# chaitjo/efficient-gnns

Measured on NVIDIA H100. Metric: edges aggregated/s (fwd+bwd), 3-layer GCN student + logit-KD, ARXIV-shape, higher is better.
Workload: dtype f32

## Files before the change

### efficient-gnns_b200/csrc/dense_rows.cu

```cuda
#include "common.cuh"
#include "philox.cuh"

namespace b200gnn {

constexpr int ROWS_THREADS = 256;

struct RowMap {
  int nvec, rows_per_iter, cv, rg;
  bool active;
};
__device__ __forceinline__ RowMap make_row_map(int K) {
  RowMap m;
  m.nvec = K >> 2;
  m.rows_per_iter = ROWS_THREADS / m.nvec;
  m.rg = threadIdx.x / m.nvec;
  m.cv = threadIdx.x - m.rg * m.nvec;
  m.active = m.rg < m.rows_per_iter;
  return m;
}

__device__ __forceinline__ float4 ld4(const float* p) { return *reinterpret_cast<const float4*>(p); }
__device__ __forceinline__ float4 ld4s(const float* p) { return __ldcs(reinterpret_cast<const float4*>(p)); }
__device__ __forceinline__ void st4(float* p, const float4& v) { *reinterpret_cast<float4*>(p) = v; }

// ... 132 lines not shown
        y.z = m.z ? y.z * inv_keep : 0.f; y.w = m.w ? y.w * inv_keep : 0.f;
      }
      st4(out + 4 * i, y);
    }
  }
}

struct RowScatter {
  float* ptr[16];
  int32_t off[17];
  int32_t n;
  int64_t ld, col;
};
__device__ __forceinline__ float* scatter_row(const RowScatter& sc, int64_t r) {
  int q = 0;
#pragma unroll 1
  while (q + 1 < sc.n && r >= sc.off[q + 1]) ++q;
  return sc.ptr[q] + (size_t)(r - sc.off[q]) * (size_t)sc.ld + sc.col;
}

template <bool P16>
__global__ void __launch_bounds__(256) affine_relu_dropout_mapped_kernel(
    const float* __restrict__ Y, float* __restrict__ out, int64_t n_rows, int nvec_l, const float* __restrict__ scale,
    const float* __restrict__ shift, int relu, float p, uint32_t thr16, uint64_t seed, uint64_t offset,
    const int32_t* __restrict__ step_dev, uint64_t step_mul, const int32_t* __restrict__ rowmap, uint64_t row_offset,
    uint64_t nvec_g, uint64_t cv_off, int paired, const RowScatter sc) {
  const float inv_keep = p > 0.f ? 1.f / (1.f - p) : 1.f;
  if (step_dev) offset += (uint64_t)(*step_dev) * step_mul;
  const int64_t tid = (int64_t)blockIdx.x * blockDim.x + threadIdx.x, stride = (int64_t)gridDim.x * blockDim.x;
  if (P16 && paired) {
    const int half_l = nvec_l >> 1;
    for (int64_t u = tid; u < n_rows * half_l; u += stride) {
      const int64_t r = u / half_l;
      const int cv = (int)(u - r * half_l) * 2;
      const uint64_t gid = rowmap ? (uint64_t)rowmap[r] : (uint64_t)r + row_offset;
      const uint64_t g = gid * nvec_g + cv_off + (uint64_t)cv;
      const uint4 rnd = philox4x32(seed, offset, g >> 1);
#pragma unroll
      for (int half = 0; half < 2; ++half) {
        const int64_t i = r * nvec_l + cv + half;
        float4 y = affine_relu4(ld4s(Y + 4 * i), scale, shift, cv + half, relu);
        const uchar4 m = keep16(half ? rnd.z : rnd.x, half ? rnd.w : rnd.y, thr16);
        y.x = m.x ? y.x * inv_keep : 0.f; y.y = m.y ? y.y * inv_keep : 0.f;
        y.z = m.z ? y.z * inv_keep : 0.f; y.w = m.w ? y.w * inv_keep : 0.f;
        st4(out + 4 * i, y);
        if (sc.n) st4(scatter_row(sc, r) + 4 * (cv + half), y);
      }
    }
    return;
  }
  for (int64_t i = tid; i < n_rows * nvec_l; i += stride) {
    const int64_t r = i / nvec_l;
    const int cv = (int)(i - r * nvec_l);
    float4 y = affine_relu4(ld4s(Y + 4 * i), scale, shift, cv, relu);
    if (p > 0.f) {
      const uint64_t gid = rowmap ? (uint64_t)rowmap[r] : (uint64_t)r + row_offset;
      const uint64_t g = gid * nvec_g + cv_off + (uint64_t)cv;
      uchar4 m;
      if (P16) {
        const uint4 rnd = philox4x32(seed, offset, g >> 1);
        m = keep16((g & 1) ? rnd.z : rnd.x, (g & 1) ? rnd.w : rnd.y, thr16);
      } else {
        m = keep24(philox4x32(seed, offset, g), p);
      }
      y.x = m.x ? y.x * inv_keep : 0.f; y.y = m.y ? y.y * inv_keep : 0.f;
      y.z = m.z ? y.z * inv_keep : 0.f; y.w = m.w ? y.w * inv_keep : 0.f;
    }
    st4(out + 4 * i, y);
    if (sc.n) st4(scatter_row(sc, r) + 4 * cv, y);
  }
}

__global__ void __launch_bounds__(256) dropout_mask_kernel(uint8_t* __restrict__ mask, int64_t n_vec, float p, int p16,
                                                           uint32_t thr16, uint64_t seed, uint64_t offset) {
  for (int64_t i = (int64_t)blockIdx.x * blockDim.x + threadIdx.x; i < n_vec; i += (int64_t)gridDim.x * blockDim.x) {
    uchar4 m;
    if (p16) {
      const uint4 r = philox4x32(seed, offset, (uint64_t)i >> 1);
      m = keep16((i & 1) ? r.z : r.x, (i & 1) ? r.w : r.y, thr16);
    } else {
      m = keep24(philox4x32(seed, offset, (uint64_t)i), p);
    }
    reinterpret_cast<uchar4*>(mask)[i] = m;
  }
}

static inline bool dropout_p16(float p, uint32_t& thr16) {
  const double t = (double)p * 65536.0;
  thr16 = (uint32_t)t;
  return p > 0.f && t == (double)thr16;
}

__global__ void __launch_bounds__(256) relu_dropout_bwd_kernel(const float4* __restrict__ dOut, const float4* __restrict__ Xout,
                                                               float4* dY, int64_t n_vec, float inv_keep) {
  for (int64_t i = (int64_t)blockIdx.x * blockDim.x + threadIdx.x; i < n_vec; i += (int64_t)gridDim.x * blockDim.x) {
    const float4 g = dOut[i], x = Xout[i];
    float4 d;
    d.x = x.x > 0.f ? g.x * inv_keep : 0.f; d.y = x.y > 0.f ? g.y * inv_keep : 0.f;
    d.z = x.z > 0.f ? g.z * inv_keep : 0.f; d.w = x.w > 0.f ? g.w * inv_keep : 0.f;
    dY[i] = d;
  }
}

__global__ void __launch_bounds__(ROWS_THREADS) bn_act_bwd_reduce_kernel(
    const float* __restrict__ dOut, const float* __restrict__ Xout, const float* __restrict__ Y,
    const float* __restrict__ mean, const float* __restrict__ invstd, int64_t n_rows, int K, float inv_keep,
    float* __restrict__ partial, int slots) {
  extern __shared__ float smem[];
  const RowMap m = make_row_map(K);
  const int64_t per = (n_rows + slots - 1) / slots;
  const int64_t r0 = (int64_t)blockIdx.x * per, r1 = min(n_rows, r0 + per);
  float4 s = make_float4(0, 0, 0, 0), q = s;
  if (m.active) {
    const float4 mu = ld4(mean + 4 * m.cv), is = ld4(invstd + 4 * m.cv);
    for (int64_t r = r0 + m.rg; r < r1; r += m.rows_per_iter) {
      const size_t o = (size_t)r * K + 4 * m.cv;
      const float4 g = ld4(dOut + o), x = ld4(Xout + o), y = ld4(Y + o);
      const float dx = x.x > 0.f ? g.x * inv_keep : 0.f, dy = x.y > 0.f ? g.y * inv_keep : 0.f;
      const float dz = x.z > 0.f ? g.z * inv_keep : 0.f, dw = x.w > 0.f ? g.w * inv_keep : 0.f;
      s.x += dx; s.y += dy; s.z += dz; s.w += dw;
      q.x = fmaf(dx, (y.x - mu.x) * is.x, q.x); q.y = fmaf(dy, (y.y - mu.y) * is.y, q.y);
      q.z = fmaf(dz, (y.z - mu.z) * is.z, q.z); q.w = fmaf(dw, (y.w - mu.w) * is.w, q.w);
    }
  }
  reduce_store_2xK(m, K, s, q, smem, partial + (size_t)blockIdx.x * 2 * K);
}

__global__ void __launch_bounds__(256) bn_bwd_finalize_kernel(const float* __restrict__ partial, int slots, int K,
                                                              int64_t n, const float* __restrict__ gamma,
                                                              const float* __restrict__ invstd, float* dgamma,
                                                              float* dbeta, float* coef ) {
  double s, q; int k;
  if (finalize_reduce(partial, slots, K, true, s, q, k)) {
    dbeta[k] = (float)s;
    dgamma[k] = (float)q;
    coef[k] = gamma[k] * invstd[k];
    coef[K + k] = (float)(s / (double)n);
    coef[2 * K + k] = (float)(q / (double)n);
  }
}

template <bool DZ>
__global__ void __launch_bounds__(ROWS_THREADS) bn_act_bwd_apply_kernel(
    const float* __restrict__ dOut, const float* __restrict__ Xout, const float* __restrict__ Y,
    const float* __restrict__ mean, const float* __restrict__ invstd, const float* __restrict__ coef, int64_t n_rows,
    int K, float inv_keep, float* __restrict__ dY, float* __restrict__ colsum_partial, int slots) {
  extern __shared__ float smem[];
  const RowMap m = make_row_map(K);
  const int64_t per = (n_rows + slots - 1) / slots;
  const int64_t r0 = (int64_t)blockIdx.x * per, r1 = min(n_rows, r0 + per);
  float4 s = make_float4(0, 0, 0, 0), q = s;
  if (m.active) {
    const float4 mu = ld4(mean + 4 * m.cv), is = ld4(invstd + 4 * m.cv);
    const float4 c1 = ld4(coef + 4 * m.cv), c2 = ld4(coef + K + 4 * m.cv), c3 = ld4(coef + 2 * K + 4 * m.cv);
    for (int64_t r = r0 + m.rg; r < r1; r += m.rows_per_iter) {
      const size_t o = (size_t)r * K + 4 * m.cv;
      float4 g = ld4s(dOut + o);
      const float4 y = ld4s(Y + o);
      if (!DZ) {
        const float4 x = ld4s(Xout + o);
        g.x = x.x > 0.f ? g.x * inv_keep : 0.f; g.y = x.y > 0.f ? g.y * inv_keep : 0.f;
        g.z = x.z > 0.f ? g.z * inv_keep : 0.f; g.w = x.w > 0.f ? g.w * inv_keep : 0.f;
      }
      float4 d;
      d.x = c1.x * (g.x - c2.x - (y.x - mu.x) * is.x * c3.x);
      d.y = c1.y * (g.y - c2.y - (y.y - mu.y) * is.y * c3.y);
// ... 87 lines not shown
  if (!rows_ok(n_rows, K) || !Y || !out || p < 0.f || p >= 1.f || ((scale == nullptr) != (shift == nullptr)) ||
      !aligned_to(Y, 16) || !aligned_to(out, 16))
    return B200GNN_ERR_BAD_ARG;
  if (n_rows == 0) return B200GNN_OK;
  const int64_t n_vec = n_rows * (K / 4);
  uint32_t thr16 = 0;
  if (dropout_p16(p, thr16))
    affine_relu_dropout_kernel<true><<<grid_for((n_vec + 1) / 2 + 1, 256 * 2), 256, 0, (cudaStream_t)stream>>>(
        Y, out, n_vec, (int)(K / 4), scale, shift, relu, p, thr16, seed, offset, step_dev, step_mul,
        row_offset * (uint64_t)(K / 4));
  else
    affine_relu_dropout_kernel<false><<<grid_for(n_vec, 256 * 4), 256, 0, (cudaStream_t)stream>>>(
        Y, out, n_vec, (int)(K / 4), scale, shift, relu, p, 0u, seed, offset, step_dev, step_mul,
        row_offset * (uint64_t)(K / 4));
  return check_launch();
}

static int mapped_launch(const float* Y, float* out, int64_t n_rows, int64_t K, const float* scale, const float* shift, int relu,
                         float p, uint64_t seed, uint64_t offset, const int32_t* step_dev, uint64_t step_mul, const int32_t* rowmap,
                         uint64_t row_offset, int64_t K_global, int64_t col_offset, const RowScatter& sc, void* stream) {
  if (!rows_ok(n_rows, K) || !Y || !out || p < 0.f || p >= 1.f || ((scale == nullptr) != (shift == nullptr)) ||
      !aligned_to(Y, 16) || !aligned_to(out, 16) || K_global < K || K_global % 4 || col_offset < 0 || col_offset % 4 ||
      col_offset + K > K_global)
    return B200GNN_ERR_BAD_ARG;
  if (n_rows == 0) return B200GNN_OK;
  const int nvec_l = (int)(K / 4);
  const uint64_t nvec_g = (uint64_t)(K_global / 4), cv_off = (uint64_t)(col_offset / 4);
  const int paired = (nvec_l % 2 == 0 && nvec_g % 2 == 0 && cv_off % 2 == 0) ? 1 : 0;
  const int64_t n_vec = n_rows * nvec_l;
  uint32_t thr16 = 0;
  if (dropout_p16(p, thr16))
    affine_relu_dropout_mapped_kernel<true><<<grid_for(paired ? n_vec / 2 : n_vec, 256 * 2), 256, 0, (cudaStream_t)stream>>>(
        Y, out, n_rows, nvec_l, scale, shift, relu, p, thr16, seed, offset, step_dev, step_mul, rowmap, row_offset, nvec_g,
        cv_off, paired, sc);
  else
    affine_relu_dropout_mapped_kernel<false><<<grid_for(n_vec, 256 * 4), 256, 0, (cudaStream_t)stream>>>(
        Y, out, n_rows, nvec_l, scale, shift, relu, p, 0u, seed, offset, step_dev, step_mul, rowmap, row_offset, nvec_g,
        cv_off, 0, sc);
  return check_launch();
}

extern "C" int b200gnn_affine_relu_dropout_mapped_f32(const float* Y, float* out, int64_t n_rows, int64_t K,
                                                      const float* scale, const float* shift, int relu, float p,
                                                      uint64_t seed, uint64_t offset, const int32_t* step_dev,
                                                      uint64_t step_mul, const int32_t* rowmap, uint64_t row_offset,
                                                      int64_t K_global, int64_t col_offset, void* stream) {
  RowScatter sc;
  sc.n = 0; sc.ld = 0; sc.col = 0;
  return mapped_launch(Y, out, n_rows, K, scale, shift, relu, p, seed, offset, step_dev, step_mul, rowmap, row_offset, K_global,
                       col_offset, sc, stream);
}

extern "C" int b200gnn_affine_relu_dropout_scatter_f32(const float* Y, float* out, int64_t n_rows, int64_t K,
                                                       const float* scale, const float* shift, int relu, float p,
                                                       uint64_t seed, uint64_t offset, const int32_t* step_dev,
                                                       uint64_t step_mul, const int32_t* rowmap, uint64_t row_offset,
                                                       int64_t K_global, int64_t col_offset, float* const* dst_ptrs,
                                                       const int32_t* row_off, int32_t world, int64_t ld_dst, void* stream) {
  if (!dst_ptrs || !row_off || world <= 0 || world > 16 || ld_dst < K_global || ld_dst % 4 || row_off[0] != 0 ||
      row_off[world] != n_rows)
    return B200GNN_ERR_BAD_ARG;
  RowScatter sc;
  sc.n = world; sc.ld = ld_dst; sc.col = col_offset;
  for (int q = 0; q < world; ++q) {
    if (!dst_ptrs[q] || !aligned_to(dst_ptrs[q], 16) || row_off[q + 1] < row_off[q]) return B200GNN_ERR_BAD_ARG;
    sc.ptr[q] = dst_ptrs[q]; sc.off[q] = row_off[q];
  }
  sc.off[world] = row_off[world];
  return mapped_launch(Y, out, n_rows, K, scale, shift, relu, p, seed, offset, step_dev, step_mul, rowmap, row_offset, K_global,
                       col_offset, sc, stream);
}

extern "C" int b200gnn_dropout_mask_u8(uint8_t* mask, int64_t n_rows, int64_t K, float p, uint64_t seed,
                                       uint64_t offset, void* stream) {
  if (!rows_ok(n_rows, K) || !mask || p < 0.f || p >= 1.f) return B200GNN_ERR_BAD_ARG;
  if (n_rows == 0) return B200GNN_OK;
  const int64_t n_vec = n_rows * (K / 4);
  uint32_t thr16 = 0;
  const int p16 = dropout_p16(p, thr16) ? 1 : 0;
  dropout_mask_kernel<<<grid_for(n_vec, 256 * 4), 256, 0, (cudaStream_t)stream>>>(mask, n_vec, p, p16, thr16, seed, offset);
  return check_launch();
}

extern "C" int b200gnn_relu_dropout_bwd_f32(const float* dOut, const float* Xout, float* dY, int64_t n_rows, int64_t K,
                                            float p, void* stream) {
  if (!rows_ok(n_rows, K) || p < 0.f || p >= 1.f) return B200GNN_ERR_BAD_ARG;
  if (n_rows == 0) return B200GNN_OK;
  if (!dOut || !Xout || !dY || !aligned_to(dOut, 16) || !aligned_to(Xout, 16) || !aligned_to(dY, 16)) return B200GNN_ERR_BAD_ARG;
  const int64_t n_vec = n_rows * (K / 4);
  const float inv_keep = p > 0.f ? 1.f / (1.f - p) : 1.f;
  relu_dropout_bwd_kernel<<<grid_for(n_vec, 256 * 4), 256, 0, (cudaStream_t)stream>>>(
      reinterpret_cast<const float4*>(dOut), reinterpret_cast<const float4*>(Xout), reinterpret_cast<float4*>(dY), n_vec, inv_keep);
  return check_launch();
}

extern "C" int b200gnn_bn_act_bwd_reduce_f32(const float* dOut, const float* Xout, const float* Y, const float* mean,
                                             const float* invstd, int64_t n_rows, int64_t K, float p, float* partial,
                                             int64_t slots, void* stream) {
  if (!rows_ok(n_rows, K) || n_rows == 0 || !dOut || !Xout || !Y || !mean || !invstd || !partial || slots < 1 ||
      p < 0.f || p >= 1.f)
    return B200GNN_ERR_BAD_ARG;
  if (ROWS_THREADS / (K / 4) < 1) return B200GNN_ERR_UNSUPPORTED;
  const float inv_keep = p > 0.f ? 1.f / (1.f - p) : 1.f;
  bn_act_bwd_reduce_kernel<<<(int)slots, ROWS_THREADS, 2 * K * sizeof(float), (cudaStream_t)stream>>>(
      dOut, Xout, Y, mean, invstd, n_rows, (int)K, inv_keep, partial, (int)slots);
  return check_launch();
}

extern "C" int b200gnn_bn_act_bwd_apply_f32(const float* dOut, const float* Xout, const float* Y, const float* mean,
                                            const float* invstd, const float* gamma, const float* sums,
                                            int64_t sum_slots, int64_t n_norm, int64_t n_rows, int64_t K, float p,
                                            float* dY, float* dgamma, float* dbeta, float* dbias, float* partial,
                                            int64_t slots, float* coef, void* stream) {
  if (!rows_ok(n_rows, K) || n_rows == 0 || !dOut || !Y || !mean || !invstd || !gamma || !sums || !dY ||
      !dgamma || !dbeta || !partial || !coef || slots < 1 || sum_slots < 1 || n_norm < 1 || p < 0.f || p >= 1.f)
    return B200GNN_ERR_BAD_ARG;
  cudaStream_t st = (cudaStream_t)stream;
  const float inv_keep = p > 0.f ? 1.f / (1.f - p) : 1.f;
  const size_t smem = 2 * K * sizeof(float);
  int rc;
  bn_bwd_finalize_kernel<<<(int)((K + FIN_COLS - 1) / FIN_COLS), 256, 0, st>>>(sums, (int)sum_slots, (int)K, n_norm, gamma,
                                                                              invstd, dgamma, dbeta, coef);
  if ((rc = check_launch())) return rc;
  if (Xout)
    bn_act_bwd_apply_kernel<false><<<(int)slots, ROWS_THREADS, smem, st>>>(dOut, Xout, Y, mean, invstd, coef, n_rows, (int)K,
                                                                          inv_keep, dY, dbias ? partial : nullptr, (int)slots);
  else
    bn_act_bwd_apply_kernel<true><<<(int)slots, ROWS_THREADS, smem, st>>>(dOut, nullptr, Y, mean, invstd, coef, n_rows, (int)K,
                                                                         inv_keep, dY, dbias ? partial : nullptr, (int)slots);
  if ((rc = check_launch())) return rc;
  if (dbias) {
    colsum_finalize_kernel<<<(int)((K + FIN_COLS - 1) / FIN_COLS), 256, 0, st>>>(partial, (int)slots, (int)K, dbias);
    if ((rc = check_launch())) return rc;
  }
  return B200GNN_OK;
}

extern "C" int b200gnn_bn_act_bwd_f32(const float* dOut, const float* Xout, const float* Y, const float* mean,
                                      const float* invstd, const float* gamma, int64_t n_rows, int64_t K, float p,
                                      float* dY, float* dgamma, float* dbeta, float* dbias, float* partial,
                                      int64_t slots, float* coef, void* stream) {
  int rc = b200gnn_bn_act_bwd_reduce_f32(dOut, Xout, Y, mean, invstd, n_rows, K, p, partial, slots, stream);
  if (rc) return rc;
  return b200gnn_bn_act_bwd_apply_f32(dOut, Xout, Y, mean, invstd, gamma, partial, slots, n_rows, n_rows, K, p, dY,
                                      dgamma, dbeta, dbias, partial, slots, coef, stream);
}

extern "C" int b200gnn_partial_reduce_f32(const float* partial, int64_t slots, int64_t K2, float* out, void* stream) {
  if (!partial || !out || slots < 1 || K2 < 1) return B200GNN_ERR_BAD_ARG;
  partial_reduce_kernel<<<(int)((K2 + FIN_COLS - 1) / FIN_COLS), 256, 0, (cudaStream_t)stream>>>(partial, (int)slots, (int)K2,
                                                                                               out);
  return check_launch();
}

extern "C" int b200gnn_col_sum_f32(const float* Y, int64_t n_rows, int64_t K, float* out, float* partial,
                                   int64_t slots, void* stream) {
  if (!rows_ok(n_rows, K) || !Y || !out || !partial || slots < 1) return B200GNN_ERR_BAD_ARG;
  cudaStream_t st = (cudaStream_t)stream;
  int rc;
  col_stats4_kernel<<<(int)slots, ROWS_THREADS, 2 * K * sizeof(float), st>>>(Y, n_rows, (int)K, partial, (int)slots);
  if ((rc = check_launch())) return rc;
  colsum_finalize_kernel<<<(int)((K + FIN_COLS - 1) / FIN_COLS), 256, 0, st>>>(partial, (int)slots, (int)K, out);
  return check_launch();
}

extern "C" int b200gnn_adam_step_f32(float* params, const float* grads, float* exp_avg, float* exp_avg_sq, int64_t n,
// ... 12 lines not shown
```

### efficient-gnns_b200/csrc/gemm_tf32x3.cu

```cuda
#include <cuda.h>

#include "common.cuh"
#include "tc_common.cuh"

namespace b200gnn {
namespace gemm {
using namespace tc;

constexpr int BM = 128, BK = 32;
constexpr int THREADS = 384;
constexpr int CONSUMER_WARPS = 8;
constexpr int TILE_BYTES = BM * BK * 4;
constexpr int BAR_BYTES = 256;
constexpr int EPI_BYTES = CONSUMER_WARPS * 16 * 32 * 4;
constexpr int STAT_MAX_N = 256;
constexpr int STAT_BYTES = CONSUMER_WARPS * 2 * STAT_MAX_N * 4;
constexpr int XY_ROWS = 16;
constexpr int XY_SLOT_BYTES = 2 * XY_ROWS * 32 * 4;
constexpr int XY_BYTES = CONSUMER_WARPS * 2 * XY_SLOT_BYTES;
constexpr int XY_BAR_OFF = 128;
constexpr int BNBWD_TMA_MAX_K = 128;

template <int BN_T, int NSTAGE, int EXTRA = 0>
struct Cfg {
  static constexpr int BN = BN_T, STAGES = NSTAGE;
  static constexpr int B_TILE_BYTES = BN_T * BK * 4;
  static constexpr int STAGE_BYTES = TILE_BYTES + 2 * B_TILE_BYTES;
  static constexpr int ACC = BN_T / 2;
  static constexpr int SMEM_BYTES = NSTAGE * STAGE_BYTES + BAR_BYTES + EPI_BYTES + STAT_BYTES + EXTRA + 1024;
  static_assert(B_TILE_BYTES % 1024 == 0 && (BN_T == 128 || BN_T == 48), "tile shape (wgmma wrappers: N = 128, 48)");
  static_assert(2 * NSTAGE * 8 <= XY_BAR_OFF, "barrier block");
  static_assert(SMEM_BYTES <= 232448, "shared memory");
};

__device__ __forceinline__ void mma(float (&d)[64], const uint32_t (&a)[4], uint64_t b, uint32_t s) { wgmma_tf32_n128_rs(d, a, b, s); }
__device__ __forceinline__ void mma(float (&d)[24], const uint32_t (&a)[4], uint64_t b, uint32_t s) { wgmma_tf32_n48_rs(d, a, b, s); }

__device__ __forceinline__ uint32_t a_frag_offset(int r0, int lane) { return r0 * 128 + ((lane >> 2) << 4) + (lane & 3) * 4; }
__device__ __forceinline__ void load_a(uint32_t frag, uint32_t (&v)[BK / 8][4]) {
  asm("" : "+r"(frag));
#pragma unroll
  for (int k = 0; k < BK / 8; ++k)
#pragma unroll
    for (int i = 0; i < 4; ++i) v[k][i] = lds32((frag ^ ((2 * k + (i >> 1)) << 4)) + (i & 1) * 8 * 128);
}

__device__ __forceinline__ int stg(int r, int c4) { return r * 32 + ((c4 ^ (r & 7)) << 2); }

struct Params {
  float* C;
  const float* bias;
  int64_t ldc;
  int32_t M, N, K;
  int32_t accumulate;
  float* Cp[16];
  int32_t n_peer, kc;
  int64_t row_off;
  int32_t bcast;
  int32_t stat_mode;
  float* stat_partial;
  const float* bn_x;
  const float* bn_y;
  const float* bn_mean;
  const float* bn_invstd;
  float inv_keep;
};

__device__ __forceinline__ void load_bn_chunk(const Params& p, int m0, int col, int q, int lane, float4 (&x)[4], float4 (&y)[4]) {
  if (col + 32 > p.N) return;
  const int sub = lane >> 3, cq = (lane & 7) * 4;
#pragma unroll
  for (int it = 0; it < 4; ++it) {
    const int grow = m0 + q * 16 + it * 4 + sub;
    if (grow < p.M) {
      const size_t o = (size_t)grow * p.ldc + col + cq;
      x[it] = __ldg(reinterpret_cast<const float4*>(p.bn_x + o));
      y[it] = __ldg(reinterpret_cast<const float4*>(p.bn_y + o));
    }
  }
}

template <class C, int STAT, bool PEER>
__global__ void __launch_bounds__(THREADS, 1)
gemm_tf32x3_kernel(const __grid_constant__ CUtensorMap tmA, const __grid_constant__ CUtensorMap tmBhi,
                   const __grid_constant__ CUtensorMap tmBlo, const __grid_constant__ CUtensorMap tmX,
                   const __grid_constant__ CUtensorMap tmY, const Params p) {
  constexpr bool BNB = STAT >= 2;
  constexpr bool XYTMA = STAT == 3;
  constexpr int BN = C::BN, STAGES = C::STAGES, STAGE_BYTES = C::STAGE_BYTES, B_TILE_BYTES = C::B_TILE_BYTES, ACC = C::ACC;
  extern __shared__ uint8_t smem_raw[];
  uint8_t* smem = reinterpret_cast<uint8_t*>((reinterpret_cast<uintptr_t>(smem_raw) + 1023) & ~(uintptr_t)1023);
  uint64_t* bars = reinterpret_cast<uint64_t*>(smem + STAGES * STAGE_BYTES);
  uint64_t* full = bars;
  uint64_t* empty = bars + STAGES;
  float* epi_smem = reinterpret_cast<float*>(smem + STAGES * STAGE_BYTES + BAR_BYTES);
  float* stat_smem = reinterpret_cast<float*>(smem + STAGES * STAGE_BYTES + BAR_BYTES + EPI_BYTES);
  uint8_t* xy_smem = smem + STAGES * STAGE_BYTES + BAR_BYTES + EPI_BYTES + STAT_BYTES;
  uint64_t* xy_full = reinterpret_cast<uint64_t*>(smem + STAGES * STAGE_BYTES + XY_BAR_OFF);

  const int warp = threadIdx.x >> 5, lane = threadIdx.x & 31;

  if (threadIdx.x == 0) {
    for (int s = 0; s < STAGES; ++s) { mbar_init(&full[s], 1); mbar_init(&empty[s], 256); }
    if (XYTMA)
      for (int i = 0; i < 2 * CONSUMER_WARPS; ++i) mbar_init(&xy_full[i], 1);
    asm volatile("fence.mbarrier_init.release.cluster;" ::: "memory");
  }
  __syncthreads();

  const int num_m = (p.M + BM - 1) / BM, num_n = (p.N + BN - 1) / BN;
  const int num_tiles = num_m * num_n;
  const int num_kb = (p.K + BK - 1) / BK;

  if (warp < 4) {
    regs_dec<40>();
    if (threadIdx.x == 0) {
      int s = 0; uint32_t ph = 0;
      for (int tile = blockIdx.x; tile < num_tiles; tile += gridDim.x) {
        const int m0 = (tile / num_n) * BM, n0 = (tile % num_n) * BN;
        for (int kb = 0; kb < num_kb; ++kb) {
          mbar_wait(&empty[s], ph ^ 1);
          uint8_t* st = smem + s * STAGE_BYTES;
          mbar_expect_tx(&full[s], TILE_BYTES + 2 * B_TILE_BYTES);
          tma_load_2d(&tmA, &full[s], st, kb * BK, m0);
          tma_load_2d(&tmBhi, &full[s], st + TILE_BYTES, kb * BK, n0);
          tma_load_2d(&tmBlo, &full[s], st + TILE_BYTES + B_TILE_BYTES, kb * BK, n0);
          if (++s == STAGES) { s = 0; ph ^= 1; }
        }
      }
    }
    return;
  }
  regs_inc<232>();

  const int q = warp - 4;
  const bool vec_ok = PEER ? true : ((p.ldc % 4 == 0) && ((reinterpret_cast<uintptr_t>(p.C) & 15) == 0));
  float* stat = stat_smem + q * (2 * STAT_MAX_N);
  if (STAT) {
    for (int i = lane; i < 2 * p.N; i += 32) stat[i] = 0.f;
    __syncwarp();
  }
  constexpr int NCHUNK = (BN + 31) / 32;
  uint8_t* xy = xy_smem + q * (2 * XY_SLOT_BYTES);
  uint64_t* xyb = xy_full + q * 2;
  int n_mine = 0;
  if (XYTMA) {
    for (int tt = blockIdx.x; tt < num_tiles; tt += gridDim.x) n_mine += NCHUNK;
    if (lane == 0)
      for (int g = 0; g < 2 && g < n_mine; ++g) {
        const int tt = blockIdx.x + (g / NCHUNK) * gridDim.x, cc = g % NCHUNK;
        mbar_expect_tx(&xyb[g], XY_SLOT_BYTES);
        tma_load_2d(&tmX, &xyb[g], xy + g * XY_SLOT_BYTES, (tt % num_n) * BN + cc * 32, (tt / num_n) * BM + q * XY_ROWS);
        tma_load_2d(&tmY, &xyb[g], xy + g * XY_SLOT_BYTES + XY_SLOT_BYTES / 2, (tt % num_n) * BN + cc * 32,
                    (tt / num_n) * BM + q * XY_ROWS);
      }
  }
  float acc[ACC], sum[ACC];
  uint32_t ah0[BK / 8][4], al0[BK / 8][4], ah1[BK / 8][4], al1[BK / 8][4];
  const uint32_t frag = a_frag_offset(q * 16 + (lane >> 2), lane);
  int s = 0; uint32_t ph = 0;
  int g_chunk = 0;
  for (int tile = blockIdx.x; tile < num_tiles; tile += gridDim.x) {
    const int m0 = (tile / num_n) * BM, n0 = (tile % num_n) * BN;
#pragma unroll
    for (int i = 0; i < ACC; ++i) sum[i] = acc[i] = 0.f;
    int prev = 0;
    auto stage = [&](int kb, uint32_t (&h)[BK / 8][4], uint32_t (&l)[BK / 8][4]) {
      mbar_wait(&full[s], ph);
      uint8_t* st = smem + s * STAGE_BYTES;
      load_a(smem_u32(st) + frag, h);
#pragma unroll
      for (int k = 0; k < BK / 8; ++k)
#pragma unroll
        for (int i = 0; i < 4; ++i) split1(h[k][i], h[k][i], l[k][i]);
      reg_fence(h); reg_fence(l);
      if (kb > 0) {
        wgmma_wait<0>();
        acc_fence(acc);
#pragma unroll
        for (int i = 0; i < ACC; ++i) sum[i] += acc[i];
        mbar_arrive(&empty[prev]);
      }
      wgmma_fence();
      const uint32_t sb = smem_u32(st + TILE_BYTES);
#pragma unroll
      for (int k = 0; k < BK / 8; ++k) {
        const uint32_t koff = k * 32;
        mma(acc, l[k], make_desc_k128(sb + koff), k != 0);
        mma(acc, h[k], make_desc_k128(sb + B_TILE_BYTES + koff), 1);
      }
#pragma unroll
      for (int k = 0; k < BK / 8; ++k) mma(acc, h[k], make_desc_k128(sb + k * 32), 1);
      wgmma_commit();
      prev = s;
      if (++s == STAGES) { s = 0; ph ^= 1; }
    };
    for (int kb = 0; kb < num_kb; kb += 2) {
      stage(kb, ah0, al0);
      if (kb + 1 < num_kb) stage(kb + 1, ah1, al1);
    }
    wgmma_wait<0>();
    acc_fence(acc);
#pragma unroll
    for (int i = 0; i < ACC; ++i) sum[i] += acc[i];
    mbar_arrive(&empty[prev]);

    float* tile_s = epi_smem + q * (16 * 32);
#pragma unroll
    for (int c = 0; c < NCHUNK; ++c, ++g_chunk) {
      const int col0 = n0 + c * 32;
      float4 xr[4], yr[4];
      if (STAT == 2) load_bn_chunk(p, m0, col0, q, lane, xr, yr);
#pragma unroll
      for (int jj = 0; jj < 4; ++jj) {
        const int j = c * 4 + jj;
        if (j * 8 < BN) {
          const int r0 = lane >> 2, cc = jj * 8 + 2 * (lane & 3);
          *reinterpret_cast<float2*>(tile_s + stg(r0, cc >> 2) + (cc & 3)) = make_float2(sum[4 * j], sum[4 * j + 1]);
          *reinterpret_cast<float2*>(tile_s + stg(r0 + 8, cc >> 2) + (cc & 3)) = make_float2(sum[4 * j + 2], sum[4 * j + 3]);
        }
      }
      __syncwarp();
      if (vec_ok && col0 + 32 <= p.N) {
        const float* xs = reinterpret_cast<const float*>(xy + (g_chunk & 1) * XY_SLOT_BYTES);
        const float* ys = xs + XY_ROWS * 32;
        if (XYTMA) mbar_wait(&xyb[g_chunk & 1], (uint32_t)((g_chunk >> 1) & 1));
        const int sub = lane >> 3, cq = (lane & 7) * 4;
        float4 b4 = make_float4(0.f, 0.f, 0.f, 0.f);
        if (p.bias) b4 = make_float4(__ldg(p.bias + col0 + cq), __ldg(p.bias + col0 + cq + 1), __ldg(p.bias + col0 + cq + 2),
                                     __ldg(p.bias + col0 + cq + 3));
        float4 s4 = make_float4(0.f, 0.f, 0.f, 0.f), q4 = s4, mu4 = s4, is4 = s4;
        if (BNB) {
          mu4 = __ldg(reinterpret_cast<const float4*>(p.bn_mean + col0 + cq));
          is4 = __ldg(reinterpret_cast<const float4*>(p.bn_invstd + col0 + cq));
        }
#pragma unroll
        for (int it = 0; it < 4; ++it) {
          const int rr = it * 4 + sub;
          const int grow = m0 + q * 16 + rr;
          float4 v = *reinterpret_cast<const float4*>(tile_s + stg(rr, lane & 7));
          v.x += b4.x; v.y += b4.y; v.z += b4.z; v.w += b4.w;
          if (PEER && grow < p.M && p.bcast) {
            for (int r = 0; r < p.n_peer; ++r)
              *reinterpret_cast<float4*>(p.Cp[r] + (size_t)(p.row_off + grow) * p.ldc + col0 + cq) = v;
          } else if (grow < p.M) {
            float4* dst;
            if (PEER) {
              const int r = col0 / p.kc;
              dst = reinterpret_cast<float4*>(p.Cp[r] + (size_t)(p.row_off + grow) * p.kc + (col0 - r * p.kc) + cq);
            } else {
              dst = reinterpret_cast<float4*>(p.C + (size_t)grow * p.ldc + col0 + cq);
            }
            if (!PEER && p.accumulate) { const float4 o = *dst; v.x += o.x; v.y += o.y; v.z += o.z; v.w += o.w; }
            if (STAT == 1) {
              vstat(s4, q4, v);
            } else if (BNB) {
              const float4 x = XYTMA ? *reinterpret_cast<const float4*>(xs + rr * 32 + cq) : xr[it];
              const float4 y = XYTMA ? *reinterpret_cast<const float4*>(ys + rr * 32 + cq) : yr[it];
              v.x = x.x > 0.f ? v.x * p.inv_keep : 0.f; v.y = x.y > 0.f ? v.y * p.inv_keep : 0.f;
              v.z = x.z > 0.f ? v.z * p.inv_keep : 0.f; v.w = x.w > 0.f ? v.w * p.inv_keep : 0.f;
              s4.x += v.x; s4.y += v.y; s4.z += v.z; s4.w += v.w;
              q4.x = fmaf(v.x, (y.x - mu4.x) * is4.x, q4.x); q4.y = fmaf(v.y, (y.y - mu4.y) * is4.y, q4.y);
              q4.z = fmaf(v.z, (y.z - mu4.z) * is4.z, q4.z); q4.w = fmaf(v.w, (y.w - mu4.w) * is4.w, q4.w);
            }
            *dst = v;
          }
        }
        if (STAT) {
#pragma unroll
          for (int d = 8; d <= 16; d <<= 1) {
            s4.x += __shfl_xor_sync(0xffffffffu, s4.x, d); s4.y += __shfl_xor_sync(0xffffffffu, s4.y, d);
            s4.z += __shfl_xor_sync(0xffffffffu, s4.z, d); s4.w += __shfl_xor_sync(0xffffffffu, s4.w, d);
            q4.x += __shfl_xor_sync(0xffffffffu, q4.x, d); q4.y += __shfl_xor_sync(0xffffffffu, q4.y, d);
            q4.z += __shfl_xor_sync(0xffffffffu, q4.z, d); q4.w += __shfl_xor_sync(0xffffffffu, q4.w, d);
          }
          if (lane < 8) {
            float4* ps = reinterpret_cast<float4*>(stat + col0 + cq);
            float4* pq = reinterpret_cast<float4*>(stat + p.N + col0 + cq);
            float4 a0 = *ps, a1 = *pq;
            a0.x += s4.x; a0.y += s4.y; a0.z += s4.z; a0.w += s4.w;
            a1.x += q4.x; a1.y += q4.y; a1.z += q4.z; a1.w += q4.w;
            *ps = a0; *pq = a1;
          }
        }
        __syncwarp();
        if (XYTMA && lane == 0 && g_chunk + 2 < n_mine) {
          const int g = g_chunk + 2, tt = blockIdx.x + (g / NCHUNK) * gridDim.x, cc = g % NCHUNK;
          uint8_t* dst = xy + (g & 1) * XY_SLOT_BYTES;
          mbar_expect_tx(&xyb[g & 1], XY_SLOT_BYTES);
          tma_load_2d(&tmX, &xyb[g & 1], dst, (tt % num_n) * BN + cc * 32, (tt / num_n) * BM + q * XY_ROWS);
          tma_load_2d(&tmY, &xyb[g & 1], dst + XY_SLOT_BYTES / 2, (tt % num_n) * BN + cc * 32, (tt / num_n) * BM + q * XY_ROWS);
        }
      } else {
        const int rr = lane & 15, cb = (lane >> 4) * 16, grow = m0 + q * 16 + rr;
        if (grow < p.M && col0 + cb < p.N) {
          for (int jx = 0; jx < 16; ++jx) {
            const int cc = cb + jx, col = col0 + cc;
            if (col >= p.N) break;
            const float v = tile_s[stg(rr, cc >> 2) + (cc & 3)] + (p.bias ? __ldg(p.bias + col) : 0.f);
            if (PEER && p.bcast) {
              for (int r = 0; r < p.n_peer; ++r) p.Cp[r][(size_t)(p.row_off + grow) * p.ldc + col] = v;
            } else if (!PEER) {
              float* dst = p.C + (size_t)grow * p.ldc + col;
              *dst = v + (p.accumulate ? *dst : 0.f);
            }
          }
        }
        __syncwarp();
      }
    }
  }
  if (STAT) {
    __syncwarp();
    float* out = p.stat_partial + (size_t)(blockIdx.x * CONSUMER_WARPS + q) * 2 * p.N;
    for (int i = lane; i < 2 * p.N; i += 32) out[i] = stat[i];
  }
}

__global__ void __launch_bounds__(256) split_tf32_kernel(const float* __restrict__ W, int64_t rows, int64_t cols,
                                                         int transpose, float* __restrict__ hi, float* __restrict__ lo) {
  const int64_t n = rows * cols;
  for (int64_t i = (int64_t)blockIdx.x * blockDim.x + threadIdx.x; i < n; i += (int64_t)gridDim.x * blockDim.x) {
    const int64_t r = i / cols, c = i - r * cols;
    uint32_t h, l;
    split1(__float_as_uint(W[i]), h, l);
    const int64_t o = transpose ? c * rows + r : i;
    hi[o] = __uint_as_float(h);
    lo[o] = __uint_as_float(l);
  }
}

static bool make_map(CUtensorMap* m, const float* base, int64_t rows, int64_t cols, int64_t ld, int box_rows, bool swizzle = true) {
  EncodeTiledFn fn = encode_fn();
  if (!fn) return false;
  cuuint64_t dims[2] = {(cuuint64_t)cols, (cuuint64_t)rows};
  cuuint64_t strides[1] = {(cuuint64_t)ld * 4};
  cuuint32_t box[2] = {(cuuint32_t)BK, (cuuint32_t)box_rows};
  cuuint32_t estr[2] = {1, 1};
  return fn(m, CU_TENSOR_MAP_DATA_TYPE_FLOAT32, 2, const_cast<float*>(base), dims, strides, box, estr,
            CU_TENSOR_MAP_INTERLEAVE_NONE, swizzle ? CU_TENSOR_MAP_SWIZZLE_128B : CU_TENSOR_MAP_SWIZZLE_NONE,
            CU_TENSOR_MAP_L2_PROMOTION_L2_256B, CU_TENSOR_MAP_FLOAT_OOB_FILL_NONE) == CUDA_SUCCESS;
}

template <class C, int STAT = 0, bool PEER = false>
static int launch(const float* A, int64_t lda, const float* B_hi, const float* B_lo, int64_t ldb, const Params& p,
                  cudaStream_t stream) {
  CUtensorMap tA, tBh, tBl, tX, tY;
  if (!make_map(&tA, A, p.M, p.K, lda, BM) || !make_map(&tBh, B_hi, p.N, p.K, ldb, C::BN) ||
      !make_map(&tBl, B_lo, p.N, p.K, ldb, C::BN))
    return B200GNN_ERR_UNSUPPORTED;
  tX = tA; tY = tA;
  if (STAT == 3 && (!make_map(&tX, p.bn_x, p.M, p.N, p.ldc, XY_ROWS, false) || !make_map(&tY, p.bn_y, p.M, p.N, p.ldc, XY_ROWS, false)))
    return B200GNN_ERR_UNSUPPORTED;
  int dev = 0, sms = 132;
  cudaGetDevice(&dev);
  static bool attr_set[64] = {};
  if (dev >= 0 && dev < 64 && !attr_set[dev]) {
    cudaError_t e = cudaFuncSetAttribute(gemm_tf32x3_kernel<C, STAT, PEER>, cudaFuncAttributeMaxDynamicSharedMemorySize, C::SMEM_BYTES);
    if (e != cudaSuccess) { set_cuda_error(e); return B200GNN_ERR_CUDA; }
    attr_set[dev] = true;
  }
  const int tiles = ((p.M + BM - 1) / BM) * ((p.N + C::BN - 1) / C::BN);
  cudaDeviceGetAttribute(&sms, cudaDevAttrMultiProcessorCount, dev);
  const int grid = tiles < sms ? tiles : sms;
  gemm_tf32x3_kernel<C, STAT, PEER><<<grid, THREADS, C::SMEM_BYTES, stream>>>(tA, tBh, tBl, tX, tY, p);
  return check_launch();
}

}
}

using namespace b200gnn;

extern "C" int b200gnn_split_tf32_f32(const float* W, int64_t rows, int64_t cols, int transpose, float* hi, float* lo,
                                      void* stream) {
  if (!W || !hi || !lo || rows <= 0 || cols <= 0) return B200GNN_ERR_BAD_ARG;
  const int64_t n = rows * cols;
  int grid = (int)((n + 255) / 256);
  if (grid > 132 * 8) grid = 132 * 8;
  gemm::split_tf32_kernel<<<grid, 256, 0, (cudaStream_t)stream>>>(W, rows, cols, transpose, hi, lo);
  return check_launch();
}

static int g_bnbwd_variant = 0;
extern "C" void b200gnn_gemm_set_bnbwd_variant(int v) { g_bnbwd_variant = v; }

static int gemm_dispatch(const float* A, int64_t lda, const float* B_hi, const float* B_lo, int64_t ldb, float* C, int64_t ldc,
                         int64_t M, int64_t N, int64_t K, const float* bias, int accumulate, void* stream,
                         const gemm::Params* st = nullptr) {
  if (!A || !B_hi || !B_lo || !C || M <= 0 || N <= 0 || K <= 0 || lda < K || ldb < K || ldc < N ||
      M >= INT32_MAX || N >= INT32_MAX || K >= INT32_MAX)
    return B200GNN_ERR_BAD_ARG;
  if (lda % 4 || ldb % 4 || !aligned_to(A, 16) || !aligned_to(B_hi, 16) || !aligned_to(B_lo, 16))
    return B200GNN_ERR_UNSUPPORTED;
  gemm::Params p{};
  p.C = C; p.bias = bias; p.ldc = ldc; p.M = (int32_t)M; p.N = (int32_t)N; p.K = (int32_t)K; p.accumulate = accumulate ? 1 : 0;
  p.n_peer = 0; p.kc = 0; p.row_off = 0; p.bcast = 0;
  if (st) {
    if (N % 32 || N > gemm::STAT_MAX_N || N <= 48 || ldc % 4 || !aligned_to(C, 16) || !st->stat_partial) return B200GNN_ERR_UNSUPPORTED;
    p.stat_mode = st->stat_mode; p.stat_partial = st->stat_partial; p.bn_x = st->bn_x; p.bn_y = st->bn_y;
    p.bn_mean = st->bn_mean; p.bn_invstd = st->bn_invstd; p.inv_keep = st->inv_keep;
    if (p.stat_mode == 1) return gemm::launch<gemm::Cfg<128, 4>, 1>(A, lda, B_hi, B_lo, ldb, p, (cudaStream_t)stream);
    if (N % 128 == 0 && (g_bnbwd_variant == 1 || (g_bnbwd_variant == 0 && K < gemm::BNBWD_TMA_MAX_K)))
      return gemm::launch<gemm::Cfg<128, 2, gemm::XY_BYTES>, 3>(A, lda, B_hi, B_lo, ldb, p, (cudaStream_t)stream);
    return gemm::launch<gemm::Cfg<128, 4>, 2>(A, lda, B_hi, B_lo, ldb, p, (cudaStream_t)stream);
  }
  if (N <= 48) return gemm::launch<gemm::Cfg<48, 6>>(A, lda, B_hi, B_lo, ldb, p, (cudaStream_t)stream);
  return gemm::launch<gemm::Cfg<128, 4>>(A, lda, B_hi, B_lo, ldb, p, (cudaStream_t)stream);
}

extern "C" int64_t b200gnn_gemm_stat_slots(int64_t M, int64_t N) {
  if (M <= 0 || N <= 0) return B200GNN_ERR_BAD_ARG;
  int dev = 0, sms = 132;
  cudaGetDevice(&dev);
  cudaDeviceGetAttribute(&sms, cudaDevAttrMultiProcessorCount, dev);
  const int64_t tiles = ((M + gemm::BM - 1) / gemm::BM) * ((N + 127) / 128);
  return gemm::CONSUMER_WARPS * (tiles < sms ? tiles : sms);
}

extern "C" int b200gnn_gemm_tf32x3_stats_f32(const float* A, int64_t lda, const float* B_hi, const float* B_lo, int64_t ldb,
                                             float* C, int64_t ldc, int64_t M, int64_t N, int64_t K, const float* bias,
                                             int accumulate, float* partial, int64_t slots, void* stream) {
  if (!partial || slots < b200gnn_gemm_stat_slots(M, N) || (accumulate && bias)) return B200GNN_ERR_BAD_ARG;
  gemm::Params st{};
  st.stat_mode = 1; st.stat_partial = partial;
  return gemm_dispatch(A, lda, B_hi, B_lo, ldb, C, ldc, M, N, K, bias, accumulate, stream, &st);
}

extern "C" int b200gnn_gemm_tf32x3_bnbwd_f32(const float* A, int64_t lda, const float* B_hi, const float* B_lo, int64_t ldb,
                                             float* C, int64_t ldc, int64_t M, int64_t N, int64_t K, int accumulate,
                                             const float* Xout, const float* Y, const float* mean, const float* invstd, float p_drop,
                                             float* partial, int64_t slots, void* stream) {
  if (!partial || !Xout || !Y || !mean || !invstd || p_drop < 0.f || p_drop >= 1.f || slots < b200gnn_gemm_stat_slots(M, N))
    return B200GNN_ERR_BAD_ARG;
  if (!aligned_to(Xout, 16) || !aligned_to(Y, 16) || !aligned_to(mean, 16) || !aligned_to(invstd, 16)) return B200GNN_ERR_UNSUPPORTED;
  gemm::Params st{};
  st.stat_mode = 2; st.stat_partial = partial; st.bn_x = Xout; st.bn_y = Y; st.bn_mean = mean; st.bn_invstd = invstd;
  st.inv_keep = p_drop > 0.f ? 1.f / (1.f - p_drop) : 1.f;
  return gemm_dispatch(A, lda, B_hi, B_lo, ldb, C, ldc, M, N, K, nullptr, accumulate, stream, &st);
}

extern "C" int b200gnn_gemm_tf32x3_f32(const float* A, int64_t lda, const float* B_hi, const float* B_lo, int64_t ldb,
                                       float* C, int64_t ldc, int64_t M, int64_t N, int64_t K, const float* bias,
                                       void* stream) {
  return gemm_dispatch(A, lda, B_hi, B_lo, ldb, C, ldc, M, N, K, bias, 0, stream);
}

extern "C" int b200gnn_gemm_tf32x3_acc_f32(const float* A, int64_t lda, const float* B_hi, const float* B_lo, int64_t ldb,
                                           float* C, int64_t ldc, int64_t M, int64_t N, int64_t K, void* stream) {
  return gemm_dispatch(A, lda, B_hi, B_lo, ldb, C, ldc, M, N, K, nullptr, 1, stream);
}

extern "C" int b200gnn_gemm_tf32x3_scatter_f32(const float* A, int64_t lda, const float* B_hi, const float* B_lo, int64_t ldb,
                                               float* const* C_ptrs, int32_t world, int64_t row_off, int64_t M, int64_t N, int64_t K,
                                               const float* bias, void* stream) {
  if (!A || !B_hi || !B_lo || !C_ptrs || world <= 0 || world > 16 || M <= 0 || N <= 0 || K <= 0 || lda < K || ldb < K || row_off < 0 ||
      M >= INT32_MAX || N >= INT32_MAX || K >= INT32_MAX)
    return B200GNN_ERR_BAD_ARG;
  if (N % world || (N / world) % 32 || N <= 48) return B200GNN_ERR_UNSUPPORTED;
  if (lda % 4 || ldb % 4 || !aligned_to(A, 16) || !aligned_to(B_hi, 16) || !aligned_to(B_lo, 16)) return B200GNN_ERR_UNSUPPORTED;
  gemm::Params p{};
  p.C = nullptr; p.bias = bias; p.ldc = N; p.M = (int32_t)M; p.N = (int32_t)N; p.K = (int32_t)K; p.accumulate = 0;
  p.n_peer = world; p.kc = (int32_t)(N / world); p.row_off = row_off; p.bcast = 0;
  for (int q = 0; q < world; ++q) {
    if (!C_ptrs[q] || !aligned_to(C_ptrs[q], 16)) return B200GNN_ERR_BAD_ARG;
    p.Cp[q] = C_ptrs[q];
  }
  return gemm::launch<gemm::Cfg<128, 4>, 0, true>(A, lda, B_hi, B_lo, ldb, p, (cudaStream_t)stream);
}

extern "C" int b200gnn_gemm_tf32x3_bcast_f32(const float* A, int64_t lda, const float* B_hi, const float* B_lo, int64_t ldb,
                                             float* const* C_ptrs, int32_t world, int64_t row_off, int64_t ldc, int64_t M, int64_t N,
                                             int64_t K, const float* bias, void* stream) {
  if (!A || !B_hi || !B_lo || !C_ptrs || world <= 0 || world > 16 || M <= 0 || N <= 0 || K <= 0 || lda < K || ldb < K || ldc < N ||
      row_off < 0 || M >= INT32_MAX || N >= INT32_MAX || K >= INT32_MAX)
    return B200GNN_ERR_BAD_ARG;
  if (lda % 4 || ldb % 4 || ldc % 4 || !aligned_to(A, 16) || !aligned_to(B_hi, 16) || !aligned_to(B_lo, 16)) return B200GNN_ERR_UNSUPPORTED;
  gemm::Params p{};
  p.C = C_ptrs[0]; p.bias = bias; p.ldc = ldc; p.M = (int32_t)M; p.N = (int32_t)N; p.K = (int32_t)K; p.accumulate = 0;
  p.n_peer = world; p.kc = (int32_t)N; p.row_off = row_off; p.bcast = 1;
  for (int q = 0; q < world; ++q) {
    if (!C_ptrs[q] || !aligned_to(C_ptrs[q], 16)) return B200GNN_ERR_BAD_ARG;
    p.Cp[q] = C_ptrs[q];
  }
  if (N <= 48) return gemm::launch<gemm::Cfg<48, 6>, 0, true>(A, lda, B_hi, B_lo, ldb, p, (cudaStream_t)stream);
  return gemm::launch<gemm::Cfg<128, 4>, 0, true>(A, lda, B_hi, B_lo, ldb, p, (cudaStream_t)stream);
}
```

### efficient-gnns_b200/csrc/gemm_wgrad_tf32x3.cu

```cuda
#include "common.cuh"
#include "tc_common.cuh"

namespace b200gnn {
namespace wgrad {
using namespace tc;

constexpr int BKN = 32;
constexpr int TM = 128, TN = 128;
constexpr int THREADS = 384;
constexpr int STAGES = 5;
constexpr int X_BOX = 8;
constexpr int RAW_BYTES = BKN * (TM + TN) * 4;
constexpr int OP_BYTES = 128 * BKN * 4;
constexpr int T_BYTES = 2 * OP_BYTES;
constexpr int SMEM_BYTES = STAGES * RAW_BYTES + 2 * T_BYTES + 256 + 1024;
constexpr int MAX_RANGES = 132;
constexpr int64_t MAX_PARTIAL_FLOATS = (int64_t)MAX_RANGES * 256 * 256;
constexpr int MAX_KIN = 2048, MAX_NOUT = 512;
static_assert(SMEM_BYTES <= 232448, "shared memory");

struct Params {
  float* partial;
  int32_t Nn, Kin, Kpad, Nout, Npad, num_kb;
  int32_t n_tn, n_ranges;
};

__global__ void __launch_bounds__(THREADS, 1)
wgrad_tf32x3_kernel(const __grid_constant__ CUtensorMap tmX, const __grid_constant__ CUtensorMap tmG, const Params p) {
  extern __shared__ uint8_t smem_raw[];
  uint8_t* smem = reinterpret_cast<uint8_t*>((reinterpret_cast<uintptr_t>(smem_raw) + 1023) & ~(uintptr_t)1023);
  uint8_t* tbuf = smem + STAGES * RAW_BYTES;
  uint64_t* full = reinterpret_cast<uint64_t*>(tbuf + 2 * T_BYTES);
  uint64_t* empty = full + STAGES;

  const int tiles = (p.Kpad / TM) * p.n_tn;
  const int tile = (int)blockIdx.x % tiles, range = (int)blockIdx.x / tiles;
  const int mt = tile / p.n_tn, nt = tile % p.n_tn;
  const int kb0 = (int)((int64_t)p.num_kb * range / p.n_ranges);
  const int kb1 = (int)((int64_t)p.num_kb * (range + 1) / p.n_ranges);

  const int warp = threadIdx.x >> 5, lane = threadIdx.x & 31;
  if (threadIdx.x == 0) {
    for (int s = 0; s < STAGES; ++s) { mbar_init(&full[s], 1); mbar_init(&empty[s], 256); }
    asm volatile("fence.mbarrier_init.release.cluster;" ::: "memory");
  }
  __syncthreads();

  if (warp < 4) {
    regs_dec<40>();
    if (threadIdx.x == 0) {
      int s = 0; uint32_t ph = 0;
      for (int kb = kb0; kb < kb1; ++kb) {
        mbar_wait(&empty[s], ph ^ 1);
        uint8_t* st = smem + s * RAW_BYTES;
        mbar_expect_tx(&full[s], RAW_BYTES);
        for (int j = 0; j < TM / X_BOX; ++j)
          tma_load_2d(&tmX, &full[s], st + j * BKN * X_BOX * 4, mt * TM + j * X_BOX, kb * BKN);
        tma_load_2d(&tmG, &full[s], st + BKN * TM * 4, nt * TN, kb * BKN);
        if (++s == STAGES) { s = 0; ph ^= 1; }
      }
    }
    return;
  }
  regs_inc<232>();

  const int cw = (warp >> 2) - 1;
  const int ct = threadIdx.x - 128;
  const uint32_t xfrag = (8 * cw + 2 * (warp & 3)) * (BKN * X_BOX * 4) + (lane & 3) * (X_BOX * 4) + (lane >> 2) * 4;
  float acc[64], sum[64];
#pragma unroll
  for (int i = 0; i < 64; ++i) sum[i] = acc[i] = 0.f;
  uint32_t xh0[BKN / 8][4], xl0[BKN / 8][4], xh1[BKN / 8][4], xl1[BKN / 8][4];
  int s = 0; uint32_t ph = 0;
  auto block = [&](int i, uint32_t (&h)[BKN / 8][4], uint32_t (&l)[BKN / 8][4]) {
    mbar_wait(&full[s], ph);
    const uint32_t sraw = smem_u32(smem + s * RAW_BYTES);
    const float* rg = reinterpret_cast<const float*>(smem + s * RAW_BYTES + BKN * TM * 4);
    uint8_t* T = tbuf + (i & 1) * T_BYTES;
#pragma unroll
    for (int u = 0; u < 4; ++u) {
      const int idx = u * 256 + ct;
      const int r = idx & 127, c = idx >> 7;
      const float* src = rg + (4 * c) * 128 + r;
      const uint4 v = make_uint4(__float_as_uint(src[0]), __float_as_uint(src[128]), __float_as_uint(src[256]),
                                 __float_as_uint(src[384]));
      uint4 hv, lv;
      split4(v, hv, lv);
      *reinterpret_cast<uint4*>(T + swz128(r, c)) = hv;
      *reinterpret_cast<uint4*>(T + OP_BYTES + swz128(r, c)) = lv;
    }
#pragma unroll
    for (int k = 0; k < BKN / 8; ++k)
#pragma unroll
      for (int j = 0; j < 4; ++j)
        split1(lds32(sraw + xfrag + (j & 1) * (BKN * X_BOX * 4) + (8 * k + 4 * (j >> 1)) * (X_BOX * 4)), h[k][j], l[k][j]);
    asm volatile("fence.proxy.async.shared::cta;" ::: "memory");
    mbar_arrive(&empty[s]);
    if (i > 0) {
      wgmma_wait<0>();
      acc_fence(acc);
#pragma unroll
      for (int j = 0; j < 64; ++j) sum[j] += acc[j];
    }
    named_sync(1, 256);
    reg_fence(h); reg_fence(l);
    wgmma_fence();
    const uint32_t sa = smem_u32(T);
#pragma unroll
    for (int k = 0; k < BKN / 8; ++k) {
      const uint32_t koff = k * 32;
      wgmma_tf32_n128_rs(acc, l[k], make_desc_k128(sa + koff), k != 0);
      wgmma_tf32_n128_rs(acc, h[k], make_desc_k128(sa + OP_BYTES + koff), 1);
    }
#pragma unroll
    for (int k = 0; k < BKN / 8; ++k) wgmma_tf32_n128_rs(acc, h[k], make_desc_k128(sa + k * 32), 1);
    wgmma_commit();
    if (++s == STAGES) { s = 0; ph ^= 1; }
  };
  for (int i = 0; i < kb1 - kb0; i += 2) {
    block(i, xh0, xl0);
    if (i + 1 < kb1 - kb0) block(i + 1, xh1, xl1);
  }
  if (kb1 > kb0) {
    wgmma_wait<0>();
    acc_fence(acc);
#pragma unroll
    for (int j = 0; j < 64; ++j) sum[j] += acc[j];
  }
  float* out = p.partial + (size_t)range * p.Kpad * p.Npad;
  const int row0 = mt * TM + cw * 64 + (warp & 3) * 16 + (lane >> 2);
#pragma unroll
  for (int j = 0; j < 16; ++j) {
    const int col = nt * TN + 8 * j + 2 * (lane & 3);
    if (col < p.Npad) {
      *reinterpret_cast<float2*>(out + (size_t)row0 * p.Npad + col) = make_float2(sum[4 * j], sum[4 * j + 1]);
      *reinterpret_cast<float2*>(out + (size_t)(row0 + 8) * p.Npad + col) = make_float2(sum[4 * j + 2], sum[4 * j + 3]);
    }
  }
}

constexpr int RED_VECS = 32, RED_GROUPS = 8;
__global__ void __launch_bounds__(RED_VECS * RED_GROUPS) wgrad_reduce_kernel(const float4* __restrict__ partial, int n_part,
                                                                             int Kin, int Kpad, int Nout, int Npad,
                                                                             float* __restrict__ out) {
  __shared__ float4 sh[RED_GROUPS][RED_VECS];
  const int64_t n_vec = (int64_t)Kpad * Npad / 4;
  const int v = threadIdx.x % RED_VECS, g = threadIdx.x / RED_VECS;
  const int64_t i = (int64_t)blockIdx.x * RED_VECS + v;
  float4 acc = make_float4(0.f, 0.f, 0.f, 0.f);
  if (i < n_vec)
    for (int c = g; c < n_part; c += RED_GROUPS) {
      const float4 x = __ldcs(partial + (size_t)c * n_vec + i);
      acc.x += x.x; acc.y += x.y; acc.z += x.z; acc.w += x.w;
    }
  sh[g][v] = acc;
  __syncthreads();
  if (g != 0 || i >= n_vec) return;
  const int row = (int)(i / (Npad / 4)), c4 = (int)(i % (Npad / 4)) * 4;
  if (c4 >= Nout || row >= Kin) return;
#pragma unroll
  for (int j = 1; j < RED_GROUPS; ++j) {
    const float4 x = sh[j][v];
    acc.x += x.x; acc.y += x.y; acc.z += x.z; acc.w += x.w;
  }
  *reinterpret_cast<float4*>(out + (size_t)row * Nout + c4) = acc;
}

static bool make_map_rows(CUtensorMap* m, const float* base, int64_t rows, int64_t width, int64_t ld, int box_cols) {
  EncodeTiledFn fn = encode_fn();
  if (!fn) return false;
  cuuint64_t dims[2] = {(cuuint64_t)width, (cuuint64_t)rows};
  cuuint64_t strides[1] = {(cuuint64_t)ld * 4};
  cuuint32_t box[2] = {(cuuint32_t)box_cols, (cuuint32_t)BKN};
  cuuint32_t estr[2] = {1, 1};
  return fn(m, CU_TENSOR_MAP_DATA_TYPE_FLOAT32, 2, const_cast<float*>(base), dims, strides, box, estr,
            CU_TENSOR_MAP_INTERLEAVE_NONE, CU_TENSOR_MAP_SWIZZLE_NONE, CU_TENSOR_MAP_L2_PROMOTION_L2_256B,
            CU_TENSOR_MAP_FLOAT_OOB_FILL_NONE) == CUDA_SUCCESS;
}

static int64_t pad_k(int64_t Kin) { return (Kin + TM - 1) / TM * TM; }
static int64_t pad_n(int64_t Nout) { return (Nout + 31) / 32 * 32; }
static int range_cap(int64_t Kin, int64_t Nout) {
  const int64_t c = MAX_PARTIAL_FLOATS / (pad_k(Kin) * pad_n(Nout));
  return (int)(c > MAX_RANGES ? MAX_RANGES : (c < 1 ? 1 : c));
}

}
}

using namespace b200gnn;

extern "C" int64_t b200gnn_wgrad_workspace_floats(int64_t Kin, int64_t Nout) {
  if (Kin <= 0 || Nout <= 0) return B200GNN_ERR_BAD_ARG;
  if (Kin > wgrad::MAX_KIN || Nout > wgrad::MAX_NOUT) return B200GNN_ERR_UNSUPPORTED;
  return wgrad::range_cap(Kin, Nout) * wgrad::pad_k(Kin) * wgrad::pad_n(Nout);
}

extern "C" int b200gnn_gemm_wgrad_tf32x3_f32(const float* X, int64_t ldx, const float* G, int64_t ldg, float* dW,
                                             int64_t Nn, int64_t Kin, int64_t Nout, float* workspace, void* stream) {
  if (!X || !G || !dW || !workspace || Nn <= 0 || Kin <= 0 || Nout <= 0 || ldx < Kin || ldg < Nout || Nn >= INT32_MAX)
    return B200GNN_ERR_BAD_ARG;
  if (Kin % 4 || Kin > wgrad::MAX_KIN || Nout % 4 || Nout > wgrad::MAX_NOUT || ldx % 4 || ldg % 4 || !aligned_to(X, 16) || !aligned_to(G, 16) ||
      !aligned_to(dW, 16) || !aligned_to(workspace, 16))
    return B200GNN_ERR_UNSUPPORTED;
  CUtensorMap tX, tG;
  if (!wgrad::make_map_rows(&tX, X, Nn, Kin, ldx, wgrad::X_BOX) || !wgrad::make_map_rows(&tG, G, Nn, Nout, ldg, wgrad::TN))
    return B200GNN_ERR_UNSUPPORTED;
  int dev = 0, sms = 132;
  cudaGetDevice(&dev);
  static bool attr_set[64] = {};
  if (dev >= 0 && dev < 64 && !attr_set[dev]) {
    cudaError_t e = cudaFuncSetAttribute(wgrad::wgrad_tf32x3_kernel, cudaFuncAttributeMaxDynamicSharedMemorySize,
                                         wgrad::SMEM_BYTES);
    if (e != cudaSuccess) { set_cuda_error(e); return B200GNN_ERR_CUDA; }
    attr_set[dev] = true;
  }
  cudaDeviceGetAttribute(&sms, cudaDevAttrMultiProcessorCount, dev);
  cudaStream_t st = (cudaStream_t)stream;
  wgrad::Params p;
  p.partial = workspace; p.Nn = (int32_t)Nn; p.Kin = (int32_t)Kin; p.Nout = (int32_t)Nout;
  p.Kpad = (int32_t)wgrad::pad_k(Kin);
  p.Npad = (int32_t)wgrad::pad_n(Nout);
  p.num_kb = (int32_t)((Nn + wgrad::BKN - 1) / wgrad::BKN);
  p.n_tn = (p.Npad + wgrad::TN - 1) / wgrad::TN;
  const int tiles = (int)(p.Kpad / wgrad::TM) * p.n_tn;
  int ranges = sms / tiles;
  const int cap = wgrad::range_cap(Kin, Nout);
  if (ranges > cap) ranges = cap;
  if (ranges > p.num_kb) ranges = p.num_kb;
  if (ranges < 1) ranges = 1;
  p.n_ranges = ranges;
  int rc;
  wgrad::wgrad_tf32x3_kernel<<<tiles * ranges, wgrad::THREADS, wgrad::SMEM_BYTES, st>>>(tX, tG, p);
  if ((rc = check_launch())) return rc;
  const int64_t n_vec = (int64_t)p.Kpad * p.Npad / 4;
  wgrad::wgrad_reduce_kernel<<<(int)((n_vec + wgrad::RED_VECS - 1) / wgrad::RED_VECS), wgrad::RED_VECS * wgrad::RED_GROUPS, 0, st>>>(
      reinterpret_cast<const float4*>(workspace), ranges, (int)Kin, p.Kpad, (int)Nout, p.Npad, dW);
  return check_launch();
}
```

### efficient-gnns_b200/dist.py

```python
from __future__ import annotations

import math
from dataclasses import dataclass
from typing import List, Optional

import torch
import torch.distributed as dist

from . import lib, ops
from .engine import GCNStudentTrainer, gcn_norm, _is_symmetric
from .sparse import SparseTensor, csr_graph_from


import os as _os
_DIAG_SKIP_COMM = _os.environ.get("B200GNN_DIAG_SKIP_ALLGATHER", "0") == "1"


@dataclass
class ShardPlan:
    world: int
    n: int
    block: int
    perm: torch.Tensor
    inv: torch.Tensor

    @property
    def n_pad(self) -> int:
        return self.world * self.block

    def real_rows(self, rank: int) -> int:
        full_rounds, rem = divmod(self.n, self.world)
        if rem == 0:
            return full_rounds
        last_round = full_rounds
        k_of_rank = rank if last_round % 2 == 0 else self.world - 1 - rank
        return full_rounds + (1 if k_of_rank < rem else 0)

    def rows_of(self, rank: int):
        return rank * self.block, rank * self.block + self.real_rows(rank)


def make_plan(rowcount: torch.Tensor, world: int) -> ShardPlan:
    n = rowcount.numel()
    block = -(-n // world)
    order = torch.argsort(rowcount.cpu(), descending=True, stable=True)
    pos = torch.arange(n)
    rnd, k = pos // world, pos % world
    rank_of = torch.where(rnd % 2 == 0, k, world - 1 - k)
    slot = rnd
    new_id = rank_of * block + slot
    inv = torch.empty(n, dtype=torch.long)
    inv[order] = new_id
    perm = torch.full((world * block,), -1, dtype=torch.long)
    perm[new_id] = order
    return ShardPlan(world, n, block, perm, inv)


def relabel_adjacency(adj: SparseTensor, plan: ShardPlan) -> SparseTensor:
    row, col, val = adj.coo()
    inv = plan.inv.to(row.device)
    return SparseTensor(row=inv[row], col=inv[col], value=val, sparse_sizes=(plan.n_pad, plan.n_pad), is_sorted=False)


def shard_rows(adj_relabelled: SparseTensor, plan: ShardPlan, rank: int):
    rowptr, col, val = adj_relabelled.csr()
    r0, r1 = plan.rows_of(rank)
    e0, e1 = int(rowptr[r0]), int(rowptr[r1])
    return (rowptr[r0:r1 + 1] - e0).contiguous(), col[e0:e1].contiguous(), None if val is None else val[e0:e1].contiguous()


def scatter_rows(t: torch.Tensor, plan: ShardPlan, fill=0) -> torch.Tensor:
    out = torch.full((plan.n_pad,) + tuple(t.shape[1:]), fill, dtype=t.dtype, device=t.device)
    out[plan.inv.to(t.device)] = t
    return out


class ShardedGCNTrainer(GCNStudentTrainer):

    def __init__(self, adj: SparseTensor, dims: List[int], group=None, **kw):
        assert dist.is_initialized(), "torch.distributed must be initialised (backend nccl)"
        self.group = group
        self.rank, self.world = dist.get_rank(group), dist.get_world_size(group)
        norm = gcn_norm(adj)
        if not _is_symmetric(norm):
            raise NotImplementedError("node-parallel backward relies on a symmetric normalised adjacency")
        self.plan = make_plan(norm.storage.rowcount(), self.world)
        rel = relabel_adjacency(norm, self.plan)
        rowptr, col, val = shard_rows(rel, self.plan, self.rank)
        self._shard = csr_graph_from(rowptr, col, val, self.plan.real_rows(self.rank), self.plan.n_pad)
        self.n_global = adj.size(0)
        super().__init__(adj, dims, _prebuilt_graph=self._shard, _rows_alloc=self.plan.block, **kw)
        dev = self.device
        self.full = {k: torch.empty(self.plan.n_pad, k, device=dev) for k in set(dims[1:])}
        self.sum_buf = {k: torch.empty(2, k, device=dev) for k in set(dims[1:])}
        self.row0 = self.rank * self.plan.block
        self.n_train_global = 0

    def shard_inputs(self, x, y, train_idx, teacher_logits=None):
        plan, dev = self.plan, self.device
        r0, r1 = plan.rows_of(self.rank)
        x_pad = scatter_rows(x.to(dev), plan)
        y_loc = scatter_rows(y.to(dev), plan)[r0:r1].contiguous()
        t_loc = None if teacher_logits is None else scatter_rows(teacher_logits.to(dev), plan)[r0:r1].contiguous()
        new_train = plan.inv.to(dev)[train_idx.to(dev)]
        mine = new_train[(new_train >= r0) & (new_train < r1)] - r0
        self.n_train_global = int(train_idx.numel())
        return x_pad, y_loc, torch.sort(mine).values.contiguous(), t_loc

    def _block_of(self, view: torch.Tensor) -> torch.Tensor:
        for blk in self._blocks:
            if blk.data_ptr() == view.data_ptr() and blk.shape[1] == view.shape[1]:
                return blk
        raise KeyError("not an engine activation buffer")

    def gather_rows(self, local: torch.Tensor) -> torch.Tensor:
        blk = torch.zeros(self.plan.block, local.shape[1], device=local.device)
        blk[:local.shape[0]] = local
        full = torch.empty(self.plan.n_pad, local.shape[1], device=local.device)
        dist.all_gather_into_tensor(full, blk, group=self.group)
        return full[self.plan.inv.to(local.device)]

    def _all_gather(self, local: torch.Tensor) -> torch.Tensor:
        full = self.full[local.shape[1]]
        if _DIAG_SKIP_COMM:
            return full
        dist.all_gather_into_tensor(full, self._block_of(local), group=self.group)
        return full

    def _global_stats(self, partial: torch.Tensor, k: int) -> torch.Tensor:
        s = ops.partial_reduce(partial, out=self.sum_buf[k])
        dist.all_reduce(s, group=self.group)
        return s.view(1, 2, k)

    def forward(self, x_pad: torch.Tensor, training: bool = True) -> torch.Tensor:
        r0 = self.row0
        inp = None
        for l in range(self.L):
            last = l == self.L - 1
            k = self.dims[l + 1]
            if l == 0 and self.agg_first:
                ops.spmm_csr(self.G, x_pad, "sum", out=self.AX)
                self._linear(0, self.AX, self.Y[0], bias=self.b[0])
                part = ops.col_stats(self.Y[0], partial=self._part(k)) if training else None
            else:
                src = x_pad[r0:r0 + self.N] if l == 0 else inp
                self._linear(l, src, self.H[l])
                full = self._all_gather(self.H[l])
                if last or not training:
                    ops.spmm_csr(self.G, full, "sum", bias=self.b[l], out=self.Y[l]); part = None
                else:
                    part = self.stat_part[l]
                    ops.spmm_csr(self.G, full, "sum", bias=self.b[l], out=self.Y[l], stat_partial=part)
            if last:
                break
            if training:
                sums = self._global_stats(part, k)
                ops.bn_finalize(sums, self.n_global, self.gamma[l], self.beta[l], self.bn_eps, self.bn_momentum,
                                self.running_mean[l], self.running_var[l], out=self.bn[l])
                ops.affine_relu_dropout(self.Y[l], self.bn[l][2], self.bn[l][3], True, self.p, self.seed, l, out=self.A[l],
                                        step_dev=self.step_count, step_mul=self.L, row_offset=r0)
            else:
                scale = self.gamma[l] * torch.rsqrt(self.running_var[l] + self.bn_eps)
                shift = self.beta[l] - self.running_mean[l] * scale
                ops.affine_relu_dropout(self.Y[l], scale, shift, True, 0.0, out=self.A[l])
            inp = self.A[l]
        return self.Y[-1]

    def backward(self, x_pad: torch.Tensor):
        r0 = self.row0
        for l in range(self.L - 1, -1, -1):
            k_out = self.dims[l + 1]
            inp = x_pad[r0:r0 + self.N] if l == 0 else self.A[l - 1]
            if l == self.L - 1:
                ops.col_sum(self.dY[l], out=self.gb[l], partial=self._part(k_out))
# ... 37 lines not shown
```

### efficient-gnns_b200/engine.py

```python
from __future__ import annotations

import math
from typing import Dict, List, Optional

import torch

from . import lib, ops
from .sparse import CsrGraph, SparseTensor


def gcn_norm(adj: SparseTensor) -> SparseTensor:
    if not adj.has_value():
        adj = adj.fill_value(1.0)
    adj = adj.fill_diag(1.0)
    deg = adj.sum(dim=1)
    dis = deg.pow(-0.5)
    dis.masked_fill_(dis == float("inf"), 0.0)
    row, col, val = adj.coo()
    return adj.set_value(dis[row] * val * dis[col])


def _is_symmetric(adj: SparseTensor) -> bool:
    st = adj.storage
    if st.sparse_sizes()[0] != st.sparse_sizes()[1]:
        return False
    perm = st.csr2csc()
    same = torch.equal(st.col()[perm], st.row()) and torch.equal(st.row()[perm], st.col())
    if same and st.value() is not None:
        same = torch.equal(st.value()[perm], st.value())
    return bool(same)


class GCNStudentTrainer:

    def __init__(self, adj: SparseTensor, dims: List[int], dropout: float = 0.5, lr: float = 0.01, seed: int = 0,
                 alpha: float = 0.9, kd_T: float = 4.0, bn_eps: float = 1e-5, bn_momentum: float = 0.1,
                 aggregate_first: Optional[bool] = None, tensor_core_gemm: bool = True, overlap_wgrad: bool = True,
                 fuse_row_passes: bool = True, _prebuilt_graph: Optional[CsrGraph] = None, _rows_alloc: Optional[int] = None):
        assert adj.is_cuda(), "the engine runs on a CUDA device"
        self.device = adj.device
        self.dims, self.L = list(dims), len(dims) - 1
        self.p, self.lr, self.alpha, self.kd_T = float(dropout), float(lr), float(alpha), float(kd_T)
        self.bn_eps, self.bn_momentum = bn_eps, bn_momentum
        self.seed = int(seed)
        self.tc_gemm = bool(tensor_core_gemm) and all(d % 4 == 0 for d in dims)
        for d in dims[1:]:
            assert d % 4 == 0 and d <= 1024, "layer widths must be multiples of 4 (128-bit rows)"
        self.N = adj.size(0)
        self.agg_first = (dims[0] < dims[1] and dims[0] % 4 == 0) if aggregate_first is None else bool(aggregate_first)
        if self.L < 2:
            self.agg_first = False

        if _prebuilt_graph is not None:
            self.G = self.Gt = _prebuilt_graph
            self.N = _prebuilt_graph.n_rows
        else:
            norm = gcn_norm(adj)
            self.G: CsrGraph = norm.storage.engine_csr()
            self.Gt: CsrGraph = self.G if _is_symmetric(norm) else norm.storage.engine_csc("value")
        self.nnz = self.G.nnz

        sizes = []
        for l in range(self.L):
            sizes += [dims[l] * dims[l + 1], dims[l + 1]]
            if l < self.L - 1:
                sizes += [dims[l + 1], dims[l + 1]]
        n_par = sum(sizes)
        dev = self.device
        self.params = torch.zeros(n_par, device=dev)
        self.n_par_pad = (n_par + 3) // 4 * 4
        self._grads_buf = torch.zeros(self.n_par_pad + 4, device=dev)
        self.grads = self._grads_buf[:n_par]
        self.exp_avg = torch.zeros(n_par, device=dev)
        self.exp_avg_sq = torch.zeros(n_par, device=dev)
        self.step_count = torch.zeros(1, dtype=torch.int32, device=dev)
        self.W, self.b, self.gamma, self.beta = [], [], [], []
        self.gW, self.gb, self.ggamma, self.gbeta = [], [], [], []
        off = 0

        def take(n, shape):
            nonlocal off
            v = (self.params[off:off + n].view(shape), self.grads[off:off + n].view(shape))
            off += n
            return v
        for l in range(self.L):
            w, gw = take(dims[l] * dims[l + 1], (dims[l], dims[l + 1]))
            b, gb = take(dims[l + 1], (dims[l + 1],))
            self.W.append(w); self.gW.append(gw); self.b.append(b); self.gb.append(gb)
            if l < self.L - 1:
                g, gg = take(dims[l + 1], (dims[l + 1],))
                be, gbe = take(dims[l + 1], (dims[l + 1],))
                self.gamma.append(g); self.ggamma.append(gg); self.beta.append(be); self.gbeta.append(gbe)
        self.Wt_split = [(torch.empty(dims[l + 1], dims[l], device=dev), torch.empty(dims[l + 1], dims[l], device=dev))
                         for l in range(self.L)]
        self.W_split = [(torch.empty(dims[l], dims[l + 1], device=dev), torch.empty(dims[l], dims[l + 1], device=dev))
                        for l in range(self.L)]
        wg = [ops.wgrad_supported(dims[l], dims[l + 1]) for l in range(self.L)]
        self.wgrad_ws = (torch.empty(max(ops.wgrad_workspace_floats(dims[l], dims[l + 1]) for l in range(self.L) if wg[l]), device=dev)
                         if self.tc_gemm and any(wg) else None)
        self.running_mean = [torch.zeros(d, device=dev) for d in dims[1:-1]]
        self.running_var = [torch.ones(d, device=dev) for d in dims[1:-1]]
        self.reset_parameters(seed)

        N = self.N
        rows_alloc = N if _rows_alloc is None else _rows_alloc
        self._blocks = []

        def buf(k):
            blk = torch.zeros(rows_alloc, k, device=dev)
            self._blocks.append(blk)
            return blk[:N]
        self.H = [buf(dims[l + 1]) for l in range(self.L)]
        self.Y = [buf(dims[l + 1]) for l in range(self.L)]
        self.A = [buf(dims[l + 1]) for l in range(self.L - 1)]
        self.dY = [buf(dims[l + 1]) for l in range(self.L)]
        self.dH = [buf(dims[l + 1]) for l in range(self.L)]
        self.dA = [buf(dims[l + 1]) for l in range(self.L - 1)]
        self.AX = buf(dims[0]) if self.agg_first else None
        slots_spmm = ops.stat_slots(self.G)
        self.stat_part = [torch.empty(slots_spmm, 2, dims[l + 1], device=dev) for l in range(self.L - 1)]
        self.bn = [torch.empty(4, dims[l + 1], device=dev) for l in range(self.L - 1)]
        self.rs = ops.rows_slots(N)
        self.fuse_rows = bool(fuse_row_passes) and self.tc_gemm
        self._gemm_part = {k: torch.empty(ops.gemm_stat_slots(N, k), 2, k, device=dev)
                           for k in set(dims[1:-1]) if self.fuse_rows and ops.gemm_stats_supported(k)}
        self.loss_out = self._grads_buf[self.n_par_pad:self.n_par_pad + 3]
        self.kd_part = torch.empty(2 * int(lib.load().b200gnn_kd_partials(N)), device=dev)
        self._graph = None
        self.overlap_wgrad = overlap_wgrad
        self._side = torch.cuda.Stream(device=dev) if overlap_wgrad else None
        self._ev_fork, self._ev_join = torch.cuda.Event(), torch.cuda.Event()
        self._static: Dict[str, torch.Tensor] = {}
        for k in set(dims[1:]):
            self._part(k); self._coef(k)

    def reset_parameters(self, seed: int = 0):
        g = torch.Generator().manual_seed(seed)
        for l in range(self.L):
            fan_in, fan_out = self.dims[l], self.dims[l + 1]
            a = math.sqrt(6.0 / (fan_in + fan_out))
            self.W[l].copy_((torch.rand(fan_in, fan_out, generator=g) * 2 - 1) * a)
            self.b[l].zero_()
        for l in range(self.L - 1):
            self.gamma[l].fill_(1.0); self.beta[l].zero_()
            self.running_mean[l].zero_(); self.running_var[l].fill_(1.0)
        self.exp_avg.zero_(); self.exp_avg_sq.zero_(); self.step_count.zero_()

    def state_dict(self) -> Dict[str, torch.Tensor]:
        sd = {}
        for l in range(self.L):
            sd[f"convs.{l}.weight"] = self.W[l].detach().clone()
            sd[f"convs.{l}.bias"] = self.b[l].detach().clone()
        for l in range(self.L - 1):
            sd[f"bns.{l}.weight"] = self.gamma[l].detach().clone()
            sd[f"bns.{l}.bias"] = self.beta[l].detach().clone()
            sd[f"bns.{l}.running_mean"] = self.running_mean[l].clone()
            sd[f"bns.{l}.running_var"] = self.running_var[l].clone()
        return sd

    def load_state_dict(self, sd: Dict[str, torch.Tensor]):
        for l in range(self.L):
            self.W[l].copy_(sd[f"convs.{l}.weight"]); self.b[l].copy_(sd[f"convs.{l}.bias"])
        for l in range(self.L - 1):
            self.gamma[l].copy_(sd[f"bns.{l}.weight"]); self.beta[l].copy_(sd[f"bns.{l}.bias"])
            if f"bns.{l}.running_mean" in sd:
                self.running_mean[l].copy_(sd[f"bns.{l}.running_mean"]); self.running_var[l].copy_(sd[f"bns.{l}.running_var"])

    def activation_pattern(self, l: int) -> torch.Tensor:
        return self.A[l] > 0

    def out_feat(self) -> torch.Tensor:
        return self.A[-1]

    def dropout_offset(self, layer: int, step: int) -> int:
        return layer + step * self.L

    def forward(self, x: torch.Tensor, training: bool = True) -> torch.Tensor:
        inp = x
        for l in range(self.L):
            last = l == self.L - 1
            if l == 0 and self.agg_first:
                ops.spmm_csr(self.G, x, "sum", out=self.AX)
                if training:
                    gp = self._gemm_part.get(self.dims[1])
                    if gp is not None:
                        hi, lo = ops.split_tf32(self.W[0], transpose=True, hi=self.Wt_split[0][0], lo=self.Wt_split[0][1])
                        ops.gemm_tf32x3_stats(self.AX, hi, lo, self.b[0], self.Y[0], gp)
                        part = gp
                    else:
                        self._linear(0, self.AX, self.Y[0], bias=self.b[0])
                        part = ops.col_stats(self.Y[0], partial=self._part(self.dims[1]))
                    ops.bn_finalize(part, self.N, self.gamma[0], self.beta[0], self.bn_eps,
                                    self.bn_momentum, self.running_mean[0], self.running_var[0], out=self.bn[0])
                    ops.affine_relu_dropout(self.Y[0], self.bn[0][2], self.bn[0][3], True, self.p, self.seed, 0,
                                            out=self.A[0], step_dev=self.step_count, step_mul=self.L)
                else:
                    self._linear(0, self.AX, self.Y[0], bias=self.b[0])
                    scale = self.gamma[0] * torch.rsqrt(self.running_var[0] + self.bn_eps)
                    shift = self.beta[0] - self.running_mean[0] * scale
                    ops.affine_relu_dropout(self.Y[0], scale, shift, True, 0.0, out=self.A[0])
                inp = self.A[0]
                continue
            self._linear(l, inp, self.H[l])
            if last:
                ops.spmm_csr(self.G, self.H[l], "sum", bias=self.b[l], out=self.Y[l])
            elif training:
                ops.spmm_csr(self.G, self.H[l], "sum", bias=self.b[l], out=self.Y[l], stat_partial=self.stat_part[l])
                ops.bn_finalize(self.stat_part[l], self.N, self.gamma[l], self.beta[l], self.bn_eps, self.bn_momentum,
                                self.running_mean[l], self.running_var[l], out=self.bn[l])
                ops.affine_relu_dropout(self.Y[l], self.bn[l][2], self.bn[l][3], True, self.p, self.seed, l,
                                        out=self.A[l], step_dev=self.step_count, step_mul=self.L)
                inp = self.A[l]
            else:
                ops.spmm_csr(self.G, self.H[l], "sum", bias=self.b[l], out=self.Y[l])
                scale = self.gamma[l] * torch.rsqrt(self.running_var[l] + self.bn_eps)
                shift = self.beta[l] - self.running_mean[l] * scale
                ops.affine_relu_dropout(self.Y[l], scale, shift, True, 0.0, out=self.A[l])
                inp = self.A[l]
        return self.Y[-1]

    def backward(self, x: torch.Tensor, d_out_feat: Optional[torch.Tensor] = None):
        for l in range(self.L - 1, -1, -1):
            inp = x if l == 0 else self.A[l - 1]
            if l == self.L - 1:
                ops.col_sum(self.dY[l], out=self.gb[l], partial=self._part(self.dims[l + 1]))
            if l == 0 and self.agg_first:
                self._wgrad_async(0, self.AX, self.dY[0])
                continue
            ops.spmm_csr(self.Gt, self.dY[l], "sum", out=self.dH[l])
            d_prev = self.dA[l - 1] if l > 0 else None
            gp = self._gemm_part.get(self.dims[l]) if l > 0 else None
            if l > 0:
                acc = d_out_feat is not None and l == self.L - 1
                if acc:
                    d_prev = d_out_feat
                if gp is not None:
                    hi, lo = ops.split_tf32(self.W[l], transpose=False, hi=self.W_split[l][0], lo=self.W_split[l][1])
                    ops.gemm_tf32x3_bnbwd(self.dH[l], hi, lo, d_prev, self.A[l - 1], self.Y[l - 1], self.bn[l - 1][0],
                                          self.bn[l - 1][1], self.p, gp, accumulate=acc)
                else:
                    self._linear_dgrad(l, self.dH[l], d_prev, accumulate=acc)
            self._wgrad_async(l, inp, self.dH[l])
            if l > 0:
                k = self.dims[l]
                part = self._part(k)
                if gp is not None:
                    ops.bn_act_bwd_apply(d_prev, None, self.Y[l - 1], self.bn[l - 1][0], self.bn[l - 1][1], self.gamma[l - 1],
                                         gp, self.N, self.p, self.dY[l - 1], self.ggamma[l - 1], self.gbeta[l - 1],
                                         self.gb[l - 1], part, self._coef(k))
                else:
                    ops.bn_act_bwd(d_prev, self.A[l - 1], self.Y[l - 1], self.bn[l - 1][0], self.bn[l - 1][1],
                                   self.gamma[l - 1], self.p, d_y=self.dY[l - 1], d_gamma=self.ggamma[l - 1],
                                   d_beta=self.gbeta[l - 1], d_bias=self.gb[l - 1], partial=part, coef=self._coef(k))
        self._wgrad_join()

    def _wgrad_async(self, l: int, inp: torch.Tensor, d_out: torch.Tensor):
        if self._side is None:
            return self._linear_wgrad(l, inp, d_out)
        self._ev_fork.record(torch.cuda.current_stream())
        self._side.wait_event(self._ev_fork)
        with torch.cuda.stream(self._side):
            self._linear_wgrad(l, inp, d_out)

    def _wgrad_join(self):
        if self._side is not None:
            self._ev_join.record(self._side)
            torch.cuda.current_stream().wait_event(self._ev_join)

    def _linear(self, l: int, inp: torch.Tensor, out: torch.Tensor, bias: Optional[torch.Tensor] = None):
        if self.tc_gemm:
            hi, lo = ops.split_tf32(self.W[l], transpose=True, hi=self.Wt_split[l][0], lo=self.Wt_split[l][1])
            ops.gemm_tf32x3(inp, hi, lo, bias=bias, out=out)
        elif bias is not None:
            torch.addmm(bias, inp, self.W[l], out=out)
        else:
            torch.mm(inp, self.W[l], out=out)

    def _linear_dgrad(self, l: int, d_out: torch.Tensor, d_inp: torch.Tensor, accumulate: bool = False):
        if self.tc_gemm:
            hi, lo = ops.split_tf32(self.W[l], transpose=False, hi=self.W_split[l][0], lo=self.W_split[l][1])
            ops.gemm_tf32x3(d_out, hi, lo, out=d_inp, accumulate=accumulate)
        elif accumulate:
            d_inp.addmm_(d_out, self.W[l].t())
        else:
            torch.mm(d_out, self.W[l].t(), out=d_inp)

    def _linear_wgrad(self, l: int, inp: torch.Tensor, d_out: torch.Tensor):
        if self.tc_gemm and ops.wgrad_supported(self.dims[l], self.dims[l + 1]):
            ops.gemm_wgrad_tf32x3(inp, d_out, out=self.gW[l], workspace=self.wgrad_ws)
        else:
            torch.mm(inp.t(), d_out, out=self.gW[l])

    def _part(self, k: int) -> torch.Tensor:
        key = f"part{k}"
        if key not in self._static:
            self._static[key] = torch.empty(self.rs, 2, k, device=self.device)
        return self._static[key]

    def _coef(self, k: int) -> torch.Tensor:
        key = f"coef{k}"
        if key not in self._static:
            self._static[key] = torch.empty(3, k, device=self.device)
        return self._static[key]

    def _step_impl(self, x, y, train_idx, teacher_logits):
        logits = self.forward(x, training=True)
        self.dY[-1].zero_()
        ops.kd_loss_fwd_bwd(logits, y, train_idx, teacher_logits, self.alpha, self.kd_T, d_logits=self.dY[-1],
                            loss_out=self.loss_out, partial=self.kd_part)
        self.backward(x)
        ops.adam_step(self.params, self.grads, self.exp_avg, self.exp_avg_sq, self.step_count, self.lr)

    def train_step(self, x, y, train_idx, teacher_logits=None, aux=None, beta: float = 1.0) -> torch.Tensor:
        if aux is None:
            self._step_impl(x, y, train_idx, teacher_logits)
            return self.loss_out
        logits = self.forward(x, training=True)
        self.dY[-1].zero_()
        ops.kd_loss_fwd_bwd(logits, y, train_idx, teacher_logits, self.alpha, self.kd_T, d_logits=self.dY[-1],
                            loss_out=self.loss_out, partial=self.kd_part)
        feat = self.out_feat().detach().requires_grad_(True)
        with torch.enable_grad():
            loss_aux = aux(feat)
            (loss_aux * beta).backward()
        d_feat = feat.grad if feat.grad is not None else torch.zeros_like(feat)
        self.backward(x, d_out_feat=d_feat.contiguous())
        ops.adam_step(self.params, self.grads, self.exp_avg, self.exp_avg_sq, self.step_count, self.lr)
        self.loss_aux = loss_aux.detach()
        self.loss_out[0].add_(self.loss_aux * beta)
        return self.loss_out

    def capture(self, x, y, train_idx, teacher_logits=None, warmup: int = 2, key: int = 0):
        self._static.update(x=x, y=y, train_idx=train_idx, teacher=teacher_logits)
        s = torch.cuda.Stream()
        s.wait_stream(torch.cuda.current_stream())
        with torch.cuda.stream(s):
            for _ in range(warmup):
                self._step_impl(x, y, train_idx, teacher_logits)
        torch.cuda.current_stream().wait_stream(s)
        torch.cuda.synchronize()
        if self._graph is None:
            self._graph = {}
        g = torch.cuda.CUDAGraph()
        with torch.cuda.graph(g):
            self._step_impl(x, y, train_idx, teacher_logits)
        self._graph[key] = g
        return self

    def replay(self, key: int = 0) -> torch.Tensor:
        self._graph[key].replay()
        return self.loss_out

    def launches_per_step(self) -> int:
        before = lib.launch_count()
        st = self._static
        self._step_impl(st["x"], st["y"], st["train_idx"], st["teacher"])
        return lib.launch_count() - before

    def aggregations_per_step(self) -> Dict[int, int]:
        out: Dict[int, int] = {}
        for l in range(self.L):
            if l == 0 and self.agg_first:
                out[self.dims[0]] = out.get(self.dims[0], 0) + 1
            else:
                out[self.dims[l + 1]] = out.get(self.dims[l + 1], 0) + 2
        return out

    def spmm_algorithmic_bytes(self) -> Dict[int, int]:
        return {k: 2 * self.N * k * 4 + self.nnz * 8 + (self.N + 1) * 4 for k in set(self.dims)}
```

### efficient-gnns_b200/hybrid.py

```python
from __future__ import annotations

from dataclasses import dataclass
from typing import Dict, List, Optional

import torch
import torch.distributed as dist

from . import lib, ops
from .engine import GCNStudentTrainer, gcn_norm, _is_symmetric
from .sparse import SparseTensor, csr_graph_from


@dataclass
class DensePlan:
    world: int
    n: int
    counts: List[int]
    offsets: List[int]
    perm: torch.Tensor
    inv: torch.Tensor

    @property
    def block(self) -> int:
        return max(self.counts)
# ... 84 lines not shown
        self.n_p = plan.counts[rank]
        self.arena = PeerArena(arena_bytes, group)
        self._order = [(rank + 1 + i) % self.world for i in range(self.world)]

    def buffer(self, name: str, shape, device) -> torch.Tensor:
        return self.arena.alloc(name, shape)

    def fused_r2c_targets(self, name: str):
        return [self.arena.peer_ptr(name, q, 0) for q in range(self.world)]

    def barrier(self):
        self.arena.barrier()

    def fused_c2r_targets(self, name: str):
        return [self.arena.peer_ptr(name, q, 0) for q in range(self.world)]

    def r2c(self, src: torch.Tensor, dst: torch.Tensor, name: str):
        from .peer import copy2d
        P, n_p, K = self.world, self.n_p, src.shape[1]
        kc = K // P
        off = self.plan.offsets[self.rank]
        copies = [(self.arena.peer_ptr(name, q, off * kc), src.data_ptr() + 4 * q * kc, kc, src.stride(0), n_p) for q in self._order]
        self.arena.exchange(copies, kc)

    def c2r(self, src: torch.Tensor, dst: torch.Tensor, name: str):
        from .peer import copy2d
        P, kc = self.world, src.shape[1]
        K = kc * P
        copies = [(self.arena.peer_ptr(name, q, self.rank * kc), src.data_ptr() + 4 * self.plan.offsets[q] * src.stride(0), K,
                   src.stride(0), self.plan.counts[q]) for q in self._order]
        self.arena.exchange(copies, kc)

    def allgather_rows(self, src: torch.Tensor, dst: torch.Tensor, name: str):
        from .peer import copy2d
        K = src.shape[1]
        off = self.plan.offsets[self.rank]
        copies = [(self.arena.peer_ptr(name, q, off * K), src.data_ptr(), K, src.stride(0), self.n_p) for q in self._order]
        self.arena.exchange(copies, K)

    def allgather_vec(self, src: torch.Tensor, dst: torch.Tensor, name: str):
        from .peer import copy2d
        m = src.numel()
        assert m % 4 == 0
        copies = [(self.arena.peer_ptr(name, q, self.rank * m), src.data_ptr(), m, m, 1) for q in self._order]
        self.arena.exchange(copies, m)

    def check(self):
        if self.arena.error_flag():
            raise lib.B200GnnError("peer barrier timed out: a rank never arrived")


def _numel(shape) -> int:
    n = 1
    for d in shape:
        n *= int(d)
    return n


class HybridGCNTrainer(GCNStudentTrainer):

    def __init__(self, adj: SparseTensor, dims: List[int], group=None, exchange: str = "peer", _fake=None, fuse_r2c: bool = True,
                 fuse_c2r: bool = True, fuse_gather: bool = False, **kw):
        self.group = group
        self.fuse_r2c, self.fuse_c2r = bool(fuse_r2c), bool(fuse_c2r)
        self.fuse_gather = bool(fuse_gather)
        if _fake is not None:
            assert exchange == "null"
            self.rank, self.world = _fake
        else:
            assert dist.is_initialized(), "torch.distributed must be initialised"
            self.rank, self.world = dist.get_rank(group), dist.get_world_size(group)
        P = self.world
        norm = gcn_norm(adj)
        if not _is_symmetric(norm):
            raise NotImplementedError("the multi-GPU backward relies on a symmetric normalised adjacency")
        self.plan = make_dense_plan(norm.storage.rowcount(), P)
        rel = relabel(norm, self.plan)
        rowptr, col, val = row_shard(rel, self.plan, self.rank)
        self.n_p = self.plan.counts[self.rank]
        self.n_global = adj.size(0)
        self._shard = csr_graph_from(rowptr, col, val, self.n_p, self.n_global)
        frp, fcol, fval = rel.csr()
        self.Gfull = csr_graph_from(frp, fcol, fval, self.n_global, self.n_global)
        super().__init__(adj, dims, _prebuilt_graph=self._shard, _rows_alloc=self.plan.block, **kw)
        dev = self.device
        N, L = self.n_global, self.L
        self.row0 = self.plan.offsets[self.rank]
        self.rowmap = self.plan.perm[self.row0:self.row0 + self.n_p].to(torch.int32).to(dev)
        self.rowmap_full = self.plan.perm.to(torch.int32).to(dev)
        self.col_mode = {k: (k % (4 * P) == 0) for k in set(dims)}
        n_par = self.params.numel()
        self.n_par = n_par
        n_red = self._grads_buf.numel()
        B = self.plan.block
        kin = dims[0]
        specs = []
        if self.agg_first and self.col_mode[kin]:
            specs += [("loc", "AXc", (N, kin // P)), ("ex", "AX_R", (B, kin))]
        for l in range(L):
            k = dims[l + 1]
            if l == 0 and self.agg_first:
                continue
            if self.col_mode[k]:
                specs += [("ex", f"Hc{l}", (N, k // P)), ("loc", f"Yc{l}", (N, k // P))]
                if l < L - 1:
                    specs += [("loc", f"Ac{l}", (N, k // P)), ("ex", f"A_R{l}", (B, k)), ("ex", f"dAc{l}", (N, k // P)),
                              ("loc", f"dYc{l}", (N, k // P))]
                else:
                    specs += [("ex", f"Y_R{l}", (B, k)), ("ex", f"dYc{l}", (N, k // P))]
                specs += [("loc", f"dHc{l}", (N, k // P)), ("ex", f"dH_R{l}", (B, k))]
            else:
                specs += [("ex", f"Hfull{l}", (N, k)), ("ex", f"dYfull{l}", (N, k))]
        for k in sorted(set(dims[1:-1])):
            specs.append(("ex", f"stat_all{k}", (P, 2, k)))
        specs += [("ex", "grads_all", (P, n_red))]
        need = sum((4 * _numel(shape) + 255) // 256 * 256 for kind, _, shape in specs if kind == "ex") + 4096
        if exchange == "peer":
            self.ex = PeerExchange(self.plan, self.rank, need, group)
        elif exchange == "null":
            self.ex = NullExchange(self.plan, self.rank, group)
        else:
            self.ex = TorchExchange(self.plan, self.rank, group)
        self.c: Dict[str, torch.Tensor] = {}
        for kind, name, shape in specs:
            t = self.ex.buffer(name, shape, dev) if kind == "ex" else torch.zeros(*shape, device=dev)
            if name.endswith("_R") or "_R" in name:
                t = t[:self.n_p]
            self.c[name] = t
        kmax = max(dims[1:])
        self.stat_loc = torch.zeros(2 * kmax, device=dev)
        self.stat_all = {k: self.c[f"stat_all{k}"] for k in set(dims[1:-1])}
        self.grads_all = self.c["grads_all"]
        self.bn_c = {l: torch.empty(4, dims[l + 1] // P, device=dev) for l in range(L - 1) if self.col_mode[dims[l + 1]]}
        slots_full = ops.stat_slots(self.Gfull)
        self.stat_part_c = {l: torch.empty(slots_full, 2, dims[l + 1] // P, device=dev)
                            for l in range(L - 1) if self.col_mode[dims[l + 1]]}
        self.rs_full = ops.rows_slots(N)
        self._layer_in: List[Optional[torch.Tensor]] = [None] * L
        self.n_train_global = 0

    def shard_inputs(self, x, y, train_idx, teacher_logits=None):
        plan, dev = self.plan, self.device
        perm = plan.perm.to(dev)
        r0, r1 = plan.rows_of(self.rank)
        mine = perm[r0:r1]
        x = x.to(dev)
        kin, P = self.dims[0], self.world
        if self.agg_first and self.col_mode[kin]:
            kc = kin // P
            x_in = x[:, self.rank * kc:(self.rank + 1) * kc][perm].contiguous()
        elif self.agg_first:
            x_in = x[perm].contiguous()
        else:
            x_in = x[mine].contiguous()
        y_loc = y.to(dev)[mine].contiguous()
        t_loc = None if teacher_logits is None else teacher_logits.to(dev)[mine].contiguous()
        new_train = plan.inv.to(dev)[train_idx.to(dev)]
        loc = new_train[(new_train >= r0) & (new_train < r1)] - r0
        self.n_train_global = int(train_idx.numel())
        return x_in, y_loc, torch.sort(loc).values.contiguous(), t_loc

    def input_bytes(self, x_in, y_loc, tr_loc, t_loc) -> int:
        return sum(t.numel() * t.element_size() for t in (x_in, y_loc, tr_loc, t_loc) if t is not None)

    def gather_rows(self, local: torch.Tensor) -> torch.Tensor:
        full = torch.empty(self.n_global, local.shape[1], device=local.device)
        dist.all_to_all_single(full, local.contiguous().repeat(self.world, 1), output_split_sizes=self.plan.counts,
# ... 258 lines not shown
```

### efficient-gnns_b200/lib.py

```python
from __future__ import annotations

import ctypes as C
import os
from pathlib import Path

import torch

PKG_DIR = Path(__file__).resolve().parent
LIB_PATH = PKG_DIR / "libb200gnn.so"

OK = 0
REDUCE_SUM = 0
REDUCE_MEAN = 1

_i32p = C.c_void_p
_f32p = C.c_void_p
_ptr = C.c_void_p
_i64 = C.c_int64
_i32 = C.c_int32
_int = C.c_int
_f32 = C.c_float
_u64 = C.c_uint64

SIGNATURES = {
    "b200gnn_abi_version": (_int, []),
    "b200gnn_error_string": (C.c_char_p, [_int]),
    "b200gnn_last_cuda_error": (C.c_char_p, []),
    "b200gnn_launch_count": (_i64, []),
    "b200gnn_reset_launch_count": (None, []),
    "b200gnn_csr_chunk_count": (_i64, [_i64, _i64, _i32, _i32]),
    "b200gnn_csr_chunk_plan": (_int, [_i32p, _i64, _i64, _i32, _i32, _i32p, _ptr]),
    "b200gnn_csr_hub_count": (_int, [_i32p, _i64, _i32, _i32, _i32p, _ptr]),
    "b200gnn_csr_hub_fill": (_int, [_i32p, _i64, _i32, _i32, _i32p, _i32p, _i64, _ptr]),
    "b200gnn_spmm_stat_slots": (_i64, [_i64, _i64]),
    "b200gnn_spmm_set_variant": (None, [_int]),
    "b200gnn_spmm_csr_f32": (_int, [_i32p, _i32p, _f32p, _f32p, _i64, _f32p, _i64, _i64, _i64, _i64, _int,
                                    _f32p, _f32p, _i32p, _i64, _i32, _i32, _i32p, _i32p, _i64, _i64, _f32p, _ptr]),
    "b200gnn_spmm_csr_scatter_f32": (_int, [_i32p, _i32p, _f32p, _f32p, _i64, _ptr, _ptr, _i32, _i64, _i64, _i64, _i64, _i64, _int,
                                            _f32p, _i32p, _i64, _i32, _i32, _i32p, _i32p, _i64, _i64, _f32p, _ptr]),
    "b200gnn_rows_slots": (_i64, [_i64]),
    "b200gnn_col_stats_f32": (_int, [_f32p, _i64, _i64, _f32p, _i64, _ptr]),
    "b200gnn_col_sum_f32": (_int, [_f32p, _i64, _i64, _f32p, _f32p, _i64, _ptr]),
    "b200gnn_bn_finalize_f32": (_int, [_f32p, _i64, _i64, _i64, _f32p, _f32p, _f32, _f32, _f32p, _f32p,
                                       _f32p, _f32p, _f32p, _f32p, _ptr]),
    "b200gnn_affine_relu_dropout_f32": (_int, [_f32p, _f32p, _i64, _i64, _f32p, _f32p, _int, _f32, _u64, _u64,
                                               _i32p, _u64, _u64, _ptr]),
    "b200gnn_affine_relu_dropout_mapped_f32": (_int, [_f32p, _f32p, _i64, _i64, _f32p, _f32p, _int, _f32, _u64, _u64,
                                                      _i32p, _u64, _i32p, _u64, _i64, _i64, _ptr]),
    "b200gnn_affine_relu_dropout_scatter_f32": (_int, [_f32p, _f32p, _i64, _i64, _f32p, _f32p, _int, _f32, _u64, _u64,
                                                       _i32p, _u64, _i32p, _u64, _i64, _i64, _ptr, _ptr, _i32, _i64, _ptr]),
    "b200gnn_dropout_mask_u8": (_int, [_ptr, _i64, _i64, _f32, _u64, _u64, _ptr]),
    "b200gnn_relu_dropout_bwd_f32": (_int, [_f32p, _f32p, _f32p, _i64, _i64, _f32, _ptr]),
    "b200gnn_bn_act_bwd_f32": (_int, [_f32p, _f32p, _f32p, _f32p, _f32p, _f32p, _i64, _i64, _f32, _f32p, _f32p,
                                      _f32p, _f32p, _f32p, _i64, _f32p, _ptr]),
    "b200gnn_bn_act_bwd_reduce_f32": (_int, [_f32p, _f32p, _f32p, _f32p, _f32p, _i64, _i64, _f32, _f32p, _i64, _ptr]),
    "b200gnn_bn_act_bwd_apply_f32": (_int, [_f32p, _f32p, _f32p, _f32p, _f32p, _f32p, _f32p, _i64, _i64, _i64, _i64, _f32,
                                            _f32p, _f32p, _f32p, _f32p, _f32p, _i64, _f32p, _ptr]),
    "b200gnn_partial_reduce_f32": (_int, [_f32p, _i64, _i64, _f32p, _ptr]),
    "b200gnn_adam_step_f32": (_int, [_f32p, _f32p, _f32p, _f32p, _i64, _f32, _f32, _f32, _f32, _i32p, _ptr]),
    "b200gnn_kd_partials": (_i64, [_i64]),
    "b200gnn_kd_loss_fwd_bwd_f32": (_int, [_f32p, _i64, _ptr, _i64, _ptr, _f32p, _i64, _i64, _f32, _f32, _i64, _f32p,
                                           _i64, _f32p, _f32p, _ptr]),
    "b200gnn_split_tf32_f32": (_int, [_f32p, _i64, _i64, _int, _f32p, _f32p, _ptr]),
    "b200gnn_gemm_tf32x3_f32": (_int, [_f32p, _i64, _f32p, _f32p, _i64, _f32p, _i64, _i64, _i64, _i64, _f32p, _ptr]),
    "b200gnn_random_walk_i64": (_int, [_i32p, _i32p, _i64, _ptr, _i64, _i32, _u64, _u64, _ptr, _ptr]),
    "b200gnn_saint_subgraph_count_i64": (_int, [_i32p, _i32p, _ptr, _i64, _i32p, _ptr, _ptr]),
    "b200gnn_saint_subgraph_fill_i64": (_int, [_i32p, _i32p, _ptr, _ptr, _i64, _i32p, _ptr, _ptr, _ptr, _ptr, _ptr]),
    "b200gnn_gemm_stat_slots": (_i64, [_i64, _i64]),
    "b200gnn_gemm_set_bnbwd_variant": (None, [_int]),
    "b200gnn_gemm_tf32x3_stats_f32": (_int, [_f32p, _i64, _f32p, _f32p, _i64, _f32p, _i64, _i64, _i64, _i64, _f32p, _int, _f32p, _i64,
                                             _ptr]),
    "b200gnn_gemm_tf32x3_bnbwd_f32": (_int, [_f32p, _i64, _f32p, _f32p, _i64, _f32p, _i64, _i64, _i64, _i64, _int,
                                             _f32p, _f32p, _f32p, _f32p, _f32, _f32p, _i64, _ptr]),
    "b200gnn_gemm_tf32x3_acc_f32": (_int, [_f32p, _i64, _f32p, _f32p, _i64, _f32p, _i64, _i64, _i64, _i64, _ptr]),
    "b200gnn_gemm_tf32x3_scatter_f32": (_int, [_f32p, _i64, _f32p, _f32p, _i64, _ptr, _i32, _i64, _i64, _i64, _i64, _f32p, _ptr]),
    "b200gnn_gemm_tf32x3_bcast_f32": (_int, [_f32p, _i64, _f32p, _f32p, _i64, _ptr, _i32, _i64, _i64, _i64, _i64, _i64, _f32p, _ptr]),
    "b200gnn_wgrad_workspace_floats": (_i64, [_i64, _i64]),
    "b200gnn_gemm_wgrad_tf32x3_f32": (_int, [_f32p, _i64, _f32p, _i64, _f32p, _i64, _i64, _i64, _f32p, _ptr]),
    "b200gnn_row_normalize_fwd_f32": (_int, [_f32p, _i64, _i64, _f32, _f32, _f32p, _f32p, _ptr]),
    "b200gnn_row_normalize_bwd_f32": (_int, [_f32p, _f32p, _f32p, _i64, _i64, _f32, _f32, _f32p, _int, _ptr]),
    "b200gnn_reduce_slots": (_i64, [_i64]),
    "b200gnn_mse_fwd_bwd_f32": (_int, [_f32p, _f32p, _i64, _f32, _f32p, _f32p, _f32p, _ptr]),
    "b200gnn_bce_logits_fwd_bwd_f32": (_int, [_f32p, _f32p, _int, _i64, _f32, _f32p, _f32p, _f32p, _ptr]),
    "b200gnn_row_sqnorm_f32": (_int, [_f32p, _i64, _i64, _f32p, _ptr]),
    "b200gnn_row_sqnorm_bwd_f32": (_int, [_f32p, _f32p, _i64, _i64, _f32p, _ptr]),
    "b200gnn_nce_rows_f32": (_int, [_f32p, _i64, _f32p, _f32p, _ptr]),
    "b200gnn_nce_rows_chunk_f32": (_int, [_f32p, _i64, _i64, _i64, _i64, _f32p, _ptr]),
    "b200gnn_nce_finish_f32": (_int, [_f32p, _i64, _f32p, _ptr]),
    "b200gnn_transpose_f32": (_int, [_f32p, _i64, _i64, _f32p, _ptr]),
    "b200gnn_gsp_pair_f32": (_int, [_f32p, _f32p, _f32p, _f32p, _i64, _int, _f32p, _f32p, _f32p, _ptr]),
    "b200gnn_row_axpy_f32": (_int, [_f32p, _f32p, _i64, _i64, _f32, _f32p, _ptr]),
    "b200gnn_edge_sim_f32": (_int, [_f32p, _i64, _i32p, _i32p, _i64, _int, _f32p, _ptr]),
    "b200gnn_lsp_partials": (_i64, [_i64]),
    "b200gnn_lsp_segment_f32": (_int, [_f32p, _f32p, _i32p, _i64, _i64, _int, _f32p, _f32p, _f32p, _ptr]),
    "b200gnn_edge_sim_bwd_f32": (_int, [_f32p, _i64, _i32p, _i32p, _i64, _int, _f32p, _f32p, _f32p, _ptr]),
    "b200gnn_lsp_bwd_values_f32": (_int, [_f32p, _i64, _i32p, _i32p, _i64, _int, _f32p, _f32p, _i32p, _i32p, _i32p, _i32p, _i64,
                                          _f32p, _f32p, _ptr]),
    "b200gnn_gat_edge_softmax_f32": (_int, [_i32p, _i32p, _f32p, _f32p, _i64, _i64, _f32, _f32, _f32p, _ptr, _ptr]),
    "b200gnn_gat_aggregate_f32": (_int, [_i32p, _i32p, _i32p, _f32p, _f32p, _i64, _f32p, _i64, _i64, _i64, _i64, _i32p, _i64,
                                         _i32, _i32, _i32p, _i32p, _i64, _i64, _f32p, _ptr]),
    "b200gnn_gat_bwd_rows_f32": (_int, [_i32p, _i32p, _f32p, _f32p, _i64, _f32p, _i64, _f32p, _f32p, _i64, _i64, _i64, _f32,
                                        _f32p, _f32p, _i32p, _i64, _i32, _i32, _i32p, _i32p, _i64, _i64, _f32p, _f32p, _ptr]),
    "b200gnn_segment_sum_heads_f32": (_int, [_i32p, _i32p, _f32p, _i64, _i64, _f32p, _ptr]),
    "b200gnn_graph_sort_workspace_bytes": (_i64, [_i64]),
    "b200gnn_graph_argsort_i64": (_int, [_ptr, _ptr, _i64, _i64, _i64, _i32p, _ptr, _ptr]),
    "b200gnn_graph_coalesce_i64": (_int, [_ptr, _ptr, _i64, _i64, _i64, _ptr, _ptr, _i32p, _ptr, _ptr, _ptr, _ptr]),
    "b200gnn_typed_gather_f32": (_int, [_ptr, _ptr, _i32, _ptr, _ptr, _i64, _i64, _f32p, _i64, _i32p, _ptr]),
    "b200gnn_typed_scatter_f32": (_int, [_f32p, _i64, _ptr, _ptr, _ptr, _i64, _i64, _ptr, _ptr, _i32, _ptr]),
    "b200gnn_embedding_adam_f32": (_int, [_f32p, _i64, _ptr, _ptr, _ptr, _i64, _i64, _f32p, _f32p, _f32p, _i64, _i64, _i32p,
                                          _f32, _f32, _f32, _f32, _i32p, _ptr]),
    "b200gnn_arena_alloc": (_int, [_i64, C.POINTER(C.c_void_p)]),
    "b200gnn_arena_free": (_int, [_ptr]),
    "b200gnn_ipc_get_handle": (_int, [_ptr, _ptr]),
    "b200gnn_ipc_open_handle": (_int, [_ptr, C.POINTER(C.c_void_p)]),
    "b200gnn_ipc_close_handle": (_int, [_ptr]),
    "b200gnn_peer_copy2d_f32": (_int, [_ptr, _i32, _i64, _ptr]),
    "b200gnn_peer_barrier": (_int, [_ptr, _i32, _i32, _ptr, _ptr, _ptr]),
    "b200gnn_peer_exchange_f32": (_int, [_ptr, _i32, _i64, _ptr, _i32, _i32, _ptr, _ptr, _ptr, _ptr]),
}


class Copy2D(C.Structure):
    _fields_ = [("dst", C.c_void_p), ("src", C.c_void_p), ("ld_dst", C.c_int64), ("ld_src", C.c_int64), ("rows", C.c_int64)]

_lib = None


class B200GnnError(RuntimeError):
    pass


def load() -> C.CDLL:
    global _lib
    if _lib is not None:
        return _lib
    if not LIB_PATH.exists():
        raise B200GnnError(
            f"{LIB_PATH} is missing: build it with `python -c 'import __graft_entry__ as g; g.build()'` "
            "(nvcc, sm_90a). There is no CPU or PyTorch fallback for the b200gnn operators.")
    lib = C.CDLL(str(LIB_PATH))
    for name, (res, args) in SIGNATURES.items():
        fn = getattr(lib, name)
        fn.restype = res
        fn.argtypes = args
    if lib.b200gnn_abi_version() != 2:
        raise B200GnnError("libb200gnn.so ABI version mismatch; rebuild")
    _lib = lib
    report = os.environ.get("B200GNN_LAUNCH_REPORT")
    if report:
        import atexit
        atexit.register(lambda: Path(report).write_text(str(int(lib.b200gnn_launch_count()))))
    return lib


def check(rc: int, what: str) -> None:
    if rc != OK:
        lib = load()
        msg = lib.b200gnn_error_string(rc).decode()
        if rc == -3:
            msg += ": " + lib.b200gnn_last_cuda_error().decode()
        raise B200GnnError(f"{what} failed: {msg}")
# ... 27 lines not shown
```

### efficient-gnns_b200/ops.py

```python
from __future__ import annotations

from typing import Optional, Tuple

import torch

from . import lib
from .sparse import CsrGraph, SparseTensor

_REDUCE = {"sum": lib.REDUCE_SUM, "add": lib.REDUCE_SUM, "mean": lib.REDUCE_MEAN}


def set_spmm_variant(variant: int) -> None:
    lib.load().b200gnn_spmm_set_variant(int(variant))


def stat_slots(g: CsrGraph) -> int:
    return int(lib.load().b200gnn_spmm_stat_slots(g.n_chunks, g.n_hub))


def spmm_csr(g: CsrGraph, x: torch.Tensor, reduce: str = "sum", bias: Optional[torch.Tensor] = None,
             out: Optional[torch.Tensor] = None, stat_partial: Optional[torch.Tensor] = None) -> torch.Tensor:
    if reduce not in _REDUCE:
        raise ValueError(f"reduce={reduce!r}: the engine implements sum/add/mean (what the reference path uses)")
    if x.dim() != 2:
# ... 80 lines not shown


def rows_slots(n_rows: int) -> int:
    return int(lib.load().b200gnn_rows_slots(n_rows))


def col_stats(y: torch.Tensor, partial: Optional[torch.Tensor] = None) -> torch.Tensor:
    n, K = y.shape
    slots = rows_slots(n)
    if partial is None:
        partial = torch.empty(slots, 2, K, dtype=torch.float32, device=y.device)
    lib.check(lib.load().b200gnn_col_stats_f32(_f32(y, "y"), n, K, _f32(partial, "partial"), slots, lib.stream_ptr()),
              "col_stats_f32")
    return partial


def col_sum(y: torch.Tensor, out: Optional[torch.Tensor] = None, partial: Optional[torch.Tensor] = None) -> torch.Tensor:
    n, K = y.shape
    slots = rows_slots(n)
    if out is None:
        out = torch.empty(K, dtype=torch.float32, device=y.device)
    if partial is None:
        partial = torch.empty(slots, 2, K, dtype=torch.float32, device=y.device)
    lib.check(lib.load().b200gnn_col_sum_f32(_f32(y, "y"), n, K, _f32(out, "out"), _f32(partial, "partial"), slots,
                                             lib.stream_ptr()), "col_sum_f32")
    return out


def bn_finalize(partial: torch.Tensor, n_rows: int, gamma, beta, eps: float = 1e-5, momentum: float = 0.1,
                running_mean=None, running_var=None, out: Optional[torch.Tensor] = None) -> torch.Tensor:
    slots, _, K = partial.shape
    if out is None:
        out = torch.empty(4, K, dtype=torch.float32, device=partial.device)
    lib.check(lib.load().b200gnn_bn_finalize_f32(
        _f32(partial, "partial"), slots, K, n_rows, _f32(gamma, "gamma"), _f32(beta, "beta"), eps, momentum,
        _f32(running_mean, "running_mean"), _f32(running_var, "running_var"),
        out[0].data_ptr(), out[1].data_ptr(), out[2].data_ptr(), out[3].data_ptr(), lib.stream_ptr()), "bn_finalize_f32")
    return out


def affine_relu_dropout(y: torch.Tensor, scale=None, shift=None, relu: bool = True, p: float = 0.0, seed: int = 0,
                        offset: int = 0, out: Optional[torch.Tensor] = None, step_dev: Optional[torch.Tensor] = None,
                        step_mul: int = 0, row_offset: int = 0) -> torch.Tensor:
    n, K = y.shape
    if out is None:
        out = torch.empty_like(y)
    lib.check(lib.load().b200gnn_affine_relu_dropout_f32(
        _f32(y, "y"), _f32(out, "out"), n, K, _f32(scale, "scale"), _f32(shift, "shift"), int(relu), p, seed, offset,
        lib.dptr(step_dev, torch.int32, "step_dev"), step_mul, row_offset, lib.stream_ptr()), "affine_relu_dropout_f32")
    return out


def affine_relu_dropout_mapped(y: torch.Tensor, scale=None, shift=None, relu: bool = True, p: float = 0.0, seed: int = 0,
                               offset: int = 0, out: Optional[torch.Tensor] = None, step_dev: Optional[torch.Tensor] = None,
                               step_mul: int = 0, rowmap: Optional[torch.Tensor] = None, row_offset: int = 0,
                               k_global: Optional[int] = None, col_offset: int = 0) -> torch.Tensor:
    n, K = y.shape
    if out is None:
        out = torch.empty_like(y)
    lib.check(lib.load().b200gnn_affine_relu_dropout_mapped_f32(
        _f32(y, "y"), _f32(out, "out"), n, K, _f32(scale, "scale"), _f32(shift, "shift"), int(relu), p, seed, offset,
        lib.dptr(step_dev, torch.int32, "step_dev"), step_mul, lib.dptr(rowmap, torch.int32, "rowmap"), row_offset,
        K if k_global is None else k_global, col_offset, lib.stream_ptr()), "affine_relu_dropout_mapped_f32")
    return out


def affine_relu_dropout_scatter(y: torch.Tensor, scale, shift, relu: bool, p: float, seed: int, offset: int, out: torch.Tensor,
                                step_dev, step_mul: int, rowmap, k_global: int, col_offset: int, dst_ptrs, row_off,
                                ld_dst: int) -> torch.Tensor:
    n, K = y.shape
    lib.check(lib.load().b200gnn_affine_relu_dropout_scatter_f32(
        _f32(y, "y"), _f32(out, "out"), n, K, _f32(scale, "scale"), _f32(shift, "shift"), int(relu), p, seed, offset,
        lib.dptr(step_dev, torch.int32, "step_dev"), step_mul, lib.dptr(rowmap, torch.int32, "rowmap"), 0, k_global, col_offset,
        _host_ptr_array(dst_ptrs), _host_i32_array(row_off), len(dst_ptrs), int(ld_dst), lib.stream_ptr()),
        "affine_relu_dropout_scatter_f32")
    return out


def dropout_mask(n_rows: int, K: int, p: float, seed: int, offset: int, device="cuda") -> torch.Tensor:
    mask = torch.empty(n_rows, K, dtype=torch.uint8, device=device)
    lib.check(lib.load().b200gnn_dropout_mask_u8(mask.data_ptr(), n_rows, K, p, seed, offset, lib.stream_ptr()),
              "dropout_mask_u8")
    return mask


def bn_act_bwd(d_out, x_out, y, mean, invstd, gamma, p: float, d_y=None, d_gamma=None, d_beta=None, d_bias=None,
               partial=None, coef=None, want_dbias: bool = True):
    n, K = y.shape
    dev = y.device
    slots = rows_slots(n)
    d_y = torch.empty_like(y) if d_y is None else d_y
    d_gamma = torch.empty(K, device=dev) if d_gamma is None else d_gamma
    d_beta = torch.empty(K, device=dev) if d_beta is None else d_beta
    if want_dbias and d_bias is None:
        d_bias = torch.empty(K, device=dev)
    partial = torch.empty(slots, 2, K, device=dev) if partial is None else partial
    coef = torch.empty(3, K, device=dev) if coef is None else coef
    lib.check(lib.load().b200gnn_bn_act_bwd_f32(
        _f32(d_out, "d_out"), _f32(x_out, "x_out"), _f32(y, "y"), _f32(mean, "mean"), _f32(invstd, "invstd"),
        _f32(gamma, "gamma"), n, K, p, _f32(d_y, "d_y"), _f32(d_gamma, "d_gamma"), _f32(d_beta, "d_beta"),
        _f32(d_bias, "d_bias") if want_dbias else None, _f32(partial, "partial"), slots, _f32(coef, "coef"),
        lib.stream_ptr()), "bn_act_bwd_f32")
    return d_y, d_gamma, d_beta, d_bias


def adam_step(params, grads, exp_avg, exp_avg_sq, step: torch.Tensor, lr: float, betas=(0.9, 0.999), eps: float = 1e-8):
    lib.check(lib.load().b200gnn_adam_step_f32(
        _f32(params, "params"), _f32(grads, "grads"), _f32(exp_avg, "exp_avg"), _f32(exp_avg_sq, "exp_avg_sq"),
        params.numel(), lr, betas[0], betas[1], eps, lib.dptr(step, torch.int32, "step"), lib.stream_ptr()),
        "adam_step_f32")


def kd_loss_fwd_bwd(logits, labels, train_idx, teacher_logits=None, alpha: float = 0.9, T: float = 4.0,
                    d_logits=None, loss_out=None, partial=None, n_norm: int = 0):
    N, C = logits.shape
    n_train = train_idx.numel() if train_idx is not None else N
    L = lib.load()
    if d_logits is None:
        d_logits = torch.zeros_like(logits)
    if loss_out is None:
        loss_out = torch.empty(3, dtype=torch.float32, device=logits.device)
    if partial is None:
        partial = torch.empty(2 * int(L.b200gnn_kd_partials(max(n_train, 1))), dtype=torch.float32, device=logits.device)
    lib.check(L.b200gnn_kd_loss_fwd_bwd_f32(
        _f32(logits, "logits"), logits.stride(0), lib.dptr(train_idx, torch.int64, "train_idx"), n_train,
        lib.dptr(labels, torch.int64, "labels"), _f32(teacher_logits, "teacher_logits"),
        teacher_logits.stride(0) if teacher_logits is not None else 0, C, alpha, T, n_norm, _f32(d_logits, "d_logits"),
        d_logits.stride(0), _f32(loss_out, "loss_out"), _f32(partial, "partial"), lib.stream_ptr()), "kd_loss_fwd_bwd_f32")
    return loss_out, d_logits


def split_tf32(w: torch.Tensor, transpose: bool = False, hi: Optional[torch.Tensor] = None,
               lo: Optional[torch.Tensor] = None) -> Tuple[torch.Tensor, torch.Tensor]:
    rows, cols = w.shape
    shape = (cols, rows) if transpose else (rows, cols)
    hi = torch.empty(shape, dtype=torch.float32, device=w.device) if hi is None else hi
    lo = torch.empty(shape, dtype=torch.float32, device=w.device) if lo is None else lo
    lib.check(lib.load().b200gnn_split_tf32_f32(_f32(w, "w"), rows, cols, int(transpose), _f32(hi, "hi"), _f32(lo, "lo"),
                                                lib.stream_ptr()), "split_tf32_f32")
    return hi, lo


def gemm_tf32x3(a: torch.Tensor, b_hi: torch.Tensor, b_lo: torch.Tensor, bias: Optional[torch.Tensor] = None,
                out: Optional[torch.Tensor] = None, accumulate: bool = False) -> torch.Tensor:
    M, K = a.shape
    N = b_hi.shape[0]
    assert b_hi.shape == b_lo.shape and b_hi.shape[1] == K
    if out is None:
        assert not accumulate
        out = torch.empty(M, N, dtype=torch.float32, device=a.device)
    L = lib.load()
    if accumulate:
        assert bias is None
        lib.check(L.b200gnn_gemm_tf32x3_acc_f32(_f32(a, "a"), a.stride(0), _f32(b_hi, "b_hi"), _f32(b_lo, "b_lo"),
                                                b_hi.stride(0), _f32(out, "out"), out.stride(0), M, N, K, lib.stream_ptr()),
                  "gemm_tf32x3_acc_f32")
        return out
    lib.check(L.b200gnn_gemm_tf32x3_f32(_f32(a, "a"), a.stride(0), _f32(b_hi, "b_hi"), _f32(b_lo, "b_lo"),
                                        b_hi.stride(0), _f32(out, "out"), out.stride(0), M, N, K,
                                        _f32(bias, "bias"), lib.stream_ptr()), "gemm_tf32x3_f32")
    return out


def gemm_stat_slots(m: int, n: int) -> int:
    return int(lib.load().b200gnn_gemm_stat_slots(m, n))


def gemm_stats_supported(n: int) -> bool:
    return n % 32 == 0 and 48 < n <= 256


def gemm_tf32x3_stats(a: torch.Tensor, b_hi: torch.Tensor, b_lo: torch.Tensor, bias: Optional[torch.Tensor], out: torch.Tensor,
                      partial: torch.Tensor, accumulate: bool = False) -> torch.Tensor:
    M, K = a.shape
    N = b_hi.shape[0]
    lib.check(lib.load().b200gnn_gemm_tf32x3_stats_f32(_f32(a, "a"), a.stride(0), _f32(b_hi, "b_hi"), _f32(b_lo, "b_lo"),
                                                       b_hi.stride(0), _f32(out, "out"), out.stride(0), M, N, K, _f32(bias, "bias"),
                                                       int(accumulate), _f32(partial, "partial"), partial.shape[0], lib.stream_ptr()),
              "gemm_tf32x3_stats_f32")
    return out


def gemm_tf32x3_bnbwd(a: torch.Tensor, b_hi: torch.Tensor, b_lo: torch.Tensor, out: torch.Tensor, x_out: torch.Tensor,
                      y: torch.Tensor, mean: torch.Tensor, invstd: torch.Tensor, p: float, partial: torch.Tensor,
                      accumulate: bool = False) -> torch.Tensor:
    M, K = a.shape
    N = b_hi.shape[0]
    assert out.shape == x_out.shape == y.shape and out.stride(0) == x_out.stride(0) == y.stride(0)
    lib.check(lib.load().b200gnn_gemm_tf32x3_bnbwd_f32(_f32(a, "a"), a.stride(0), _f32(b_hi, "b_hi"), _f32(b_lo, "b_lo"),
                                                       b_hi.stride(0), _f32(out, "out"), out.stride(0), M, N, K, int(accumulate),
                                                       _f32(x_out, "x_out"), _f32(y, "y"), _f32(mean, "mean"),
                                                       _f32(invstd, "invstd"), float(p), _f32(partial, "partial"),
                                                       partial.shape[0], lib.stream_ptr()), "gemm_tf32x3_bnbwd_f32")
    return out


def gemm_tf32x3_scatter(a: torch.Tensor, b_hi: torch.Tensor, b_lo: torch.Tensor, dst_ptrs, row_off: int,
                        bias: Optional[torch.Tensor] = None) -> None:
    import ctypes as C
    M, K = a.shape
    N = b_hi.shape[0]
    world = len(dst_ptrs)
    arr = (C.c_void_p * world)(*[C.c_void_p(int(p)) for p in dst_ptrs])
    lib.check(lib.load().b200gnn_gemm_tf32x3_scatter_f32(_f32(a, "a"), a.stride(0), _f32(b_hi, "b_hi"), _f32(b_lo, "b_lo"),
                                                         b_hi.stride(0), arr, world, int(row_off), M, N, K, _f32(bias, "bias"),
                                                         lib.stream_ptr()), "gemm_tf32x3_scatter_f32")


def gemm_tf32x3_bcast(a: torch.Tensor, b_hi: torch.Tensor, b_lo: torch.Tensor, dst_ptrs, row_off: int, ldc: int,
                      bias: Optional[torch.Tensor] = None) -> None:
    M, K = a.shape
    N = b_hi.shape[0]
    lib.check(lib.load().b200gnn_gemm_tf32x3_bcast_f32(_f32(a, "a"), a.stride(0), _f32(b_hi, "b_hi"), _f32(b_lo, "b_lo"),
                                                       b_hi.stride(0), _host_ptr_array(dst_ptrs), len(dst_ptrs), int(row_off), int(ldc),
                                                       M, N, K, _f32(bias, "bias"), lib.stream_ptr()), "gemm_tf32x3_bcast_f32")


def wgrad_supported(k_in: int, n_out: int) -> bool:
    return k_in in (128, 256) and n_out % 4 == 0 and 0 < n_out <= 256


def wgrad_workspace_floats(k_in: int, n_out: int) -> int:
    return int(lib.load().b200gnn_wgrad_workspace_floats(k_in, n_out))


def gemm_wgrad_tf32x3(x: torch.Tensor, g: torch.Tensor, out: Optional[torch.Tensor] = None,
                      workspace: Optional[torch.Tensor] = None, wide: bool = False) -> torch.Tensor:
    nn_, k_in = x.shape
    n_out = g.shape[1]
    assert g.shape[0] == nn_
    if not wide and not wgrad_supported(k_in, n_out):
        raise lib.B200GnnError(f"gemm_wgrad_tf32x3: Kin={k_in}, Nout={n_out} is outside the 128/256-row tilings "
                               "(pass wide=True for the padded ones)")
    L = lib.load()
    if out is None:
        out = torch.empty(k_in, n_out, dtype=torch.float32, device=x.device)
    if workspace is None:
        n_ws = int(L.b200gnn_wgrad_workspace_floats(k_in, n_out))
        if n_ws < 0:
            lib.check(n_ws, "wgrad_workspace_floats")
        workspace = torch.empty(n_ws, dtype=torch.float32, device=x.device)
    lib.check(L.b200gnn_gemm_wgrad_tf32x3_f32(_f32(x, "x"), x.stride(0), _f32(g, "g"), g.stride(0), _f32(out, "out"), nn_,
                                              k_in, n_out, _f32(workspace, "workspace"), lib.stream_ptr()),
              "gemm_wgrad_tf32x3_f32")
    return out


def partial_reduce(partial: torch.Tensor, out: Optional[torch.Tensor] = None) -> torch.Tensor:
    slots = partial.shape[0]
    k2 = partial.numel() // slots
    if out is None:
        out = torch.empty(partial.shape[1:], dtype=torch.float32, device=partial.device)
    lib.check(lib.load().b200gnn_partial_reduce_f32(_f32(partial, "partial"), slots, k2, _f32(out, "out"), lib.stream_ptr()),
              "partial_reduce_f32")
    return out


def bn_act_bwd_reduce(d_out, x_out, y, mean, invstd, p: float, partial: torch.Tensor) -> torch.Tensor:
    n, K = y.shape
    lib.check(lib.load().b200gnn_bn_act_bwd_reduce_f32(_f32(d_out, "d_out"), _f32(x_out, "x_out"), _f32(y, "y"),
                                                       _f32(mean, "mean"), _f32(invstd, "invstd"), n, K, p,
                                                       _f32(partial, "partial"), partial.shape[0], lib.stream_ptr()),
              "bn_act_bwd_reduce_f32")
    return partial


def bn_act_bwd_apply(d_out, x_out, y, mean, invstd, gamma, sums, n_norm: int, p: float, d_y, d_gamma, d_beta, d_bias,
                     partial, coef):
    n, K = y.shape
    sum_slots = sums.numel() // (2 * K)
    lib.check(lib.load().b200gnn_bn_act_bwd_apply_f32(
        _f32(d_out, "d_out"), _f32(x_out, "x_out"), _f32(y, "y"), _f32(mean, "mean"), _f32(invstd, "invstd"),
        _f32(gamma, "gamma"), _f32(sums, "sums"), sum_slots, n_norm, n, K, p, _f32(d_y, "d_y"), _f32(d_gamma, "d_gamma"),
        _f32(d_beta, "d_beta"), _f32(d_bias, "d_bias"), _f32(partial, "partial"), partial.shape[0], _f32(coef, "coef"),
        lib.stream_ptr()), "bn_act_bwd_apply_f32")


def relu_dropout_bwd(d_out: torch.Tensor, x_out: torch.Tensor, p: float, out: Optional[torch.Tensor] = None) -> torch.Tensor:
    n, K = x_out.shape
    assert d_out.shape == x_out.shape and d_out.is_contiguous() and x_out.is_contiguous()
    out = torch.empty_like(x_out) if out is None else out
    lib.check(lib.load().b200gnn_relu_dropout_bwd_f32(_f32(d_out, "d_out"), _f32(x_out, "x_out"), _f32(out, "out"), n, K, float(p),
                                                      lib.stream_ptr()), "relu_dropout_bwd_f32")
    return out


def _table_arrays(tables: dict, n_tables: int):
    import ctypes as C
    ptrs = (C.c_void_p * n_tables)()
    rows = (C.c_int64 * n_tables)()
    for k, t in tables.items():
        ptrs[k], rows[k] = t.data_ptr(), t.shape[0]
    return ptrs, rows


def typed_gather(tables: dict, n_tables: int, node_type: torch.Tensor, local_idx: torch.Tensor, out: torch.Tensor) -> torch.Tensor:
    ptrs, rows = _table_arrays(tables, n_tables)
    err = torch.zeros(1, dtype=torch.int32, device=out.device)
    lib.check(lib.load().b200gnn_typed_gather_f32(ptrs, rows, n_tables, lib.dptr(node_type, torch.int64, "node_type"),
                                                  lib.dptr(local_idx, torch.int64, "local_idx"), out.shape[0], out.shape[1],
                                                  _f32(out, "out"), out.stride(0), err.data_ptr(), lib.stream_ptr()),
              "typed_gather_f32")
    return out


def typed_scatter(d_out: torch.Tensor, node_type: torch.Tensor, local_idx: torch.Tensor, order: torch.Tensor, grads: dict,
                  n_tables: int) -> None:
    ptrs, rows = _table_arrays(grads, n_tables)
    lib.check(lib.load().b200gnn_typed_scatter_f32(_f32(d_out, "d_out"), d_out.stride(0), lib.dptr(node_type, torch.int64, "node_type"),
                                                   lib.dptr(local_idx, torch.int64, "local_idx"), lib.dptr(order, torch.int64, "order"),
                                                   d_out.shape[0], d_out.shape[1], ptrs, rows, n_tables, lib.stream_ptr()),
              "typed_scatter_f32")


def embedding_adam(d_out: torch.Tensor, node_type: torch.Tensor, local_idx: torch.Tensor, order: torch.Tensor, table_type: int,
                   table: torch.Tensor, exp_avg: torch.Tensor, exp_avg_sq: torch.Tensor, head: torch.Tensor, step: torch.Tensor,
                   lr: float, betas=(0.9, 0.999), eps: float = 1e-8) -> None:
    rows, F_ = table.shape
    assert exp_avg.shape == table.shape == exp_avg_sq.shape and head.numel() >= rows and d_out.shape[1] == F_
    lib.check(lib.load().b200gnn_embedding_adam_f32(
        _f32(d_out, "d_out"), d_out.stride(0), lib.dptr(node_type, torch.int64, "node_type"),
        lib.dptr(local_idx, torch.int64, "local_idx"), lib.dptr(order, torch.int64, "order"), d_out.shape[0], int(table_type),
        _f32(table, "table"), _f32(exp_avg, "exp_avg"), _f32(exp_avg_sq, "exp_avg_sq"), rows, F_,
        lib.dptr(head, torch.int32, "head"), lr, betas[0], betas[1], eps, lib.dptr(step, torch.int32, "step"), lib.stream_ptr()),
        "embedding_adam_f32")
```

### include/b200gnn.h

```cpp
#ifndef B200GNN_H_
#define B200GNN_H_

#include <stdint.h>

#ifdef __cplusplus
extern "C" {
#endif

#define B200GNN_OK 0
#define B200GNN_ERR_BAD_ARG (-1)
#define B200GNN_ERR_UNSUPPORTED (-2)
#define B200GNN_ERR_CUDA (-3)

#define B200GNN_REDUCE_SUM 0
#define B200GNN_REDUCE_MEAN 1

#define B200GNN_ABI_VERSION 2

int b200gnn_abi_version(void);
const char* b200gnn_error_string(int code);
const char* b200gnn_last_cuda_error(void);
int64_t b200gnn_launch_count(void);
void b200gnn_reset_launch_count(void);

int64_t b200gnn_csr_chunk_count(int64_t n_rows, int64_t nnz, int32_t chunk_nnz,
                                int32_t row_cost);
int b200gnn_csr_chunk_plan(const int32_t* rowptr, int64_t n_rows, int64_t nnz,
                           int32_t chunk_nnz, int32_t row_cost,
                           int32_t* chunk_rowptr, void* stream);

int b200gnn_csr_hub_count(const int32_t* rowptr, int64_t n_rows,
                          int32_t hub_threshold, int32_t seg_len,
                          int32_t* counts_out, void* stream);
int b200gnn_csr_hub_fill(const int32_t* rowptr, int64_t n_rows,
                         int32_t hub_threshold, int32_t seg_len,
                         int32_t* hub_rows, int32_t* hub_segptr,
                         int64_t n_hub, void* stream);

int64_t b200gnn_spmm_stat_slots(int64_t n_chunks, int64_t n_hub);
void b200gnn_spmm_set_variant(int variant);
int b200gnn_spmm_csr_f32(const int32_t* rowptr, const int32_t* col,
                         const float* val, const float* X, int64_t ldx,
                         float* Y, int64_t ldy, int64_t n_rows, int64_t n_src,
                         int64_t K, int reduce, const float* bias,
                         float* stat_partial, const int32_t* chunk_rowptr,
                         int64_t n_chunks, int32_t hub_threshold,
                         int32_t seg_len, const int32_t* hub_rows,
                         const int32_t* hub_segptr, int64_t n_hub,
                         int64_t n_seg, float* hub_workspace, void* stream);
int b200gnn_spmm_csr_scatter_f32(const int32_t* rowptr, const int32_t* col, const float* val, const float* X,
                                 int64_t ldx, float* const* Y_ptrs, const int32_t* row_off, int32_t world,
                                 int64_t ldy_dst, int64_t col_dst, int64_t n_rows, int64_t n_src, int64_t K,
                                 int reduce, const float* bias, const int32_t* chunk_rowptr, int64_t n_chunks,
                                 int32_t hub_threshold, int32_t seg_len, const int32_t* hub_rows,
                                 const int32_t* hub_segptr, int64_t n_hub, int64_t n_seg,
                                 float* hub_workspace, void* stream);

int64_t b200gnn_rows_slots(int64_t n_rows);
int b200gnn_col_stats_f32(const float* Y, int64_t n_rows, int64_t K,
                          float* partial, int64_t slots, void* stream);
int b200gnn_col_sum_f32(const float* Y, int64_t n_rows, int64_t K, float* out,
                        float* partial, int64_t slots, void* stream);
int b200gnn_bn_finalize_f32(const float* partial, int64_t slots, int64_t K,
                            int64_t n_rows, const float* gamma,
                            const float* beta, float eps, float momentum,
                            float* running_mean, float* running_var,
                            float* mean_out, float* invstd_out,
                            float* scale_out, float* shift_out, void* stream);
int b200gnn_affine_relu_dropout_f32(const float* Y, float* out, int64_t n_rows,
                                    int64_t K, const float* scale,
                                    const float* shift, int relu, float p,
                                    uint64_t seed, uint64_t offset,
                                    const int32_t* step_dev, uint64_t step_mul,
                                    uint64_t row_offset, void* stream);
int b200gnn_affine_relu_dropout_mapped_f32(const float* Y, float* out, int64_t n_rows, int64_t K,
                                           const float* scale, const float* shift, int relu, float p,
                                           uint64_t seed, uint64_t offset, const int32_t* step_dev,
                                           uint64_t step_mul, const int32_t* rowmap, uint64_t row_offset,
                                           int64_t K_global, int64_t col_offset, void* stream);
int b200gnn_affine_relu_dropout_scatter_f32(const float* Y, float* out, int64_t n_rows, int64_t K,
                                            const float* scale, const float* shift, int relu, float p,
                                            uint64_t seed, uint64_t offset, const int32_t* step_dev,
                                            uint64_t step_mul, const int32_t* rowmap, uint64_t row_offset,
                                            int64_t K_global, int64_t col_offset, float* const* dst_ptrs,
                                            const int32_t* row_off, int32_t world, int64_t ld_dst, void* stream);
int b200gnn_dropout_mask_u8(uint8_t* mask, int64_t n_rows, int64_t K, float p,
                            uint64_t seed, uint64_t offset, void* stream);
int b200gnn_relu_dropout_bwd_f32(const float* dOut, const float* Xout, float* dY,
                                 int64_t n_rows, int64_t K, float p, void* stream);
int b200gnn_bn_act_bwd_f32(const float* dOut, const float* Xout, const float* Y,
                           const float* mean, const float* invstd,
                           const float* gamma, int64_t n_rows, int64_t K,
                           float p, float* dY, float* dgamma, float* dbeta,
                           float* dbias, float* partial, int64_t slots,
                           float* coef, void* stream);
int b200gnn_bn_act_bwd_reduce_f32(const float* dOut, const float* Xout,
                                  const float* Y, const float* mean,
                                  const float* invstd, int64_t n_rows,
                                  int64_t K, float p, float* partial,
                                  int64_t slots, void* stream);
int b200gnn_bn_act_bwd_apply_f32(const float* dOut, const float* Xout,
                                 const float* Y, const float* mean,
                                 const float* invstd, const float* gamma,
                                 const float* sums, int64_t sum_slots,
                                 int64_t n_norm, int64_t n_rows, int64_t K,
                                 float p, float* dY, float* dgamma,
                                 float* dbeta, float* dbias, float* partial,
                                 int64_t slots, float* coef, void* stream);
int b200gnn_partial_reduce_f32(const float* partial, int64_t slots, int64_t K2,
                               float* out, void* stream);
int b200gnn_adam_step_f32(float* params, const float* grads, float* exp_avg,
                          float* exp_avg_sq, int64_t n, float lr, float beta1,
                          float beta2, float eps, int32_t* step, void* stream);

int64_t b200gnn_kd_partials(int64_t n_train);
int b200gnn_kd_loss_fwd_bwd_f32(const float* logits, int64_t ld,
                                const int64_t* train_idx, int64_t n_train,
                                const int64_t* labels,
                                const float* teacher_logits, int64_t ldt,
                                int64_t C, float alpha, float T,
                                int64_t n_norm, float* dlogits, int64_t ldd,
                                float* loss_out, float* partial, void* stream);

int b200gnn_split_tf32_f32(const float* W, int64_t rows, int64_t cols,
                           int transpose, float* hi, float* lo, void* stream);
int b200gnn_gemm_tf32x3_f32(const float* A, int64_t lda, const float* B_hi,
                            const float* B_lo, int64_t ldb, float* C,
                            int64_t ldc, int64_t M, int64_t N, int64_t K,
                            const float* bias, void* stream);
int b200gnn_gemm_tf32x3_acc_f32(const float* A, int64_t lda, const float* B_hi, const float* B_lo,
                                int64_t ldb, float* C, int64_t ldc, int64_t M, int64_t N, int64_t K,
                                void* stream);
int64_t b200gnn_gemm_stat_slots(int64_t M, int64_t N);
void b200gnn_gemm_set_bnbwd_variant(int v);
int b200gnn_gemm_tf32x3_stats_f32(const float* A, int64_t lda, const float* B_hi, const float* B_lo, int64_t ldb,
                                  float* C, int64_t ldc, int64_t M, int64_t N, int64_t K, const float* bias,
                                  int accumulate, float* partial, int64_t slots, void* stream);
int b200gnn_gemm_tf32x3_bnbwd_f32(const float* A, int64_t lda, const float* B_hi, const float* B_lo, int64_t ldb,
                                  float* C, int64_t ldc, int64_t M, int64_t N, int64_t K, int accumulate,
                                  const float* Xout, const float* Y, const float* mean, const float* invstd, float p_drop,
                                  float* partial, int64_t slots, void* stream);
int b200gnn_gemm_tf32x3_scatter_f32(const float* A, int64_t lda, const float* B_hi, const float* B_lo,
                                    int64_t ldb, float* const* C_ptrs, int32_t world, int64_t row_off,
                                    int64_t M, int64_t N, int64_t K, const float* bias, void* stream);
int b200gnn_gemm_tf32x3_bcast_f32(const float* A, int64_t lda, const float* B_hi, const float* B_lo,
                                  int64_t ldb, float* const* C_ptrs, int32_t world, int64_t row_off, int64_t ldc,
                                  int64_t M, int64_t N, int64_t K, const float* bias, void* stream);

int64_t b200gnn_wgrad_workspace_floats(int64_t Kin, int64_t Nout);
int b200gnn_gemm_wgrad_tf32x3_f32(const float* X, int64_t ldx, const float* G,
                                  int64_t ldg, float* dW, int64_t Nn,
                                  int64_t Kin, int64_t Nout, float* workspace,
                                  void* stream);

int b200gnn_row_normalize_fwd_f32(const float* x, int64_t n, int64_t F, float eps,
                                  float scale, float* out, float* norm_out,
                                  void* stream);
int b200gnn_row_normalize_bwd_f32(const float* out, const float* norm,
                                  const float* d_out, int64_t n, int64_t F,
                                  float eps, float scale, float* d_x,
                                  int accumulate, void* stream);
int64_t b200gnn_reduce_slots(int64_t n);
int b200gnn_mse_fwd_bwd_f32(const float* a, const float* b, int64_t n,
                            float grad_weight, float* d_a, float* loss_out,
                            float* partial, void* stream);
int b200gnn_bce_logits_fwd_bwd_f32(const float* z, const float* target,
                                   int target_is_logits, int64_t n,
                                   float grad_weight, float* d_z, float* loss_out,
                                   float* partial, void* stream);
int b200gnn_row_sqnorm_f32(const float* x, int64_t n, int64_t F, float* out, void* stream);
int b200gnn_row_sqnorm_bwd_f32(const float* x, const float* d_out, int64_t n,
                               int64_t F, float* d_x, void* stream);
int b200gnn_nce_rows_f32(float* Z, int64_t S, float* loss_out, float* partial, void* stream);
int b200gnn_nce_rows_chunk_f32(float* Z, int64_t ldz, int64_t n_rows, int64_t S, int64_t row_offset,
                               float* partial, void* stream);
int b200gnn_nce_finish_f32(const float* partial, int64_t S, float* loss_out, void* stream);
int b200gnn_transpose_f32(const float* in, int64_t rows, int64_t cols, float* out, void* stream);
int b200gnn_gsp_pair_f32(float* Gs, const float* Gt, const float* ns, const float* nt,
                         int64_t S, int kernel, float* rowcoef, float* loss_out,
                         float* partial, void* stream);
int b200gnn_row_axpy_f32(const float* x, const float* coef, int64_t n, int64_t F,
                         float alpha, float* y, void* stream);

int b200gnn_edge_sim_f32(const float* feat, int64_t F, const int32_t* src,
                         const int32_t* dst, int64_t E, int kernel, float* sim,
                         void* stream);
int64_t b200gnn_lsp_partials(int64_t n_seg);
int b200gnn_lsp_segment_f32(const float* sim_s, const float* sim_t,
                            const int32_t* rowptr, int64_t n_seg, int64_t E,
                            int criterion, float* g, float* loss_out,
                            float* partial, void* stream);
int b200gnn_edge_sim_bwd_f32(const float* feat, int64_t F, const int32_t* src,
                             const int32_t* dst, int64_t E, int kernel,
                             const float* sim, const float* g, float* dfeat,
                             void* stream);
int b200gnn_lsp_bwd_values_f32(const float* feat, int64_t F, const int32_t* src, const int32_t* dst,
                               int64_t E, int kernel, const float* sim, const float* g,
                               const int32_t* pos_dst, const int32_t* pos_src,
                               const int32_t* comb_rowptr, const int32_t* diag_pos, int64_t n_nodes,
                               float* val, float* selfc, void* stream);

int b200gnn_gat_edge_softmax_f32(const int32_t* rowptr, const int32_t* col,
                                 const float* el, const float* er, int64_t n_rows,
                                 int64_t H, float negative_slope, float softmax_eps,
                                 float* a, const uint8_t* edge_keep, void* stream);
int b200gnn_gat_aggregate_f32(const int32_t* rowptr, const int32_t* col,
                              const int32_t* eidx, const float* a, const float* ft,
                              int64_t ldf, float* out, int64_t ldo, int64_t n_rows,
                              int64_t H, int64_t D, const int32_t* chunk_rowptr,
                              int64_t n_chunks, int32_t hub_threshold, int32_t seg_len,
                              const int32_t* hub_rows, const int32_t* hub_segptr,
                              int64_t n_hub, int64_t n_seg, float* hub_workspace,
                              void* stream);
int b200gnn_gat_bwd_rows_f32(const int32_t* rowptr, const int32_t* col, const float* a,
                             const float* ft, int64_t ldf, const float* dout,
                             int64_t ldd, const float* el, const float* er,
                             int64_t n_rows, int64_t H, int64_t D,
                             float negative_slope, float* dpre, float* der,
                             const int32_t* chunk_rowptr, int64_t n_chunks,
                             int32_t hub_threshold, int32_t seg_len,
                             const int32_t* hub_rows, const int32_t* hub_segptr,
                             int64_t n_hub, int64_t n_seg, float* hub_workspace,
                             const float* attn_scale, void* stream);
int b200gnn_segment_sum_heads_f32(const int32_t* rowptr, const int32_t* eidx,
                                  const float* vals, int64_t n_rows, int64_t H,
                                  float* out, void* stream);

typedef struct b200gnn_copy2d {
  float* dst;
  const float* src;
  int64_t ld_dst;
  int64_t ld_src;
  int64_t rows;
} b200gnn_copy2d;
int b200gnn_arena_alloc(int64_t bytes, void** out);
int b200gnn_arena_free(void* ptr);
// ... 44 lines not shown
```

Baseline: 3.204 billion.

## Fuse BN-affine, ReLU and bit-packed dropout into GEMM operand loads

Adds a bit-packed dropout mask (one bit per element, generated for all layers in one launch) and GEMM variants that apply the BN affine, ReLU and dropout to the A operand as it is loaded. The backward BN GEMM and the weight-grad GEMM recompute the activation from Y and the bits, so the post-activation tensor no longer has to be materialized or reread. The aim is to cut HBM traffic from writing and reading the activated hidden tensor and the byte-per-element mask. The cost is extra per-fragment ALU work and scattered bit-word loads inside the GEMM mainloop, plus more template variants to maintain.

New measurement: 3.368 billion (median of 6 runs). +5.1%, better.

```diff
diff --git a/efficient-gnns_b200/csrc/dense_rows.cu b/efficient-gnns_b200/csrc/dense_rows.cu
--- a/efficient-gnns_b200/csrc/dense_rows.cu
+++ b/efficient-gnns_b200/csrc/dense_rows.cu
@@ -238,6 +238,54 @@
       m = keep24(philox4x32(seed, offset, (uint64_t)i), p);
     }
     reinterpret_cast<uchar4*>(mask)[i] = m;
+  }
+}
+
+__global__ void __launch_bounds__(256) dropout_bits_kernel(uint32_t* __restrict__ bits, int n_layers, int64_t n_rows, int nvec_row,
+                                                           int words, float p, int p16, uint32_t thr16, uint64_t seed,
+                                                           uint64_t offset, const int32_t* __restrict__ step_dev,
+                                                           uint64_t step_mul) {
+  if (step_dev) offset += (uint64_t)(*step_dev) * step_mul;
+  const int64_t per_layer = n_rows * words;
+  for (int64_t t = (int64_t)blockIdx.x * blockDim.x + threadIdx.x; t < per_layer * n_layers; t += (int64_t)gridDim.x * blockDim.x) {
+    const int layer = (int)(t / per_layer);
+    const int64_t e = t - layer * per_layer, row = e / words;
+    const int w = (int)(e - row * words);
+    const uint64_t off = offset + (uint64_t)layer;
+    uint32_t out = 0u;
+    uint64_t blk = ~0ull;
+    uint4 r = make_uint4(0u, 0u, 0u, 0u);
+#pragma unroll
+    for (int j = 0; j < 8; ++j) {
+      const int cv = 8 * w + j;
+      if (cv >= nvec_row) break;
+      const uint64_t g = (uint64_t)row * nvec_row + cv;
+      uchar4 m;
+      if (p16) {
+        if ((g >> 1) != blk) { blk = g >> 1; r = philox4x32(seed, off, blk); }
+        m = keep16((g & 1) ? r.z : r.x, (g & 1) ? r.w : r.y, thr16);
+      } else {
+        m = keep24(philox4x32(seed, off, g), p);
+      }
+      out |= ((uint32_t)m.x | ((uint32_t)m.y << 1) | ((uint32_t)m.z << 2) | ((uint32_t)m.w << 3)) << (4 * j);
+    }
+    bits[t] = out;
+  }
+}
+
+__global__ void __launch_bounds__(256) affine_relu_bits_kernel(const float* __restrict__ Y, const uint32_t* __restrict__ bits,
+                                                               const float* __restrict__ scale, const float* __restrict__ shift,
+                                                               float* __restrict__ out, int64_t n_vec, int nvec_row, int words,
+                                                               float p) {
+  const float inv_keep = p > 0.f ? 1.f / (1.f - p) : 1.f;
+  for (int64_t i = (int64_t)blockIdx.x * blockDim.x + threadIdx.x; i < n_vec; i += (int64_t)gridDim.x * blockDim.x) {
+    const int64_t row = i / nvec_row;
+    const int cv = (int)(i - row * nvec_row);
+    float4 y = affine_relu4(ld4(Y + 4 * i), scale, shift, cv, 1);
+    const uint32_t b = bits[row * words + (cv >> 3)] >> (4 * (cv & 7));
+    y.x = (b & 1u) ? y.x * inv_keep : 0.f; y.y = (b & 2u) ? y.y * inv_keep : 0.f;
+    y.z = (b & 4u) ? y.z * inv_keep : 0.f; y.w = (b & 8u) ? y.w * inv_keep : 0.f;
+    st4(out + 4 * i, y);
   }
 }
 
@@ -491,6 +539,30 @@
   return check_launch();
 }
 
+extern "C" int b200gnn_dropout_bits_u32(uint32_t* bits, int64_t n_layers, int64_t n_rows, int64_t K, float p, uint64_t seed,
+                                        uint64_t offset, const int32_t* step_dev, uint64_t step_mul, void* stream) {
+  if (!rows_ok(n_rows, K) || !bits || n_layers < 1 || p < 0.f || p >= 1.f) return B200GNN_ERR_BAD_ARG;
+  if (n_rows == 0) return B200GNN_OK;
+  const int words = (int)((K + 31) / 32);
+  uint32_t thr16 = 0;
+  const int p16 = dropout_p16(p, thr16) ? 1 : 0;
+  dropout_bits_kernel<<<grid_for(n_layers * n_rows * words, 256 * 2), 256, 0, (cudaStream_t)stream>>>(
+      bits, (int)n_layers, n_rows, (int)(K / 4), words, p, p16, thr16, seed, offset, step_dev, step_mul);
+  return check_launch();
+}
+
+extern "C" int b200gnn_affine_relu_bits_f32(const float* Y, const uint32_t* bits, const float* scale, const float* shift,
+                                            float p, float* out, int64_t n_rows, int64_t K, void* stream) {
+  if (!rows_ok(n_rows, K) || !Y || !bits || !scale || !shift || !out || p < 0.f || p >= 1.f || !aligned_to(Y, 16) ||
+      !aligned_to(out, 16) || !aligned_to(scale, 16) || !aligned_to(shift, 16))
+    return B200GNN_ERR_BAD_ARG;
+  if (n_rows == 0) return B200GNN_OK;
+  const int64_t n_vec = n_rows * (K / 4);
+  affine_relu_bits_kernel<<<grid_for(n_vec, 256 * 4), 256, 0, (cudaStream_t)stream>>>(Y, bits, scale, shift, out, n_vec,
+                                                                                     (int)(K / 4), (int)((K + 31) / 32), p);
+  return check_launch();
+}
+
 extern "C" int b200gnn_relu_dropout_bwd_f32(const float* dOut, const float* Xout, float* dY, int64_t n_rows, int64_t K,
                                             float p, void* stream) {
   if (!rows_ok(n_rows, K) || p < 0.f || p >= 1.f) return B200GNN_ERR_BAD_ARG;
diff --git a/efficient-gnns_b200/csrc/gemm_tf32x3.cu b/efficient-gnns_b200/csrc/gemm_tf32x3.cu
--- a/efficient-gnns_b200/csrc/gemm_tf32x3.cu
+++ b/efficient-gnns_b200/csrc/gemm_tf32x3.cu
@@ -64,8 +64,13 @@
   const float* bn_mean;
   const float* bn_invstd;
   float inv_keep;
+  const float* act_scale;
+  const float* act_shift;
+  const uint32_t* act_bits;
+  int32_t act_words;
 };
 
+template <bool ACT>
 __device__ __forceinline__ void load_bn_chunk(const Params& p, int m0, int col, int q, int lane, float4 (&x)[4], float4 (&y)[4]) {
   if (col + 32 > p.N) return;
   const int sub = lane >> 3, cq = (lane & 7) * 4;
@@ -74,13 +79,26 @@
     const int grow = m0 + q * 16 + it * 4 + sub;
     if (grow < p.M) {
       const size_t o = (size_t)grow * p.ldc + col + cq;
-      x[it] = __ldg(reinterpret_cast<const float4*>(p.bn_x + o));
+      if (!ACT) x[it] = __ldg(reinterpret_cast<const float4*>(p.bn_x + o));
       y[it] = __ldg(reinterpret_cast<const float4*>(p.bn_y + o));
     }
   }
 }
 
-template <class C, int STAT, bool PEER>
+__device__ __forceinline__ void load_bits_chunk(const Params& p, int m0, int col, int q, int lane, uint32_t (&w)[4]) {
+  const int sub = lane >> 3;
+#pragma unroll
+  for (int it = 0; it < 4; ++it) {
+    const int grow = m0 + q * 16 + it * 4 + sub;
+    w[it] = grow < p.M ? __ldg(p.act_bits + (size_t)grow * p.act_words + (col >> 5)) : 0u;
+  }
+}
+
+__device__ __forceinline__ uint32_t act1(uint32_t y, float sc, float sh, uint32_t keep, float inv_keep) {
+  return keep ? __float_as_uint(fmaxf(fmaf(__uint_as_float(y), sc, sh), 0.f) * inv_keep) : 0u;
+}
+
+template <class C, int STAT, bool PEER, bool ACT = false>
 __global__ void __launch_bounds__(THREADS, 1)
 gemm_tf32x3_kernel(const __grid_constant__ CUtensorMap tmA, const __grid_constant__ CUtensorMap tmBhi,
                    const __grid_constant__ CUtensorMap tmBlo, const __grid_constant__ CUtensorMap tmX,
@@ -149,12 +167,30 @@
     if (lane == 0)
       for (int g = 0; g < 2 && g < n_mine; ++g) {
         const int tt = blockIdx.x + (g / NCHUNK) * gridDim.x, cc = g % NCHUNK;
-        mbar_expect_tx(&xyb[g], XY_SLOT_BYTES);
-        tma_load_2d(&tmX, &xyb[g], xy + g * XY_SLOT_BYTES, (tt % num_n) * BN + cc * 32, (tt / num_n) * BM + q * XY_ROWS);
+        mbar_expect_tx(&xyb[g], ACT ? XY_SLOT_BYTES / 2 : XY_SLOT_BYTES);
+        if (!ACT)
+          tma_load_2d(&tmX, &xyb[g], xy + g * XY_SLOT_BYTES, (tt % num_n) * BN + cc * 32, (tt / num_n) * BM + q * XY_ROWS);
         tma_load_2d(&tmY, &xyb[g], xy + g * XY_SLOT_BYTES + XY_SLOT_BYTES / 2, (tt % num_n) * BN + cc * 32,
                     (tt / num_n) * BM + q * XY_ROWS);
       }
   }
+  const float* act_ss = stat_smem;
+  if (ACT && !STAT) {
+    for (int c = threadIdx.x - 128; c < num_kb * BK; c += 256) {
+      const int w = c & 31;
+      const float2 v = c < p.K ? make_float2(__ldg(p.act_scale + c), __ldg(p.act_shift + c)) : make_float2(0.f, 0.f);
+      *reinterpret_cast<float2*>(stat_smem + (c >> 5) * 64 + (w & 3) * 16 + (w >> 3) * 4 + ((w >> 2) & 1) * 2) = v;
+    }
+    named_sync(1, 256);
+  }
+  const int arow = q * 16 + (lane >> 2);
+  auto act_words = [&](int tile, int kb, uint32_t (&w)[2]) {
+    const int r = (tile / num_n) * BM + arow;
+    w[0] = r < p.M ? __ldg(p.act_bits + (size_t)r * p.act_words + kb) : 0u;
+    w[1] = r + 8 < p.M ? __ldg(p.act_bits + (size_t)(r + 8) * p.act_words + kb) : 0u;
+  };
+  uint32_t wnext[2] = {0u, 0u};
+  if (ACT && !STAT && blockIdx.x < num_tiles) act_words(blockIdx.x, 0, wnext);
   float acc[ACC], sum[ACC];
   uint32_t ah0[BK / 8][4], al0[BK / 8][4], ah1[BK / 8][4], al1[BK / 8][4];
   const uint32_t frag = a_frag_offset(q * 16 + (lane >> 2), lane);
@@ -166,9 +202,26 @@
     for (int i = 0; i < ACC; ++i) sum[i] = acc[i] = 0.f;
     int prev = 0;
     auto stage = [&](int kb, uint32_t (&h)[BK / 8][4], uint32_t (&l)[BK / 8][4]) {
+      uint32_t wcur[2];
+      if (ACT && !STAT) {
+        wcur[0] = wnext[0] >> (lane & 3); wcur[1] = wnext[1] >> (lane & 3);
+        if (kb + 1 < num_kb) act_words(tile, kb + 1, wnext);
+        else if (tile + (int)gridDim.x < num_tiles) act_words(tile + gridDim.x, 0, wnext);
+      }
       mbar_wait(&full[s], ph);
       uint8_t* st = smem + s * STAGE_BYTES;
       load_a(smem_u32(st) + frag, h);
+      if (ACT && !STAT) {
+        const float4* ss = reinterpret_cast<const float4*>(act_ss + kb * 64 + (lane & 3) * 16);
+#pragma unroll
+        for (int k = 0; k < BK / 8; ++k) {
+          const float4 t = ss[k];
+#pragma unroll
+          for (int i = 0; i < 4; ++i)
+            h[k][i] = act1(h[k][i], (i >> 1) ? t.z : t.x, (i >> 1) ? t.w : t.y, (wcur[i & 1] >> (8 * k + 4 * (i >> 1))) & 1u,
+                           p.inv_keep);
+        }
+      }
 #pragma unroll
       for (int k = 0; k < BK / 8; ++k)
 #pragma unroll
@@ -210,7 +263,7 @@
     for (int c = 0; c < NCHUNK; ++c, ++g_chunk) {
       const int col0 = n0 + c * 32;
       float4 xr[4], yr[4];
-      if (STAT == 2) load_bn_chunk(p, m0, col0, q, lane, xr, yr);
+      if (STAT == 2) load_bn_chunk<ACT>(p, m0, col0, q, lane, xr, yr);
 #pragma unroll
       for (int jj = 0; jj < 4; ++jj) {
         const int j = c * 4 + jj;
@@ -229,10 +282,16 @@
         float4 b4 = make_float4(0.f, 0.f, 0.f, 0.f);
         if (p.bias) b4 = make_float4(__ldg(p.bias + col0 + cq), __ldg(p.bias + col0 + cq + 1), __ldg(p.bias + col0 + cq + 2),
                                      __ldg(p.bias + col0 + cq + 3));
-        float4 s4 = make_float4(0.f, 0.f, 0.f, 0.f), q4 = s4, mu4 = s4, is4 = s4;
+        float4 s4 = make_float4(0.f, 0.f, 0.f, 0.f), q4 = s4, mu4 = s4, is4 = s4, sc4 = s4, sh4 = s4;
         if (BNB) {
           mu4 = __ldg(reinterpret_cast<const float4*>(p.bn_mean + col0 + cq));
           is4 = __ldg(reinterpret_cast<const float4*>(p.bn_invstd + col0 + cq));
+        }
+        uint32_t wb[4];
+        if (BNB && ACT) {
+          sc4 = __ldg(reinterpret_cast<const float4*>(p.act_scale + col0 + cq));
+          sh4 = __ldg(reinterpret_cast<const float4*>(p.act_shift + col0 + cq));
+          load_bits_chunk(p, m0, col0, q, lane, wb);
         }
 #pragma unroll
         for (int it = 0; it < 4; ++it) {
@@ -255,10 +314,19 @@
             if (STAT == 1) {
               vstat(s4, q4, v);
             } else if (BNB) {
-              const float4 x = XYTMA ? *reinterpret_cast<const float4*>(xs + rr * 32 + cq) : xr[it];
+              float4 x = make_float4(0.f, 0.f, 0.f, 0.f);
+              if (!ACT) x = XYTMA ? *reinterpret_cast<const float4*>(xs + rr * 32 + cq) : xr[it];
               const float4 y = XYTMA ? *reinterpret_cast<const float4*>(ys + rr * 32 + cq) : yr[it];
-              v.x = x.x > 0.f ? v.x * p.inv_keep : 0.f; v.y = x.y > 0.f ? v.y * p.inv_keep : 0.f;
-              v.z = x.z > 0.f ? v.z * p.inv_keep : 0.f; v.w = x.w > 0.f ? v.w * p.inv_keep : 0.f;
+              if (ACT) {
+                const uint32_t b = wb[it] >> cq;
+                v.x = (b & 1u) && fmaf(y.x, sc4.x, sh4.x) > 0.f ? v.x * p.inv_keep : 0.f;
+                v.y = (b & 2u) && fmaf(y.y, sc4.y, sh4.y) > 0.f ? v.y * p.inv_keep : 0.f;
+                v.z = (b & 4u) && fmaf(y.z, sc4.z, sh4.z) > 0.f ? v.z * p.inv_keep : 0.f;
+                v.w = (b & 8u) && fmaf(y.w, sc4.w, sh4.w) > 0.f ? v.w * p.inv_keep : 0.f;
+              } else {
+                v.x = x.x > 0.f ? v.x * p.inv_keep : 0.f; v.y = x.y > 0.f ? v.y * p.inv_keep : 0.f;
+                v.z = x.z > 0.f ? v.z * p.inv_keep : 0.f; v.w = x.w > 0.f ? v.w * p.inv_keep : 0.f;
+              }
               s4.x += v.x; s4.y += v.y; s4.z += v.z; s4.w += v.w;
               q4.x = fmaf(v.x, (y.x - mu4.x) * is4.x, q4.x); q4.y = fmaf(v.y, (y.y - mu4.y) * is4.y, q4.y);
               q4.z = fmaf(v.z, (y.z - mu4.z) * is4.z, q4.z); q4.w = fmaf(v.w, (y.w - mu4.w) * is4.w, q4.w);
@@ -287,8 +355,8 @@
         if (XYTMA && lane == 0 && g_chunk + 2 < n_mine) {
           const int g = g_chunk + 2, tt = blockIdx.x + (g / NCHUNK) * gridDim.x, cc = g % NCHUNK;
           uint8_t* dst = xy + (g & 1) * XY_SLOT_BYTES;
-          mbar_expect_tx(&xyb[g & 1], XY_SLOT_BYTES);
-          tma_load_2d(&tmX, &xyb[g & 1], dst, (tt % num_n) * BN + cc * 32, (tt / num_n) * BM + q * XY_ROWS);
+          mbar_expect_tx(&xyb[g & 1], ACT ? XY_SLOT_BYTES / 2 : XY_SLOT_BYTES);
+          if (!ACT) tma_load_2d(&tmX, &xyb[g & 1], dst, (tt % num_n) * BN + cc * 32, (tt / num_n) * BM + q * XY_ROWS);
           tma_load_2d(&tmY, &xyb[g & 1], dst + XY_SLOT_BYTES / 2, (tt % num_n) * BN + cc * 32, (tt / num_n) * BM + q * XY_ROWS);
         }
       } else {
@@ -342,7 +410,7 @@
             CU_TENSOR_MAP_L2_PROMOTION_L2_256B, CU_TENSOR_MAP_FLOAT_OOB_FILL_NONE) == CUDA_SUCCESS;
 }
 
-template <class C, int STAT = 0, bool PEER = false>
+template <class C, int STAT = 0, bool PEER = false, bool ACT = false>
 static int launch(const float* A, int64_t lda, const float* B_hi, const float* B_lo, int64_t ldb, const Params& p,
                   cudaStream_t stream) {
   CUtensorMap tA, tBh, tBl, tX, tY;
@@ -350,20 +418,21 @@
       !make_map(&tBl, B_lo, p.N, p.K, ldb, C::BN))
     return B200GNN_ERR_UNSUPPORTED;
   tX = tA; tY = tA;
-  if (STAT == 3 && (!make_map(&tX, p.bn_x, p.M, p.N, p.ldc, XY_ROWS, false) || !make_map(&tY, p.bn_y, p.M, p.N, p.ldc, XY_ROWS, false)))
+  if (STAT == 3 && ((!ACT && !make_map(&tX, p.bn_x, p.M, p.N, p.ldc, XY_ROWS, false)) ||
+                    !make_map(&tY, p.bn_y, p.M, p.N, p.ldc, XY_ROWS, false)))
     return B200GNN_ERR_UNSUPPORTED;
   int dev = 0, sms = 132;
   cudaGetDevice(&dev);
   static bool attr_set[64] = {};
   if (dev >= 0 && dev < 64 && !attr_set[dev]) {
-    cudaError_t e = cudaFuncSetAttribute(gemm_tf32x3_kernel<C, STAT, PEER>, cudaFuncAttributeMaxDynamicSharedMemorySize, C::SMEM_BYTES);
+    cudaError_t e = cudaFuncSetAttribute(gemm_tf32x3_kernel<C, STAT, PEER, ACT>, cudaFuncAttributeMaxDynamicSharedMemorySize, C::SMEM_BYTES);
     if (e != cudaSuccess) { set_cuda_error(e); return B200GNN_ERR_CUDA; }
     attr_set[dev] = true;
   }
   const int tiles = ((p.M + BM - 1) / BM) * ((p.N + C::BN - 1) / C::BN);
   cudaDeviceGetAttribute(&sms, cudaDevAttrMultiProcessorCount, dev);
   const int grid = tiles < sms ? tiles : sms;
-  gemm_tf32x3_kernel<C, STAT, PEER><<<grid, THREADS, C::SMEM_BYTES, stream>>>(tA, tBh, tBl, tX, tY, p);
+  gemm_tf32x3_kernel<C, STAT, PEER, ACT><<<grid, THREADS, C::SMEM_BYTES, stream>>>(tA, tBh, tBl, tX, tY, p);
   return check_launch();
 }
 
@@ -387,7 +456,7 @@
 
 static int gemm_dispatch(const float* A, int64_t lda, const float* B_hi, const float* B_lo, int64_t ldb, float* C, int64_t ldc,
                          int64_t M, int64_t N, int64_t K, const float* bias, int accumulate, void* stream,
-                         const gemm::Params* st = nullptr) {
+                         const gemm::Params* st = nullptr, const gemm::Params* act = nullptr) {
   if (!A || !B_hi || !B_lo || !C || M <= 0 || N <= 0 || K <= 0 || lda < K || ldb < K || ldc < N ||
       M >= INT32_MAX || N >= INT32_MAX || K >= INT32_MAX)
     return B200GNN_ERR_BAD_ARG;
@@ -396,13 +465,27 @@
   gemm::Params p{};
   p.C = C; p.bias = bias; p.ldc = ldc; p.M = (int32_t)M; p.N = (int32_t)N; p.K = (int32_t)K; p.accumulate = accumulate ? 1 : 0;
   p.n_peer = 0; p.kc = 0; p.row_off = 0; p.bcast = 0;
+  if (act) {
+    if (!act->act_scale || !act->act_shift || !act->act_bits || !aligned_to(act->act_scale, 16) || !aligned_to(act->act_shift, 16))
+      return B200GNN_ERR_BAD_ARG;
+    p.act_scale = act->act_scale; p.act_shift = act->act_shift; p.act_bits = act->act_bits; p.act_words = act->act_words;
+    p.inv_keep = act->inv_keep;
+  }
+  if (act && !st) {
+    if (K > (int64_t)gemm::STAT_BYTES / 8) return B200GNN_ERR_UNSUPPORTED;
+    if (N <= 48) return gemm::launch<gemm::Cfg<48, 6>, 0, false, true>(A, lda, B_hi, B_lo, ldb, p, (cudaStream_t)stream);
+    return gemm::launch<gemm::Cfg<128, 4>, 0, false, true>(A, lda, B_hi, B_lo, ldb, p, (cudaStream_t)stream);
+  }
   if (st) {
     if (N % 32 || N > gemm::STAT_MAX_N || N <= 48 || ldc % 4 || !aligned_to(C, 16) || !st->stat_partial) return B200GNN_ERR_UNSUPPORTED;
     p.stat_mode = st->stat_mode; p.stat_partial = st->stat_partial; p.bn_x = st->bn_x; p.bn_y = st->bn_y;
     p.bn_mean = st->bn_mean; p.bn_invstd = st->bn_invstd; p.inv_keep = st->inv_keep;
     if (p.stat_mode == 1) return gemm::launch<gemm::Cfg<128, 4>, 1>(A, lda, B_hi, B_lo, ldb, p, (cudaStream_t)stream);
-    if (N % 128 == 0 && (g_bnbwd_variant == 1 || (g_bnbwd_variant == 0 && K < gemm::BNBWD_TMA_MAX_K)))
-      return gemm::launch<gemm::Cfg<128, 2, gemm::XY_BYTES>, 3>(A, lda, B_hi, B_lo, ldb, p, (cudaStream_t)stream);
+    const bool tma = N % 128 == 0 && (g_bnbwd_variant == 1 || (g_bnbwd_variant == 0 && K < gemm::BNBWD_TMA_MAX_K));
+    if (act)
+      return tma ? gemm::launch<gemm::Cfg<128, 2, gemm::XY_BYTES>, 3, false, true>(A, lda, B_hi, B_lo, ldb, p, (cudaStream_t)stream)
+                 : gemm::launch<gemm::Cfg<128, 4>, 2, false, true>(A, lda, B_hi, B_lo, ldb, p, (cudaStream_t)stream);
+    if (tma) return gemm::launch<gemm::Cfg<128, 2, gemm::XY_BYTES>, 3>(A, lda, B_hi, B_lo, ldb, p, (cudaStream_t)stream);
     return gemm::launch<gemm::Cfg<128, 4>, 2>(A, lda, B_hi, B_lo, ldb, p, (cudaStream_t)stream);
   }
   if (N <= 48) return gemm::launch<gemm::Cfg<48, 6>>(A, lda, B_hi, B_lo, ldb, p, (cudaStream_t)stream);
@@ -438,6 +521,33 @@
   st.stat_mode = 2; st.stat_partial = partial; st.bn_x = Xout; st.bn_y = Y; st.bn_mean = mean; st.bn_invstd = invstd;
   st.inv_keep = p_drop > 0.f ? 1.f / (1.f - p_drop) : 1.f;
   return gemm_dispatch(A, lda, B_hi, B_lo, ldb, C, ldc, M, N, K, nullptr, accumulate, stream, &st);
+}
+
+extern "C" int b200gnn_gemm_tf32x3_bnbwd_bits_f32(const float* A, int64_t lda, const float* B_hi, const float* B_lo, int64_t ldb,
+                                                  float* C, int64_t ldc, int64_t M, int64_t N, int64_t K, int accumulate,
+                                                  const uint32_t* bits, const float* Y, const float* mean, const float* invstd,
+                                                  const float* scale, const float* shift, float p_drop, float* partial,
+                                                  int64_t slots, void* stream) {
+  if (!partial || !bits || !Y || !mean || !invstd || p_drop < 0.f || p_drop >= 1.f || slots < b200gnn_gemm_stat_slots(M, N))
+    return B200GNN_ERR_BAD_ARG;
+  if (!aligned_to(Y, 16) || !aligned_to(mean, 16) || !aligned_to(invstd, 16)) return B200GNN_ERR_UNSUPPORTED;
+  gemm::Params st{}, act{};
+  st.stat_mode = 2; st.stat_partial = partial; st.bn_y = Y; st.bn_mean = mean; st.bn_invstd = invstd;
+  st.inv_keep = p_drop > 0.f ? 1.f / (1.f - p_drop) : 1.f;
+  act.act_scale = scale; act.act_shift = shift; act.act_bits = bits; act.act_words = (int32_t)((N + 31) / 32);
+  act.inv_keep = st.inv_keep;
+  return gemm_dispatch(A, lda, B_hi, B_lo, ldb, C, ldc, M, N, K, nullptr, accumulate, stream, &st, &act);
+}
+
+extern "C" int b200gnn_gemm_tf32x3_act_f32(const float* Y, int64_t lda, const float* B_hi, const float* B_lo, int64_t ldb,
+                                           float* C, int64_t ldc, int64_t M, int64_t N, int64_t K, const float* bias,
+                                           const float* scale, const float* shift, const uint32_t* bits, float p_drop,
+                                           void* stream) {
+  if (p_drop < 0.f || p_drop >= 1.f) return B200GNN_ERR_BAD_ARG;
+  gemm::Params act{};
+  act.act_scale = scale; act.act_shift = shift; act.act_bits = bits; act.act_words = (int32_t)((K + 31) / 32);
+  act.inv_keep = p_drop > 0.f ? 1.f / (1.f - p_drop) : 1.f;
+  return gemm_dispatch(Y, lda, B_hi, B_lo, ldb, C, ldc, M, N, K, bias, 0, stream, nullptr, &act);
 }
 
 extern "C" int b200gnn_gemm_tf32x3_f32(const float* A, int64_t lda, const float* B_hi, const float* B_lo, int64_t ldb,
diff --git a/efficient-gnns_b200/csrc/gemm_wgrad_tf32x3.cu b/efficient-gnns_b200/csrc/gemm_wgrad_tf32x3.cu
--- a/efficient-gnns_b200/csrc/gemm_wgrad_tf32x3.cu
+++ b/efficient-gnns_b200/csrc/gemm_wgrad_tf32x3.cu
@@ -13,7 +13,8 @@
 constexpr int RAW_BYTES = BKN * (TM + TN) * 4;
 constexpr int OP_BYTES = 128 * BKN * 4;
 constexpr int T_BYTES = 2 * OP_BYTES;
-constexpr int SMEM_BYTES = STAGES * RAW_BYTES + 2 * T_BYTES + 256 + 1024;
+constexpr int SS_BYTES = TM / 2 * 16;
+constexpr int SMEM_BYTES = STAGES * RAW_BYTES + 2 * T_BYTES + 256 + SS_BYTES + 1024;
 constexpr int MAX_RANGES = 132;
 constexpr int64_t MAX_PARTIAL_FLOATS = (int64_t)MAX_RANGES * 256 * 256;
 constexpr int MAX_KIN = 2048, MAX_NOUT = 512;
@@ -23,8 +24,14 @@
   float* partial;
   int32_t Nn, Kin, Kpad, Nout, Npad, num_kb;
   int32_t n_tn, n_ranges;
+  const float* act_scale;
+  const float* act_shift;
+  const uint32_t* act_bits;
+  int32_t act_words;
+  float inv_keep;
 };
 
+template <bool ACT>
 __global__ void __launch_bounds__(THREADS, 1)
 wgrad_tf32x3_kernel(const __grid_constant__ CUtensorMap tmX, const __grid_constant__ CUtensorMap tmG, const Params p) {
   extern __shared__ uint8_t smem_raw[];
@@ -32,6 +39,7 @@
   uint8_t* tbuf = smem + STAGES * RAW_BYTES;
   uint64_t* full = reinterpret_cast<uint64_t*>(tbuf + 2 * T_BYTES);
   uint64_t* empty = full + STAGES;
+  float4* act_ss = reinterpret_cast<float4*>(tbuf + 2 * T_BYTES + 256);
 
   const int tiles = (p.Kpad / TM) * p.n_tn;
   const int tile = (int)blockIdx.x % tiles, range = (int)blockIdx.x / tiles;
@@ -67,13 +75,42 @@
   const int cw = (warp >> 2) - 1;
   const int ct = threadIdx.x - 128;
   const uint32_t xfrag = (8 * cw + 2 * (warp & 3)) * (BKN * X_BOX * 4) + (lane & 3) * (X_BOX * 4) + (lane >> 2) * 4;
+  const int pair = cw * 32 + (warp & 3) * 8 + (lane >> 2);
+  const int c0 = mt * TM + cw * 64 + (warp & 3) * 16 + (lane >> 2);
+  uint32_t wnext = 0u;
+  auto act_word = [&](int kb) {
+    const int node = kb * BKN + lane;
+    return node < p.Nn && (c0 >> 5) < p.act_words ? __ldg(p.act_bits + (size_t)node * p.act_words + (c0 >> 5)) : 0u;
+  };
+  if (ACT) {
+    if (ct < TM / 2) {
+      const int c = mt * TM + (ct >> 3) * 16 + (ct & 7);
+      float4 v = make_float4(0.f, 0.f, 0.f, 0.f);
+      if (c < p.Kin) { v.x = __ldg(p.act_scale + c); v.y = __ldg(p.act_shift + c); }
+      if (c + 8 < p.Kin) { v.z = __ldg(p.act_scale + c + 8); v.w = __ldg(p.act_shift + c + 8); }
+      act_ss[ct] = v;
+    }
+    if (kb0 < kb1) wnext = act_word(kb0);
+    named_sync(1, 256);
+  }
   float acc[64], sum[64];
 #pragma unroll
   for (int i = 0; i < 64; ++i) sum[i] = acc[i] = 0.f;
   uint32_t xh0[BKN / 8][4], xl0[BKN / 8][4], xh1[BKN / 8][4], xl1[BKN / 8][4];
   int s = 0; uint32_t ph = 0;
   auto block = [&](int i, uint32_t (&h)[BKN / 8][4], uint32_t (&l)[BKN / 8][4]) {
+    uint32_t wcur = 0u;
+    if (ACT) {
+      wcur = wnext;
+      if (kb0 + i + 1 < kb1) wnext = act_word(kb0 + i + 1);
+    }
     mbar_wait(&full[s], ph);
+    float4 ss = make_float4(0.f, 0.f, 0.f, 0.f);
+    int l4 = lane & 3;
+    if (ACT) {
+      ss = act_ss[pair];
+      asm volatile("" : "+r"(l4));
+    }
     const uint32_t sraw = smem_u32(smem + s * RAW_BYTES);
     const float* rg = reinterpret_cast<const float*>(smem + s * RAW_BYTES + BKN * TM * 4);
     uint8_t* T = tbuf + (i & 1) * T_BYTES;
@@ -92,8 +129,15 @@
 #pragma unroll
     for (int k = 0; k < BKN / 8; ++k)
 #pragma unroll
-      for (int j = 0; j < 4; ++j)
-        split1(lds32(sraw + xfrag + (j & 1) * (BKN * X_BOX * 4) + (8 * k + 4 * (j >> 1)) * (X_BOX * 4)), h[k][j], l[k][j]);
+      for (int j = 0; j < 4; ++j) {
+        uint32_t v = lds32(sraw + xfrag + (j & 1) * (BKN * X_BOX * 4) + (8 * k + 4 * (j >> 1)) * (X_BOX * 4));
+        if (ACT) {
+          const uint32_t w = __shfl_sync(0xffffffffu, wcur, 8 * k + l4 + 4 * (j >> 1));
+          const float y = fmaxf(fmaf(__uint_as_float(v), (j & 1) ? ss.z : ss.x, (j & 1) ? ss.w : ss.y), 0.f) * p.inv_keep;
+          v = (w >> ((c0 & 31) + 8 * (j & 1))) & 1u ? __float_as_uint(y) : 0u;
+        }
+        split1(v, h[k][j], l[k][j]);
+      }
     asm volatile("fence.proxy.async.shared::cta;" ::: "memory");
     mbar_arrive(&empty[s]);
     if (i > 0) {
@@ -196,8 +240,9 @@
   return wgrad::range_cap(Kin, Nout) * wgrad::pad_k(Kin) * wgrad::pad_n(Nout);
 }
 
-extern "C" int b200gnn_gemm_wgrad_tf32x3_f32(const float* X, int64_t ldx, const float* G, int64_t ldg, float* dW,
-                                             int64_t Nn, int64_t Kin, int64_t Nout, float* workspace, void* stream) {
+template <bool ACT>
+static int wgrad_launch(const float* X, int64_t ldx, const float* G, int64_t ldg, float* dW, int64_t Nn, int64_t Kin, int64_t Nout,
+                        float* workspace, const wgrad::Params& act, void* stream) {
   if (!X || !G || !dW || !workspace || Nn <= 0 || Kin <= 0 || Nout <= 0 || ldx < Kin || ldg < Nout || Nn >= INT32_MAX)
     return B200GNN_ERR_BAD_ARG;
   if (Kin % 4 || Kin > wgrad::MAX_KIN || Nout % 4 || Nout > wgrad::MAX_NOUT || ldx % 4 || ldg % 4 || !aligned_to(X, 16) || !aligned_to(G, 16) ||
@@ -210,14 +255,14 @@
   cudaGetDevice(&dev);
   static bool attr_set[64] = {};
   if (dev >= 0 && dev < 64 && !attr_set[dev]) {
-    cudaError_t e = cudaFuncSetAttribute(wgrad::wgrad_tf32x3_kernel, cudaFuncAttributeMaxDynamicSharedMemorySize,
+    cudaError_t e = cudaFuncSetAttribute(wgrad::wgrad_tf32x3_kernel<ACT>, cudaFuncAttributeMaxDynamicSharedMemorySize,
                                          wgrad::SMEM_BYTES);
     if (e != cudaSuccess) { set_cuda_error(e); return B200GNN_ERR_CUDA; }
     attr_set[dev] = true;
   }
   cudaDeviceGetAttribute(&sms, cudaDevAttrMultiProcessorCount, dev);
   cudaStream_t st = (cudaStream_t)stream;
-  wgrad::Params p;
+  wgrad::Params p = act;
   p.partial = workspace; p.Nn = (int32_t)Nn; p.Kin = (int32_t)Kin; p.Nout = (int32_t)Nout;
   p.Kpad = (int32_t)wgrad::pad_k(Kin);
   p.Npad = (int32_t)wgrad::pad_n(Nout);
@@ -231,10 +276,25 @@
   if (ranges < 1) ranges = 1;
   p.n_ranges = ranges;
   int rc;
-  wgrad::wgrad_tf32x3_kernel<<<tiles * ranges, wgrad::THREADS, wgrad::SMEM_BYTES, st>>>(tX, tG, p);
+  wgrad::wgrad_tf32x3_kernel<ACT><<<tiles * ranges, wgrad::THREADS, wgrad::SMEM_BYTES, st>>>(tX, tG, p);
   if ((rc = check_launch())) return rc;
   const int64_t n_vec = (int64_t)p.Kpad * p.Npad / 4;
   wgrad::wgrad_reduce_kernel<<<(int)((n_vec + wgrad::RED_VECS - 1) / wgrad::RED_VECS), wgrad::RED_VECS * wgrad::RED_GROUPS, 0, st>>>(
       reinterpret_cast<const float4*>(workspace), ranges, (int)Kin, p.Kpad, (int)Nout, p.Npad, dW);
   return check_launch();
 }
+
+extern "C" int b200gnn_gemm_wgrad_tf32x3_f32(const float* X, int64_t ldx, const float* G, int64_t ldg, float* dW,
+                                             int64_t Nn, int64_t Kin, int64_t Nout, float* workspace, void* stream) {
+  return wgrad_launch<false>(X, ldx, G, ldg, dW, Nn, Kin, Nout, workspace, wgrad::Params{}, stream);
+}
+
+extern "C" int b200gnn_gemm_wgrad_tf32x3_act_f32(const float* Y, int64_t ldx, const float* G, int64_t ldg, float* dW,
+                                                 int64_t Nn, int64_t Kin, int64_t Nout, const float* scale, const float* shift,
+                                                 const uint32_t* bits, float p_drop, float* workspace, void* stream) {
+  if (!scale || !shift || !bits || p_drop < 0.f || p_drop >= 1.f) return B200GNN_ERR_BAD_ARG;
+  wgrad::Params act{};
+  act.act_scale = scale; act.act_shift = shift; act.act_bits = bits; act.act_words = (int32_t)((Kin + 31) / 32);
+  act.inv_keep = p_drop > 0.f ? 1.f / (1.f - p_drop) : 1.f;
+  return wgrad_launch<true>(Y, ldx, G, ldg, dW, Nn, Kin, Nout, workspace, act, stream);
+}
diff --git a/efficient-gnns_b200/dist.py b/efficient-gnns_b200/dist.py
--- a/efficient-gnns_b200/dist.py
+++ b/efficient-gnns_b200/dist.py
@@ -89,7 +89,7 @@
         rowptr, col, val = shard_rows(rel, self.plan, self.rank)
         self._shard = csr_graph_from(rowptr, col, val, self.plan.real_rows(self.rank), self.plan.n_pad)
         self.n_global = adj.size(0)
-        super().__init__(adj, dims, _prebuilt_graph=self._shard, _rows_alloc=self.plan.block, **kw)
+        super().__init__(adj, dims, _prebuilt_graph=self._shard, _rows_alloc=self.plan.block, **{**kw, "fuse_activations": False})
         dev = self.device
         self.full = {k: torch.empty(self.plan.n_pad, k, device=dev) for k in set(dims[1:])}
         self.sum_buf = {k: torch.empty(2, k, device=dev) for k in set(dims[1:])}
diff --git a/efficient-gnns_b200/engine.py b/efficient-gnns_b200/engine.py
--- a/efficient-gnns_b200/engine.py
+++ b/efficient-gnns_b200/engine.py
@@ -36,7 +36,7 @@
     def __init__(self, adj: SparseTensor, dims: List[int], dropout: float = 0.5, lr: float = 0.01, seed: int = 0,
                  alpha: float = 0.9, kd_T: float = 4.0, bn_eps: float = 1e-5, bn_momentum: float = 0.1,
                  aggregate_first: Optional[bool] = None, tensor_core_gemm: bool = True, overlap_wgrad: bool = True,
-                 fuse_row_passes: bool = True, _prebuilt_graph: Optional[CsrGraph] = None, _rows_alloc: Optional[int] = None):
+                 fuse_row_passes: bool = True, fuse_activations: bool = True, _prebuilt_graph: Optional[CsrGraph] = None, _rows_alloc: Optional[int] = None):
         assert adj.is_cuda(), "the engine runs on a CUDA device"
         self.device = adj.device
         self.dims, self.L = list(dims), len(dims) - 1
@@ -112,7 +112,7 @@
             return blk[:N]
         self.H = [buf(dims[l + 1]) for l in range(self.L)]
         self.Y = [buf(dims[l + 1]) for l in range(self.L)]
-        self.A = [buf(dims[l + 1]) for l in range(self.L - 1)]
+        self._A = [buf(dims[l + 1]) for l in range(self.L - 1)]
         self.dY = [buf(dims[l + 1]) for l in range(self.L)]
         self.dH = [buf(dims[l + 1]) for l in range(self.L)]
         self.dA = [buf(dims[l + 1]) for l in range(self.L - 1)]
@@ -124,6 +124,15 @@
         self.fuse_rows = bool(fuse_row_passes) and self.tc_gemm
         self._gemm_part = {k: torch.empty(ops.gemm_stat_slots(N, k), 2, k, device=dev)
                            for k in set(dims[1:-1]) if self.fuse_rows and ops.gemm_stats_supported(k)}
+        hid = dims[1:-1]
+        self.fuse_act = (bool(fuse_activations) and self.fuse_rows and self.L >= 2 and len(set(hid)) == 1
+                         and ops.gemm_stats_supported(hid[0]) and hid[0] <= 2048
+                         and all(ops.wgrad_supported(dims[l], dims[l + 1]) for l in range(1, self.L)))
+        self.keep_bits = (torch.zeros(self.L - 1, N, (hid[0] + 31) // 32, dtype=torch.int32, device=dev)
+                          if self.fuse_act else None)
+        self._act_stale = False
+        self._fwd_fused = False
+        self._ev_bits = torch.cuda.Event()
         self.loss_out = self._grads_buf[self.n_par_pad:self.n_par_pad + 3]
         self.kd_part = torch.empty(2 * int(lib.load().b200gnn_kd_partials(N)), device=dev)
         self._graph = None
@@ -166,6 +175,17 @@
             if f"bns.{l}.running_mean" in sd:
                 self.running_mean[l].copy_(sd[f"bns.{l}.running_mean"]); self.running_var[l].copy_(sd[f"bns.{l}.running_var"])
 
+    @property
+    def A(self) -> List[torch.Tensor]:
+        if self._act_stale:
+            self._act_stale = False
+            for l in range(self.L - 1):
+                ops.affine_relu_bits(self.Y[l], self.keep_bits[l], self.bn[l][2], self.bn[l][3], self.p, out=self._A[l])
+        return self._A
+
+    def _act(self, l: int):
+        return self.Y[l], self.bn[l][2], self.bn[l][3], self.keep_bits[l]
+
     def activation_pattern(self, l: int) -> torch.Tensor:
         return self.A[l] > 0
 
@@ -176,6 +196,18 @@
         return layer + step * self.L
 
     def forward(self, x: torch.Tensor, training: bool = True) -> torch.Tensor:
+        fused = training and self.fuse_act
+        self._act_stale = False
+        if fused:
+            if self._side is not None:
+                self._ev_fork.record(torch.cuda.current_stream())
+                self._side.wait_event(self._ev_fork)
+                with torch.cuda.stream(self._side):
+                    ops.dropout_bits(self.keep_bits, self.p, self.seed, 0, step_dev=self.step_count, step_mul=self.L)
+                self._ev_bits.record(self._side)
+            else:
+                ops.dropout_bits(self.keep_bits, self.p, self.seed, 0, step_dev=self.step_count, step_mul=self.L)
+        A = self._A
         inp = x
         for l in range(self.L):
             last = l == self.L - 1
@@ -192,36 +224,46 @@
                         part = ops.col_stats(self.Y[0], partial=self._part(self.dims[1]))
                     ops.bn_finalize(part, self.N, self.gamma[0], self.beta[0], self.bn_eps,
                                     self.bn_momentum, self.running_mean[0], self.running_var[0], out=self.bn[0])
-                    ops.affine_relu_dropout(self.Y[0], self.bn[0][2], self.bn[0][3], True, self.p, self.seed, 0,
-                                            out=self.A[0], step_dev=self.step_count, step_mul=self.L)
+                    if not fused:
+                        ops.affine_relu_dropout(self.Y[0], self.bn[0][2], self.bn[0][3], True, self.p, self.seed, 0,
+                                                out=A[0], step_dev=self.step_count, step_mul=self.L)
                 else:
                     self._linear(0, self.AX, self.Y[0], bias=self.b[0])
                     scale = self.gamma[0] * torch.rsqrt(self.running_var[0] + self.bn_eps)
                     shift = self.beta[0] - self.running_mean[0] * scale
-                    ops.affine_relu_dropout(self.Y[0], scale, shift, True, 0.0, out=self.A[0])
-                inp = self.A[0]
+                    ops.affine_relu_dropout(self.Y[0], scale, shift, True, 0.0, out=A[0])
+                inp = A[0]
                 continue
-            self._linear(l, inp, self.H[l])
+            if fused and l > 0:
+                if l == 1 and self._side is not None:
+                    torch.cuda.current_stream().wait_event(self._ev_bits)
+                self._linear(l, None, self.H[l], act=self._act(l - 1))
+            else:
+                self._linear(l, inp, self.H[l])
             if last:
                 ops.spmm_csr(self.G, self.H[l], "sum", bias=self.b[l], out=self.Y[l])
             elif training:
                 ops.spmm_csr(self.G, self.H[l], "sum", bias=self.b[l], out=self.Y[l], stat_partial=self.stat_part[l])
                 ops.bn_finalize(self.stat_part[l], self.N, self.gamma[l], self.beta[l], self.bn_eps, self.bn_momentum,
                                 self.running_mean[l], self.running_var[l], out=self.bn[l])
-                ops.affine_relu_dropout(self.Y[l], self.bn[l][2], self.bn[l][3], True, self.p, self.seed, l,
-                                        out=self.A[l], step_dev=self.step_count, step_mul=self.L)
-                inp = self.A[l]
+                if not fused:
+                    ops.affine_relu_dropout(self.Y[l], self.bn[l][2], self.bn[l][3], True, self.p, self.seed, l,
+                                            out=A[l], step_dev=self.step_count, step_mul=self.L)
+                inp = A[l]
             else:
                 ops.spmm_csr(self.G, self.H[l], "sum", bias=self.b[l], out=self.Y[l])
                 scale = self.gamma[l] * torch.rsqrt(self.running_var[l] + self.bn_eps)
                 shift = self.beta[l] - self.running_mean[l] * scale
-                ops.affine_relu_dropout(self.Y[l], scale, shift, True, 0.0, out=self.A[l])
-                inp = self.A[l]
+                ops.affine_relu_dropout(self.Y[l], scale, shift, True, 0.0, out=A[l])
+                inp = A[l]
+        self._act_stale = self._fwd_fused = fused
         return self.Y[-1]
 
     def backward(self, x: torch.Tensor, d_out_feat: Optional[torch.Tensor] = None):
+        fused = self._fwd_fused
         for l in range(self.L - 1, -1, -1):
-            inp = x if l == 0 else self.A[l - 1]
+            act = self._act(l - 1) if fused and l > 0 else None
+            inp = x if l == 0 else (None if act else self._A[l - 1])
             if l == self.L - 1:
                 ops.col_sum(self.dY[l], out=self.gb[l], partial=self._part(self.dims[l + 1]))
             if l == 0 and self.agg_first:
@@ -236,11 +278,15 @@
                     d_prev = d_out_feat
                 if gp is not None:
                     hi, lo = ops.split_tf32(self.W[l], transpose=False, hi=self.W_split[l][0], lo=self.W_split[l][1])
-                    ops.gemm_tf32x3_bnbwd(self.dH[l], hi, lo, d_prev, self.A[l - 1], self.Y[l - 1], self.bn[l - 1][0],
-                                          self.bn[l - 1][1], self.p, gp, accumulate=acc)
+                    if act:
+                        ops.gemm_tf32x3_bnbwd_bits(self.dH[l], hi, lo, d_prev, act[3], self.Y[l - 1], self.bn[l - 1][0],
+                                                   self.bn[l - 1][1], act[1], act[2], self.p, gp, accumulate=acc)
+                    else:
+                        ops.gemm_tf32x3_bnbwd(self.dH[l], hi, lo, d_prev, self._A[l - 1], self.Y[l - 1], self.bn[l - 1][0],
+                                              self.bn[l - 1][1], self.p, gp, accumulate=acc)
                 else:
                     self._linear_dgrad(l, self.dH[l], d_prev, accumulate=acc)
-            self._wgrad_async(l, inp, self.dH[l])
+            self._wgrad_async(l, inp, self.dH[l], act=act)
             if l > 0:
                 k = self.dims[l]
                 part = self._part(k)
@@ -249,26 +295,29 @@
                                          gp, self.N, self.p, self.dY[l - 1], self.ggamma[l - 1], self.gbeta[l - 1],
                                          self.gb[l - 1], part, self._coef(k))
                 else:
-                    ops.bn_act_bwd(d_prev, self.A[l - 1], self.Y[l - 1], self.bn[l - 1][0], self.bn[l - 1][1],
+                    ops.bn_act_bwd(d_prev, self._A[l - 1], self.Y[l - 1], self.bn[l - 1][0], self.bn[l - 1][1],
                                    self.gamma[l - 1], self.p, d_y=self.dY[l - 1], d_gamma=self.ggamma[l - 1],
                                    d_beta=self.gbeta[l - 1], d_bias=self.gb[l - 1], partial=part, coef=self._coef(k))
         self._wgrad_join()
 
-    def _wgrad_async(self, l: int, inp: torch.Tensor, d_out: torch.Tensor):
+    def _wgrad_async(self, l: int, inp: Optional[torch.Tensor], d_out: torch.Tensor, act=None):
         if self._side is None:
-            return self._linear_wgrad(l, inp, d_out)
+            return self._linear_wgrad(l, inp, d_out, act)
         self._ev_fork.record(torch.cuda.current_stream())
         self._side.wait_event(self._ev_fork)
         with torch.cuda.stream(self._side):
-            self._linear_wgrad(l, inp, d_out)
+            self._linear_wgrad(l, inp, d_out, act)
 
     def _wgrad_join(self):
         if self._side is not None:
             self._ev_join.record(self._side)
             torch.cuda.current_stream().wait_event(self._ev_join)
 
-    def _linear(self, l: int, inp: torch.Tensor, out: torch.Tensor, bias: Optional[torch.Tensor] = None):
-        if self.tc_gemm:
+    def _linear(self, l: int, inp: Optional[torch.Tensor], out: torch.Tensor, bias: Optional[torch.Tensor] = None, act=None):
+        if act is not None:
+            hi, lo = ops.split_tf32(self.W[l], transpose=True, hi=self.Wt_split[l][0], lo=self.Wt_split[l][1])
+            ops.gemm_tf32x3_act(*act, self.p, hi, lo, bias=bias, out=out)
+        elif self.tc_gemm:
             hi, lo = ops.split_tf32(self.W[l], transpose=True, hi=self.Wt_split[l][0], lo=self.Wt_split[l][1])
             ops.gemm_tf32x3(inp, hi, lo, bias=bias, out=out)
         elif bias is not None:
@@ -285,8 +334,10 @@
         else:
             torch.mm(d_out, self.W[l].t(), out=d_inp)
 
-    def _linear_wgrad(self, l: int, inp: torch.Tensor, d_out: torch.Tensor):
-        if self.tc_gemm and ops.wgrad_supported(self.dims[l], self.dims[l + 1]):
+    def _linear_wgrad(self, l: int, inp: Optional[torch.Tensor], d_out: torch.Tensor, act=None):
+        if act is not None:
+            ops.gemm_wgrad_tf32x3_act(*act, self.p, d_out, out=self.gW[l], workspace=self.wgrad_ws)
+        elif self.tc_gemm and ops.wgrad_supported(self.dims[l], self.dims[l + 1]):
             ops.gemm_wgrad_tf32x3(inp, d_out, out=self.gW[l], workspace=self.wgrad_ws)
         else:
             torch.mm(inp.t(), d_out, out=self.gW[l])
@@ -349,6 +400,7 @@
 
     def replay(self, key: int = 0) -> torch.Tensor:
         self._graph[key].replay()
+        self._act_stale = self.fuse_act
         return self.loss_out
 
     def launches_per_step(self) -> int:
diff --git a/efficient-gnns_b200/hybrid.py b/efficient-gnns_b200/hybrid.py
--- a/efficient-gnns_b200/hybrid.py
+++ b/efficient-gnns_b200/hybrid.py
@@ -190,7 +190,7 @@
         self._shard = csr_graph_from(rowptr, col, val, self.n_p, self.n_global)
         frp, fcol, fval = rel.csr()
         self.Gfull = csr_graph_from(frp, fcol, fval, self.n_global, self.n_global)
-        super().__init__(adj, dims, _prebuilt_graph=self._shard, _rows_alloc=self.plan.block, **kw)
+        super().__init__(adj, dims, _prebuilt_graph=self._shard, _rows_alloc=self.plan.block, **{**kw, "fuse_activations": False})
         dev = self.device
         N, L = self.n_global, self.L
         self.row0 = self.plan.offsets[self.rank]
diff --git a/efficient-gnns_b200/lib.py b/efficient-gnns_b200/lib.py
--- a/efficient-gnns_b200/lib.py
+++ b/efficient-gnns_b200/lib.py
@@ -50,6 +50,8 @@
     "b200gnn_affine_relu_dropout_scatter_f32": (_int, [_f32p, _f32p, _i64, _i64, _f32p, _f32p, _int, _f32, _u64, _u64,
                                                        _i32p, _u64, _i32p, _u64, _i64, _i64, _ptr, _ptr, _i32, _i64, _ptr]),
     "b200gnn_dropout_mask_u8": (_int, [_ptr, _i64, _i64, _f32, _u64, _u64, _ptr]),
+    "b200gnn_dropout_bits_u32": (_int, [_ptr, _i64, _i64, _i64, _f32, _u64, _u64, _i32p, _u64, _ptr]),
+    "b200gnn_affine_relu_bits_f32": (_int, [_f32p, _ptr, _f32p, _f32p, _f32, _f32p, _i64, _i64, _ptr]),
     "b200gnn_relu_dropout_bwd_f32": (_int, [_f32p, _f32p, _f32p, _i64, _i64, _f32, _ptr]),
     "b200gnn_bn_act_bwd_f32": (_int, [_f32p, _f32p, _f32p, _f32p, _f32p, _f32p, _i64, _i64, _f32, _f32p, _f32p,
                                       _f32p, _f32p, _f32p, _i64, _f32p, _ptr]),
@@ -72,11 +74,17 @@
                                              _ptr]),
     "b200gnn_gemm_tf32x3_bnbwd_f32": (_int, [_f32p, _i64, _f32p, _f32p, _i64, _f32p, _i64, _i64, _i64, _i64, _int,
                                              _f32p, _f32p, _f32p, _f32p, _f32, _f32p, _i64, _ptr]),
+    "b200gnn_gemm_tf32x3_bnbwd_bits_f32": (_int, [_f32p, _i64, _f32p, _f32p, _i64, _f32p, _i64, _i64, _i64, _i64, _int,
+                                                  _ptr, _f32p, _f32p, _f32p, _f32p, _f32p, _f32, _f32p, _i64, _ptr]),
+    "b200gnn_gemm_tf32x3_act_f32": (_int, [_f32p, _i64, _f32p, _f32p, _i64, _f32p, _i64, _i64, _i64, _i64, _f32p,
+                                           _f32p, _f32p, _ptr, _f32, _ptr]),
     "b200gnn_gemm_tf32x3_acc_f32": (_int, [_f32p, _i64, _f32p, _f32p, _i64, _f32p, _i64, _i64, _i64, _i64, _ptr]),
     "b200gnn_gemm_tf32x3_scatter_f32": (_int, [_f32p, _i64, _f32p, _f32p, _i64, _ptr, _i32, _i64, _i64, _i64, _i64, _f32p, _ptr]),
     "b200gnn_gemm_tf32x3_bcast_f32": (_int, [_f32p, _i64, _f32p, _f32p, _i64, _ptr, _i32, _i64, _i64, _i64, _i64, _i64, _f32p, _ptr]),
     "b200gnn_wgrad_workspace_floats": (_i64, [_i64, _i64]),
     "b200gnn_gemm_wgrad_tf32x3_f32": (_int, [_f32p, _i64, _f32p, _i64, _f32p, _i64, _i64, _i64, _f32p, _ptr]),
+    "b200gnn_gemm_wgrad_tf32x3_act_f32": (_int, [_f32p, _i64, _f32p, _i64, _f32p, _i64, _i64, _i64, _f32p, _f32p, _ptr, _f32,
+                                                 _f32p, _ptr]),
     "b200gnn_row_normalize_fwd_f32": (_int, [_f32p, _i64, _i64, _f32, _f32, _f32p, _f32p, _ptr]),
     "b200gnn_row_normalize_bwd_f32": (_int, [_f32p, _f32p, _f32p, _i64, _i64, _f32, _f32, _f32p, _int, _ptr]),
     "b200gnn_reduce_slots": (_i64, [_i64]),
diff --git a/efficient-gnns_b200/ops.py b/efficient-gnns_b200/ops.py
--- a/efficient-gnns_b200/ops.py
+++ b/efficient-gnns_b200/ops.py
@@ -186,6 +186,33 @@
     lib.check(lib.load().b200gnn_dropout_mask_u8(mask.data_ptr(), n_rows, K, p, seed, offset, lib.stream_ptr()),
               "dropout_mask_u8")
     return mask
+
+
+def dropout_bits(bits: torch.Tensor, p: float, seed: int, offset: int, step_dev: Optional[torch.Tensor] = None,
+                 step_mul: int = 0, K: Optional[int] = None) -> torch.Tensor:
+    n_layers, n, words = bits.shape
+    K = 32 * words if K is None else K
+    assert bits.dtype == torch.int32 and bits.is_contiguous() and words == (K + 31) // 32
+    lib.check(lib.load().b200gnn_dropout_bits_u32(bits.data_ptr(), n_layers, n, K, p, seed, offset,
+                                                  lib.dptr(step_dev, torch.int32, "step_dev"), step_mul, lib.stream_ptr()),
+              "dropout_bits_u32")
+    return bits
+
+
+def _bits(bits: torch.Tensor, n: int, K: int) -> int:
+    if bits.dtype != torch.int32 or not bits.is_cuda or not bits.is_contiguous() or tuple(bits.shape) != (n, (K + 31) // 32):
+        raise lib.B200GnnError(f"keep bits: expected a contiguous CUDA int32 [{n}, {(K + 31) // 32}] tensor")
+    return bits.data_ptr()
+
+
+def affine_relu_bits(y: torch.Tensor, bits: torch.Tensor, scale: torch.Tensor, shift: torch.Tensor, p: float,
+                     out: Optional[torch.Tensor] = None) -> torch.Tensor:
+    n, K = y.shape
+    if out is None:
+        out = torch.empty_like(y)
+    lib.check(lib.load().b200gnn_affine_relu_bits_f32(_f32(y, "y"), _bits(bits, n, K), _f32(scale, "scale"), _f32(shift, "shift"),
+                                                      p, _f32(out, "out"), n, K, lib.stream_ptr()), "affine_relu_bits_f32")
+    return out
 
 
 def bn_act_bwd(d_out, x_out, y, mean, invstd, gamma, p: float, d_y=None, d_gamma=None, d_beta=None, d_bias=None,
@@ -299,6 +326,35 @@
     return out
 
 
+def gemm_tf32x3_bnbwd_bits(a: torch.Tensor, b_hi: torch.Tensor, b_lo: torch.Tensor, out: torch.Tensor, bits: torch.Tensor,
+                           y: torch.Tensor, mean: torch.Tensor, invstd: torch.Tensor, scale: torch.Tensor, shift: torch.Tensor,
+                           p: float, partial: torch.Tensor, accumulate: bool = False) -> torch.Tensor:
+    M, K = a.shape
+    N = b_hi.shape[0]
+    assert out.shape == y.shape and out.stride(0) == y.stride(0)
+    lib.check(lib.load().b200gnn_gemm_tf32x3_bnbwd_bits_f32(_f32(a, "a"), a.stride(0), _f32(b_hi, "b_hi"), _f32(b_lo, "b_lo"),
+                                                            b_hi.stride(0), _f32(out, "out"), out.stride(0), M, N, K, int(accumulate),
+                                                            _bits(bits, M, N), _f32(y, "y"), _f32(mean, "mean"), _f32(invstd, "invstd"),
+                                                            _f32(scale, "scale"), _f32(shift, "shift"), float(p),
+                                                            _f32(partial, "partial"), partial.shape[0], lib.stream_ptr()),
+              "gemm_tf32x3_bnbwd_bits_f32")
+    return out
+
+
+def gemm_tf32x3_act(y: torch.Tensor, scale: torch.Tensor, shift: torch.Tensor, bits: torch.Tensor, p: float, b_hi: torch.Tensor,
+                    b_lo: torch.Tensor, bias: Optional[torch.Tensor] = None, out: Optional[torch.Tensor] = None) -> torch.Tensor:
+    M, K = y.shape
+    N = b_hi.shape[0]
+    assert b_hi.shape == b_lo.shape and b_hi.shape[1] == K
+    if out is None:
+        out = torch.empty(M, N, dtype=torch.float32, device=y.device)
+    lib.check(lib.load().b200gnn_gemm_tf32x3_act_f32(_f32(y, "y"), y.stride(0), _f32(b_hi, "b_hi"), _f32(b_lo, "b_lo"),
+                                                     b_hi.stride(0), _f32(out, "out"), out.stride(0), M, N, K, _f32(bias, "bias"),
+                                                     _f32(scale, "scale"), _f32(shift, "shift"), _bits(bits, M, K), float(p),
+                                                     lib.stream_ptr()), "gemm_tf32x3_act_f32")
+    return out
+
+
 def gemm_tf32x3_scatter(a: torch.Tensor, b_hi: torch.Tensor, b_lo: torch.Tensor, dst_ptrs, row_off: int,
                         bias: Optional[torch.Tensor] = None) -> None:
     import ctypes as C
@@ -347,6 +403,26 @@
     lib.check(L.b200gnn_gemm_wgrad_tf32x3_f32(_f32(x, "x"), x.stride(0), _f32(g, "g"), g.stride(0), _f32(out, "out"), nn_,
                                               k_in, n_out, _f32(workspace, "workspace"), lib.stream_ptr()),
               "gemm_wgrad_tf32x3_f32")
+    return out
+
+
+def gemm_wgrad_tf32x3_act(y: torch.Tensor, scale: torch.Tensor, shift: torch.Tensor, bits: torch.Tensor, p: float,
+                          g: torch.Tensor, out: Optional[torch.Tensor] = None,
+                          workspace: Optional[torch.Tensor] = None) -> torch.Tensor:
+    nn_, k_in = y.shape
+    n_out = g.shape[1]
+    assert g.shape[0] == nn_
+    if not wgrad_supported(k_in, n_out):
+        raise lib.B200GnnError(f"gemm_wgrad_tf32x3_act: Kin={k_in}, Nout={n_out} is outside the 128/256-row tilings")
+    L = lib.load()
+    if out is None:
+        out = torch.empty(k_in, n_out, dtype=torch.float32, device=y.device)
+    if workspace is None:
+        workspace = torch.empty(int(L.b200gnn_wgrad_workspace_floats(k_in, n_out)), dtype=torch.float32, device=y.device)
+    lib.check(L.b200gnn_gemm_wgrad_tf32x3_act_f32(_f32(y, "y"), y.stride(0), _f32(g, "g"), g.stride(0), _f32(out, "out"), nn_,
+                                                  k_in, n_out, _f32(scale, "scale"), _f32(shift, "shift"), _bits(bits, nn_, k_in),
+                                                  float(p), _f32(workspace, "workspace"), lib.stream_ptr()),
+              "gemm_wgrad_tf32x3_act_f32")
     return out
 
 
diff --git a/include/b200gnn.h b/include/b200gnn.h
--- a/include/b200gnn.h
+++ b/include/b200gnn.h
@@ -86,6 +86,10 @@
                                             const int32_t* row_off, int32_t world, int64_t ld_dst, void* stream);
 int b200gnn_dropout_mask_u8(uint8_t* mask, int64_t n_rows, int64_t K, float p,
                             uint64_t seed, uint64_t offset, void* stream);
+int b200gnn_dropout_bits_u32(uint32_t* bits, int64_t n_layers, int64_t n_rows, int64_t K, float p, uint64_t seed,
+                             uint64_t offset, const int32_t* step_dev, uint64_t step_mul, void* stream);
+int b200gnn_affine_relu_bits_f32(const float* Y, const uint32_t* bits, const float* scale, const float* shift,
+                                 float p, float* out, int64_t n_rows, int64_t K, void* stream);
 int b200gnn_relu_dropout_bwd_f32(const float* dOut, const float* Xout, float* dY,
                                  int64_t n_rows, int64_t K, float p, void* stream);
 int b200gnn_bn_act_bwd_f32(const float* dOut, const float* Xout, const float* Y,
@@ -140,6 +144,15 @@
                                   float* C, int64_t ldc, int64_t M, int64_t N, int64_t K, int accumulate,
                                   const float* Xout, const float* Y, const float* mean, const float* invstd, float p_drop,
                                   float* partial, int64_t slots, void* stream);
+int b200gnn_gemm_tf32x3_bnbwd_bits_f32(const float* A, int64_t lda, const float* B_hi, const float* B_lo, int64_t ldb,
+                                       float* C, int64_t ldc, int64_t M, int64_t N, int64_t K, int accumulate,
+                                       const uint32_t* bits, const float* Y, const float* mean, const float* invstd,
+                                       const float* scale, const float* shift, float p_drop, float* partial,
+                                       int64_t slots, void* stream);
+int b200gnn_gemm_tf32x3_act_f32(const float* Y, int64_t lda, const float* B_hi, const float* B_lo, int64_t ldb,
+                                float* C, int64_t ldc, int64_t M, int64_t N, int64_t K, const float* bias,
+                                const float* scale, const float* shift, const uint32_t* bits, float p_drop,
+                                void* stream);
 int b200gnn_gemm_tf32x3_scatter_f32(const float* A, int64_t lda, const float* B_hi, const float* B_lo,
                                     int64_t ldb, float* const* C_ptrs, int32_t world, int64_t row_off,
                                     int64_t M, int64_t N, int64_t K, const float* bias, void* stream);
@@ -152,6 +165,9 @@
                                   int64_t ldg, float* dW, int64_t Nn,
                                   int64_t Kin, int64_t Nout, float* workspace,
                                   void* stream);
+int b200gnn_gemm_wgrad_tf32x3_act_f32(const float* Y, int64_t ldx, const float* G, int64_t ldg, float* dW,
+                                      int64_t Nn, int64_t Kin, int64_t Nout, const float* scale, const float* shift,
+                                      const uint32_t* bits, float p_drop, float* workspace, void* stream);
 
 int b200gnn_row_normalize_fwd_f32(const float* x, int64_t n, int64_t F, float eps,
                                   float scale, float* out, float* norm_out,
```
